# loyer-yuan/GeneralSparse

Hardware: AMD Instinct MI355X
Metric: SpMM GFLOP/s + achieved HBM GB/s vs rocSPARSE, pruned-weight fp16 N=32 (higher is better)
Workload: dtype f16 (fp32 accumulate)

## Files before the change

### generalsparse_amd/_lib.py

```python
import ctypes
import os

PKG_DIR = os.path.dirname(os.path.abspath(__file__))
LIB_PATH = os.environ.get("GS_LIBRARY") or os.path.join(PKG_DIR, "libgeneralsparse.so")

GS_F32 = 0
GS_F16 = 1
GS_BF16 = 2

u64p = ctypes.POINTER(ctypes.c_uint64)
f32p = ctypes.POINTER(ctypes.c_float)
f64p = ctypes.POINTER(ctypes.c_double)


class GsOpts(ctypes.Structure):
    _fields_ = [("pipeline", ctypes.c_char_p), ("dtype", ctypes.c_int), ("dense_n", ctypes.c_int),
                ("p0", ctypes.c_int), ("p1", ctypes.c_int), ("ones_values", ctypes.c_int),
                ("device", ctypes.c_int)]


class GsPlanInfo(ctypes.Structure):
    _fields_ = [("rows", ctypes.c_uint64), ("cols", ctypes.c_uint64), ("nnz", ctypes.c_uint64),
                ("nnz_stored", ctypes.c_uint64), ("n_units", ctypes.c_uint64),
                ("device_bytes_A", ctypes.c_uint64), ("family", ctypes.c_int), ("col_bytes", ctypes.c_int),
                ("dtype", ctypes.c_int), ("replicas", ctypes.c_int), ("needs_memset", ctypes.c_int),
                ("kernel_name", ctypes.c_char * 64), ("lds_stage", ctypes.c_int), ("lds_n", ctypes.c_uint32),
                ("lds_kc", ctypes.c_uint32), ("lds_chunks", ctypes.c_uint32), ("lds_waves", ctypes.c_uint32),
                ("lds_bytes", ctypes.c_uint64), ("tile_bytes", ctypes.c_uint64), ("ksplit", ctypes.c_uint32),
                ("n_kernels", ctypes.c_int), ("device_kernel", ctypes.c_char * 32),
                ("index_formulas", ctypes.c_int), ("index_bytes_saved", ctypes.c_uint64),
                ("ks_nt", ctypes.c_uint32), ("ks_head_groups", ctypes.c_uint32),
                ("nm_tiles", ctypes.c_uint32)]


SIGNATURES = {
    "gs_plan_logical_check": ([ctypes.c_void_p, ctypes.c_char_p, ctypes.c_int], ctypes.c_int),
    "gs_plan_array_set_u64": ([ctypes.c_void_p, ctypes.c_char_p, ctypes.c_uint64, ctypes.c_uint64], ctypes.c_int),
    "gs_last_error": ([], ctypes.c_char_p),
    "gs_version": ([], ctypes.c_char_p),
    "gs_opts_default": ([ctypes.POINTER(GsOpts)], None),
    "gs_plan_create_from_mtx": ([ctypes.c_char_p, ctypes.c_int, ctypes.POINTER(ctypes.c_void_p)], ctypes.c_int),
    "gs_plan_create_from_coo": ([ctypes.c_uint64, ctypes.c_uint64, ctypes.c_uint64, u64p, u64p, f32p,
                                 ctypes.POINTER(ctypes.c_void_p)], ctypes.c_int),
    "gs_set_config_int": ([ctypes.c_char_p, ctypes.c_longlong], ctypes.c_int),
    "gs_get_config_int": ([ctypes.c_char_p, ctypes.POINTER(ctypes.c_longlong)], ctypes.c_int),
    "gs_plan_add_operator": ([ctypes.c_void_p, ctypes.c_char_p, ctypes.POINTER(ctypes.c_longlong), ctypes.c_int],
                             ctypes.c_int),
    "gs_plan_run_pipeline": ([ctypes.c_void_p, ctypes.c_char_p, ctypes.c_int, ctypes.c_int, ctypes.c_int],
                             ctypes.c_int),
    "gs_plan_add_operator_sub": ([ctypes.c_void_p, ctypes.c_int, ctypes.c_char_p, ctypes.POINTER(ctypes.c_longlong),
                                  ctypes.c_int], ctypes.c_int),
    "gs_plan_run_pipeline_sub": ([ctypes.c_void_p, ctypes.c_int, ctypes.c_char_p, ctypes.c_int, ctypes.c_int,
                                  ctypes.c_int], ctypes.c_int),
    "gs_plan_sub_matrices": ([ctypes.c_void_p, ctypes.POINTER(ctypes.c_int), ctypes.c_int], ctypes.c_int),
    "gs_plan_compile": ([ctypes.c_void_p], ctypes.c_int),
    "gs_plan_generate_program": ([ctypes.c_void_p, ctypes.c_char_p, ctypes.c_int, ctypes.c_char_p, ctypes.c_int],
                                 ctypes.c_int),
    "gs_plan_upload": ([ctypes.c_void_p, ctypes.c_int, ctypes.c_int], ctypes.c_int),
    "gs_convert_values": ([f32p, ctypes.c_uint64, ctypes.c_int, ctypes.c_void_p], ctypes.c_int),
    "gs_plan_add_replica": ([ctypes.c_void_p], ctypes.c_int),
    "gs_spmm": ([ctypes.c_void_p, ctypes.c_void_p, ctypes.c_void_p, ctypes.c_int, ctypes.c_void_p], ctypes.c_int),
    "gs_spmm_replica": ([ctypes.c_void_p, ctypes.c_int, ctypes.c_void_p, ctypes.c_void_p, ctypes.c_int,
                         ctypes.c_void_p], ctypes.c_int),
    "gs_spmm_batch": ([ctypes.POINTER(ctypes.c_void_p), ctypes.POINTER(ctypes.c_int), ctypes.POINTER(ctypes.c_void_p),
                       ctypes.POINTER(ctypes.c_void_p), ctypes.c_int, ctypes.c_int, ctypes.c_void_p], ctypes.c_int),
    "gs_spmm_rotate": ([ctypes.c_void_p, ctypes.c_int, ctypes.c_int, ctypes.POINTER(ctypes.c_void_p),
                        ctypes.POINTER(ctypes.c_void_p), ctypes.c_int, ctypes.c_int, ctypes.c_void_p], ctypes.c_int),
    "gs_batch_launches": ([ctypes.POINTER(ctypes.c_void_p), ctypes.POINTER(ctypes.c_int), ctypes.c_int, ctypes.c_int,
                           ctypes.POINTER(ctypes.c_int), ctypes.c_int], ctypes.c_int),
    "gs_plan_device_status": ([ctypes.c_void_p, ctypes.c_void_p], ctypes.c_int),
    "gs_plan_info_get": ([ctypes.c_void_p, ctypes.POINTER(GsPlanInfo)], ctypes.c_int),
    "gs_plan_array_count": ([ctypes.c_void_p], ctypes.c_int),
    "gs_plan_array_key": ([ctypes.c_void_p, ctypes.c_int, ctypes.c_char_p, ctypes.c_int], ctypes.c_int),
    "gs_plan_array_len": ([ctypes.c_void_p, ctypes.c_char_p], ctypes.c_longlong),
    "gs_plan_array_is_float": ([ctypes.c_void_p, ctypes.c_char_p], ctypes.c_int),
    "gs_plan_array_read_u64": ([ctypes.c_void_p, ctypes.c_char_p, u64p, ctypes.c_uint64], ctypes.c_int),
    "gs_plan_array_read_f64": ([ctypes.c_void_p, ctypes.c_char_p, f64p, ctypes.c_uint64], ctypes.c_int),
    "gs_plan_log": ([ctypes.c_void_p, ctypes.c_char_p, ctypes.c_int], ctypes.c_int),
    "gs_plan_save": ([ctypes.c_void_p, ctypes.c_char_p], ctypes.c_int),
    "gs_plan_load": ([ctypes.c_char_p, ctypes.POINTER(ctypes.c_void_p)], ctypes.c_int),
    "gs_plan_index_compression": ([ctypes.c_void_p, ctypes.c_char_p, ctypes.c_char_p, ctypes.c_int, ctypes.c_char_p,
                                   ctypes.c_int, ctypes.POINTER(ctypes.c_int)], ctypes.c_int),
    "gs_index_compression_of_array": ([u64p, ctypes.c_uint64, ctypes.c_int, ctypes.c_int, ctypes.c_char_p, ctypes.c_int,
                                       u64p, ctypes.POINTER(ctypes.c_int)], ctypes.c_int),
    "gs_debug_mfma_timeline": ([ctypes.c_void_p, ctypes.c_void_p, ctypes.c_void_p, ctypes.c_int, ctypes.c_void_p,
# ... 42 lines not shown
```

### generalsparse_amd/csrc/hip_code/mfma_ks.hpp

```cpp
#pragma once

#include "kernel_common.hpp"

namespace gsk {

template <int N>
__device__ constexpr int vmcnt_imm() {
    static_assert(N >= 0 && N < 64, "vmcnt is six bits");
    return (N & 0xF) | ((N >> 4) << 14) | 0x70 | 0xF00;
}


template <int CT, int RT, int W, int D, int MAXG, bool STAMPS, bool AP = true, bool P8 = false, int NTL = 0, class ET = f16>
__device__ __forceinline__ void ks_body(const uint32_t *__restrict__ bmtb_first_row, const u32x4 *__restrict__ tP,
                                        const u32x4 *__restrict__ tV, const u32x2 *__restrict__ steps,
                                        const ET *__restrict__ B, ET *__restrict__ C, uint32_t K, uint32_t N, uint32_t S,
                                        uint32_t NS, uint32_t nwg, uint32_t row_base, float *__restrict__ slabs,
                                        uint32_t *__restrict__ arrivals, uint64_t *__restrict__ stamps, uint32_t bx,
                                        uint32_t prio) {
    constexpr uint32_t RB = 32 * CT;
    constexpr uint32_t UB = 2 * CT;
    constexpr uint32_t IMG = ks_image_bytes<RT>();
    constexpr uint32_t STG = 32u * RB;
    extern __shared__ __attribute__((aligned(16))) unsigned char lds[];
    const uint32_t tid = threadIdx.x, lane = tid & 63u;
    const uint32_t wv = __builtin_amdgcn_readfirstlane(tid >> 6);
    const uint32_t u = xcd_block(bx, nwg);
    const uint32_t g = u / S, q = u - g * S;
#define GS_KS_STAMP(slot)                                                                          \
    if constexpr (STAMPS) {                                                                        \
        if (lane == 0) stamps[((size_t)blockIdx.x * W + wv) * 32u + (slot)] = __builtin_amdgcn_s_memtime(); \
    }
    GS_KS_STAMP(0u);
    const uint32_t k0 = q * NS * 32u;
    const uint32_t col0 = blockIdx.y * 16u * CT, nv = min(16u * CT, N - col0);
    unsigned char *img = lds + wv * (IMG + STG);
    unsigned char *bst = img + IMG;
    const u32x4 zero4 = {0u, 0u, 0u, 0u};

    const uint32_t nsw = NS > wv ? (NS - wv + W - 1u) / W : 0u;
    const size_t ubase = (size_t)u * NS;
    using PV = typename std::conditional<P8, u32x2, u32x4>::type;
    const PV *tPp = reinterpret_cast<const PV *>(tP);
    PV P[D][MAXG];
    u32x4 V[D][MAXG], BR[D][CT];
    u32x2 NX[D];
    uint32_t CN[D];
    uint32_t vz;
    __asm__ volatile("v_mov_b32 %0, 0" : "=v"(vz));
    auto rec_of = [&](uint32_t i) -> u32x2 {
        const uint32_t st = __builtin_amdgcn_readfirstlane(i < nsw ? wv + i * W : 0u);
        return steps[ubase + st + vz];
    };
    auto load_b = [&](uint32_t i, u32x4 (&B_)[CT]) {
        const uint32_t st = __builtin_amdgcn_readfirstlane(i < nsw ? wv + i * W : 0u);
        const uint32_t kr = k0 + st * 32u;
#pragma unroll
        for (int c = 0; c < CT; c++) {
            const uint32_t un = lane + 64u * c;
            const uint32_t k = kr + un / UB, cu = (un % UB) * 8u;
            B_[c] = ld_once_if<(NTL & 2) != 0>(
                reinterpret_cast<const u32x4 *>(B + (size_t)(k < K ? k : K - 1u) * N + col0 + (cu < nv ? cu : 0u)));
        }
    };
    auto load_g_at = [&](uint32_t i, uint32_t b0, uint32_t gc, u32x2 &NX_, uint32_t &CN_, PV (&P_)[MAXG],
                         u32x4 (&V_)[MAXG]) {
        CN_ = gc;
        NX_ = rec_of(i + D);
#pragma unroll
        for (int j = 0; j < MAXG; j++) {
            const uint32_t qg = lane + 64u * j;
            const size_t at = (size_t)b0 + (qg < gc ? qg : 0u);
            P_[j] = ld_once_if<(NTL & 1) != 0>(tPp + at);
            V_[j] = ld_once_if<(NTL & 1) != 0>(tV + at);
        }
    };
    auto load_g = [&](uint32_t i, u32x2 &NX_, uint32_t &CN_, PV (&P_)[MAXG], u32x4 (&V_)[MAXG]) {
        load_g_at(i, __builtin_amdgcn_readfirstlane(NX_[0]), __builtin_amdgcn_readfirstlane(NX_[1]), NX_, CN_, P_, V_);
    };
    const uint32_t GH = (prio >> 8) & 0x3ffu;
    if (GH) {
#pragma unroll
        for (int d = 0; d < D; d++) load_b((uint32_t)d, BR[d]);
#pragma unroll
        for (int d = 0; d < D; d++) {
            const uint32_t st = (uint32_t)d < nsw ? wv + (uint32_t)d * W : 0u;
            load_g_at((uint32_t)d, (u * min((uint32_t)(W * D), NS) + st) * GH, GH, NX[d], CN[d], P[d], V[d]);
        }
        for (uint32_t x = lane; x < IMG / 16u; x += 64u) *reinterpret_cast<u32x4 *>(img + x * 16u) = zero4;
    } else {
#pragma unroll
        for (int d = 0; d < D; d++) NX[d] = rec_of((uint32_t)d);
#pragma unroll
        for (int d = 0; d < D; d++) load_b((uint32_t)d, BR[d]);
        for (uint32_t x = lane; x < IMG / 16u; x += 64u) *reinterpret_cast<u32x4 *>(img + x * 16u) = zero4;
#pragma unroll
        for (int d = 0; d < D; d++) load_g((uint32_t)d, NX[d], CN[d], P[d], V[d]);
    }
    GS_KS_STAMP(1u);

    f4v acc[RT][CT];
#pragma unroll
    for (int rt = 0; rt < RT; rt++)
#pragma unroll
        for (int ct = 0; ct < CT; ct++) acc[rt][ct] = f4v{0.f, 0.f, 0.f, 0.f};
    uint32_t arow[RT];
#pragma unroll
    for (int rt = 0; rt < RT; rt++) arow[rt] = (16u * rt + (lane & 15u)) * kKsStride + 16u * (lane >> 4);

    auto ent_h = [&](const PV &p, uint32_t hb, int e) -> uint32_t {
        if constexpr (P8) {
            const uint32_t b = (p[e >> 2] >> (8 * (e & 3))) & 0x7fu;
            return hb + 48u * (b >> 4) + (b & 15u);
        } else {
            return (p[e >> 1] >> (16 * (e & 1))) & 0xffffu;
        }
    };
    auto grp_hb = [&](const PV &p) -> uint32_t {
        if constexpr (P8) {
            const uint32_t x = p[0], y = p[1];
            const uint32_t sg = ((x >> 7) & 1u) | ((x >> 14) & 2u) | ((x >> 21) & 4u) | ((x >> 28) & 8u) | ((y >> 3) & 16u);
            return 384u * (sg >> 1) + 16u * (sg & 1u);
        } else {
            return 0u;
        }
    };
    auto step = [&](uint32_t i, u32x2 &NX_, uint32_t &CN_, PV (&P_)[MAXG], u32x4 (&V_)[MAXG], u32x4 (&B_)[CT]) {
        const bool live = i < nsw;
        const uint32_t gc = CN_;
        typedef typename mfma_elem<ET>::frag frag;
        frag av[RT], bv[CT];
        if (live) {
            const uint32_t kr = k0 + (wv + i * W) * 32u;
#pragma unroll
            for (int c = 0; c < CT; c++) {
                const uint32_t un = lane + 64u * c, k = un / UB, s = un % UB;
                *reinterpret_cast<u32x4 *>(bst + k * RB + b_piece<CT>(k, s >> 1) * 32u + (s & 1u) * 16u) =
                    kr + k < K && s * 8u < nv ? B_[c] : zero4;
            }
#pragma unroll
            for (int j = 0; j < MAXG; j++) {
                if (lane + 64u * j < gc) {
                    const uint32_t hb = grp_hb(P_[j]);
#pragma unroll
                    for (int e = 0; e < 8; e++) {
                        const uint32_t h = ent_h(P_[j], hb, e);
                        const uint16_t v = (uint16_t)((V_[j][e >> 1] >> (16 * (e & 1))) & 0xffffu);
                        *reinterpret_cast<uint16_t *>(img + h * 2u) = v;
                    }
                }
            }
#pragma unroll
            for (int rt = 0; rt < RT; rt++) av[rt] = *reinterpret_cast<const frag *>(img + arow[rt]);
            const uint32_t kb = 8u * (lane >> 4);
#pragma unroll
            for (int ct = 0; ct < CT; ct++) {
                s4v t[2];
#pragma unroll
                for (int hh = 0; hh < 2; hh++) {
                    const uint32_t k = kb + 4u * hh + ((lane & 15u) >> 2);
                    t[hh] = __builtin_amdgcn_ds_read_tr16_b64_v4i16(
                        (lds_s4v *)(bst + k * RB + b_piece<CT>(k, ct) * 32u + (lane & 3u) * 8u));
                }
                __builtin_memcpy(&bv[ct], t, 16);
            }
#pragma unroll
            for (int j = 0; j < MAXG; j++) {
                if (lane + 64u * j < gc) {
                    const uint32_t hb = grp_hb(P_[j]);
#pragma unroll
                    for (int e = 0; e < 8; e++) *reinterpret_cast<uint16_t *>(img + ent_h(P_[j], hb, e) * 2u) = (uint16_t)0;
                }
            }
        }
        load_b(i + D, B_);
        load_g(i + D, NX_, CN_, P_, V_);
        if (live) {
#pragma unroll
            for (int rt = 0; rt < RT; rt++)
#pragma unroll
                for (int ct = 0; ct < CT; ct++)
                    acc[rt][ct] = mfma_elem<ET>::mfma_16x16x32(av[rt], bv[ct], acc[rt][ct]);
            if (i < 16u) GS_KS_STAMP(3u + i);
        }
    };
    const bool young = wv >= W / 2u;
    if ((prio & 3u) && young) __builtin_amdgcn_s_setprio(1);
    for (uint32_t i0 = 0; i0 < nsw; i0 += D) {
#pragma unroll
        for (int d = 0; d < D; d++) step(i0 + d, NX[d], CN[d], P[d], V[d], BR[d]);
        if ((prio & 3u) == 2u && young && i0 + D >= nsw / 2u && i0 < nsw / 2u) __builtin_amdgcn_s_setprio(0);
    }
    if ((prio & 3u) && young) __builtin_amdgcn_s_setprio(0);
    GS_KS_STAMP(20u);
    uint32_t *arr = arrivals + (size_t)g * gridDim.y + blockIdx.y;
    uint32_t ticket = 0;
    if (S > 1 && wv == 0 && lane == 0) ticket = __hip_atomic_fetch_add(arr, 1u, __ATOMIC_RELAXED, __HIP_MEMORY_SCOPE_AGENT);
    constexpr bool APART = ks_red_apart(CT, RT, W, AP);
    f4v *red = reinterpret_cast<f4v *>(lds + (APART ? (size_t)W * (IMG + STG) : 0u));
    constexpr bool HALVES = !APART && ks_red_halves(CT, RT, W);
    constexpr uint32_t WR = HALVES ? W / 2 : W;
    uint32_t *flag = reinterpret_cast<uint32_t *>(reinterpret_cast<unsigned char *>(red) + (size_t)WR * RT * CT * 1024u);
    if constexpr (!APART) {
        __asm__ volatile("s_waitcnt lgkmcnt(0)" ::: "memory");
        __builtin_amdgcn_s_barrier();
        __asm__ volatile("" ::: "memory");
    }
    if constexpr (HALVES) {
        if (wv >= WR) {
#pragma unroll
            for (int rt = 0; rt < RT; rt++)
#pragma unroll
                for (int ct = 0; ct < CT; ct++) red[(((wv - WR) * RT + rt) * CT + ct) * 64u + lane] = acc[rt][ct];
        }
        __asm__ volatile("s_waitcnt lgkmcnt(0)" ::: "memory");
        __builtin_amdgcn_s_barrier();
        __asm__ volatile("" ::: "memory");
        if (wv < WR) {
#pragma unroll
            for (int rt = 0; rt < RT; rt++)
#pragma unroll
                for (int ct = 0; ct < CT; ct++) acc[rt][ct] += red[((wv * RT + rt) * CT + ct) * 64u + lane];
        }
        __asm__ volatile("s_waitcnt lgkmcnt(0)" ::: "memory");
        __builtin_amdgcn_s_barrier();
        __asm__ volatile("" ::: "memory");
    }
    if (wv < WR) {
#pragma unroll
        for (int rt = 0; rt < RT; rt++)
#pragma unroll
            for (int ct = 0; ct < CT; ct++) red[((wv * RT + rt) * CT + ct) * 64u + lane] = acc[rt][ct];
    }
    if (S > 1 && wv == 0 && lane == 0) *flag = ticket;
    __asm__ volatile("s_waitcnt lgkmcnt(0)" ::: "memory");
    __builtin_amdgcn_s_barrier();
    __asm__ volatile("" ::: "memory");
    constexpr uint32_t NI = RT * CT * 64u, NT = 64u * W;
    const uint32_t r0 = bmtb_first_row[g], R = bmtb_first_row[g + 1] - r0;
    auto item_sum = [&](uint32_t t) {
        f4v sum = red[t];
#pragma unroll
        for (uint32_t w = 1; w < WR; w++) sum += red[w * NI + t];
// ... 4 lines not shown
        const uint32_t col = 16u * ct + (ln & 15u), rb = 16u * rt + 4u * (ln >> 4);
        if (col >= nv) return;
#pragma unroll
        for (uint32_t i = 0; i < 4; i++)
            if (rb + i < R) C[(size_t)(row_base + r0 + rb + i) * N + col0 + col] = (ET)v[i];
    };
    GS_KS_STAMP(21u);
    if (S == 1) {
        for (uint32_t t = tid; t < NI; t += NT) store_item(t, item_sum(t));
        GS_KS_STAMP(22u);
        return;
    }
    const uint32_t tk = *flag & 0xffffu, tag = ((*flag >> 16) & 1u) ^ 1u;
    f4v *slab = reinterpret_cast<f4v *>(slabs) + ((size_t)u * gridDim.y + blockIdx.y) * NI;
    auto tagged = [&](const f4v &v) {
        u32x4 w;
        __builtin_memcpy(&w, &v, 16);
        w[0] = (w[0] & ~1u) | tag; w[1] = (w[1] & ~1u) | tag; w[2] = (w[2] & ~1u) | tag; w[3] = (w[3] & ~1u) | tag;
        return w;
    };
    for (uint32_t t = tid; t < NI; t += NT) {
        const u32x4 w = tagged(item_sum(t));
        __asm__ volatile("global_store_dwordx4 %0, %1, off sc1" ::"v"(slab + t), "v"(w) : "memory");
    }
    if (tk != S - 1u) {
        GS_KS_STAMP(22u);
        return;
    }
    if (tid == 0) __hip_atomic_store(arr, tag << 16, __ATOMIC_RELAXED, __HIP_MEMORY_SCOPE_AGENT);
    const f4v *base = reinterpret_cast<const f4v *>(slabs) + blockIdx.y * NI;
    const size_t qstride = (size_t)gridDim.y * NI;
    uint32_t *err = arrivals + (size_t)(nwg / S) * gridDim.y;
    for (uint32_t t = tid; t < NI; t += NT) {
        f4v sum = {0.f, 0.f, 0.f, 0.f};
        for (uint32_t qq = 0; qq < S; qq++) {
            u32x4 w;
            if (qq == q) {
                w = tagged(item_sum(t));
            } else {
                w = ks_slab_wait(reinterpret_cast<const uint32_t *>(base + ((size_t)g * S + qq) * qstride + t), tag, err,
                                 GS_KS_FORCE(prio));
            }
            w[0] &= ~1u; w[1] &= ~1u; w[2] &= ~1u; w[3] &= ~1u;
            f4v x;
            __builtin_memcpy(&x, &w, 16);
            sum += x;
        }
        store_item(t, sum);
    }
    GS_KS_STAMP(22u);
#undef GS_KS_STAMP
}

template <int CT, int RT, int W, int D, int MAXG, bool STAMPS = false, bool AP = true, bool P8 = false, int NTL = 0, class ET = f16>
__global__ __launch_bounds__(64 * W) void k_mfma_ks(const uint32_t *__restrict__ bmtb_first_row,
                                                    const u32x4 *__restrict__ tP,
                                                    const u32x4 *__restrict__ tV,
                                                    const u32x2 *__restrict__ steps,
                                                    const ET *__restrict__ B, ET *__restrict__ C, uint32_t K,
                                                    uint32_t N, uint32_t S, uint32_t NS, uint32_t nwg,
                                                    uint32_t row_base, float *__restrict__ slabs,
                                                    uint32_t *__restrict__ arrivals, uint64_t *__restrict__ stamps = nullptr,
                                                    uint32_t prio = 0) {
    ks_body<CT, RT, W, D, MAXG, STAMPS, AP, P8, NTL, ET>(bmtb_first_row, tP, tV, steps, B, C, K, N, S, NS, nwg, row_base, slabs,
                                                    arrivals, stamps, blockIdx.x, prio);
}

#ifdef GS_EXPERIMENTS
template <int CT, int RT, int W, int D, int MAXG, int NTL = 0>
__global__ __launch_bounds__(64 * W) void k_mfma_ks_persist(const uint32_t *__restrict__ bmtb_first_row,
                                                            const u32x4 *__restrict__ tP, const u32x4 *__restrict__ tV,
                                                            const u32x2 *__restrict__ steps, const f16 *__restrict__ B,
                                                            f16 *__restrict__ C, uint32_t K, uint32_t N, uint32_t S,
                                                            uint32_t NS, uint32_t nunits, uint32_t row_base,
                                                            float *__restrict__ slabs, uint32_t *__restrict__ arrivals,
                                                            uint32_t prio, uint32_t *__restrict__ queue) {
    __shared__ uint32_t next_sh;
    uint32_t xcc;
    asm volatile("s_getreg_b32 %0, hwreg(HW_REG_XCC_ID, 0, 4)" : "=s"(xcc));
    xcc &= 7u;
    const uint32_t grid = gridDim.x;
    uint32_t u = blockIdx.x, qx = xcc, tried = 0;
    while (u < nunits) {
        uint32_t pulled = 0;
        if (threadIdx.x == 0) pulled = __hip_atomic_fetch_add(queue + qx, 1u, __ATOMIC_RELAXED, __HIP_MEMORY_SCOPE_AGENT);
        ks_body<CT, RT, W, D, MAXG, false, true, false, NTL>(bmtb_first_row, tP, tV, steps, B, C, K, N, S, NS, nunits,
                                                          row_base, slabs, arrivals, nullptr, u, prio);
        __syncthreads();
        if (threadIdx.x == 0) next_sh = pulled;
        __syncthreads();
        u = grid + qx + 8u * next_sh;
        __syncthreads();
        while (u >= nunits && ++tried < 8u) {
            qx = (qx + 1u) & 7u;
            if (threadIdx.x == 0) next_sh = __hip_atomic_fetch_add(queue + qx, 1u, __ATOMIC_RELAXED, __HIP_MEMORY_SCOPE_AGENT);
            __syncthreads();
            u = grid + qx + 8u * next_sh;
            __syncthreads();
        }
    }
    if (threadIdx.x == 0 && __hip_atomic_fetch_add(queue + 8, 1u, __ATOMIC_RELAXED, __HIP_MEMORY_SCOPE_AGENT) == grid - 1u) {
        for (int i = 0; i < 9; i++) __hip_atomic_store(queue + i, 0u, __ATOMIC_RELAXED, __HIP_MEMORY_SCOPE_AGENT);
    }
}
#endif

struct ks_entry {
    const uint32_t *tbr;
    const u32x4 *tP, *tV;
    const u32x2 *steps;
    const void *B;
    void *C;
    float *slabs;
    uint32_t *arrivals;
    uint32_t K, S, NS, nwg, row_base, pad0, pad1, pad2;
};
struct ks_group_args {
    uint32_t begin[kKsGroupMax + 1];
    uint32_t n, N, pad[2];
    ks_entry e[kKsGroupMax];
};

template <int CT, int RT, int W, int D, int MAXG, bool P8 = false, bool AP = true, int NTL = 0, class ET = f16>
__global__ __launch_bounds__(64 * W) void k_mfma_ks_group(ks_group_args args) {
    const uint32_t bx = blockIdx.x, n = args.n;
    uint32_t sel = 0;
#pragma unroll
    for (int i = 1; i < kKsGroupMax; i++)
        if ((uint32_t)i < n && args.begin[i] <= bx) sel = (uint32_t)i;
    sel = __builtin_amdgcn_readfirstlane(sel);
    const ks_entry &e = args.e[sel];
    if (bx - args.begin[sel] >= e.nwg) return;
    ks_body<CT, RT, W, D, MAXG, false, AP, P8, NTL, ET>(e.tbr, e.tP, e.tV, e.steps, (const ET *)e.B, (ET *)e.C, e.K, args.N, e.S, e.NS,
                                                   e.nwg, e.row_base, e.slabs, e.arrivals, nullptr, bx - args.begin[sel],
                                                   args.pad[0] | (e.pad0 << 8));
}

}
```

### generalsparse_amd/csrc/host/capi.cc

```cpp
#include "../../../include/generalsparse.h"
#include "gs_plan.hpp"
#include "index_compress.hpp"

#include <algorithm>
#include <cstring>
#include <map>
#include <memory>

struct replica_scratch {
    std::vector<void *> bufs;
    void **ptrs_dev = nullptr;
    uint32_t N = 0;
};

struct parent_group {
    uint64_t base = 0, rows = 0;
    std::vector<gs::plan_state *> subs;
    std::vector<uint32_t> part_rows;
    std::vector<replica_scratch> rep;
    uint32_t *rows_dev = nullptr;
    int device = 0;
};

struct gs_plan {
// ... 758 lines not shown
                                   "): the affected rows of C hold NaN", GS_ERR_DEVICE);
    });
}

int gs_spmm(gs_plan_t *p, const void *B, void *C, int N, gs_stream_t stream) {
    return gs_spmm_replica(p, 0, B, C, N, stream);
}

int gs_debug_mfma_timeline(gs_plan_t *p, const void *B, void *C, int N, gs_stream_t stream, uint64_t *stamps,
                           uint64_t n_stamps) {
    return guard([&] {
        GS_CHECK(p && B && C && stamps, "null argument");
        gs::debug_mfma_timeline(p->st, B, C, (uint32_t)N, (hipStream_t)stream, stamps, n_stamps);
    });
}

int gs_plan_info_get(gs_plan_t *p, gs_plan_info *info) {
    return guard([&] {
        GS_CHECK(p && info, "null argument");
        std::memset(info, 0, sizeof(*info));
        auto ks = kernel_states(p, false);
        auto &s = *ks.front();
        info->rows = s.M;
        info->cols = s.K;
        info->nnz = s.nnz;
        info->n_kernels = (int)ks.size();
        for (gs::plan_state *k : ks) info->nnz_stored += s.meta->u(gs::GLOBAL_META, "nz_col_indices", k->cg->get_sub_matrix_id()).size();
        if (s.cg->is_compiled()) {
            const auto &sp = s.cg->get_kernel_spec();
            info->family = sp.family;
            std::strncpy(info->kernel_name, sp.name().c_str(), sizeof(info->kernel_name) - 1);
        }
        if (s.uploaded) {
            info->n_units = s.dev.n_units;
            info->device_bytes_A = s.dev.bytes_A;
            info->col_bytes = s.dev.col_bytes;
            info->dtype = s.dev.dtype;
            info->replicas = (int)s.dev.replicas.size();
            info->needs_memset = s.dev.needs_memset ? 1 : 0;
            info->lds_stage = s.dev.nm ? 3 : (s.dev.mfma ? 2 : (s.dev.lds ? 1 : 0));
            info->lds_n = s.dev.lds_N;
            info->lds_kc = s.dev.KC;
            info->lds_chunks = s.dev.nc;
            info->lds_waves = s.dev.waves;
            info->lds_bytes = s.dev.lds_bytes;
            info->tile_bytes = s.dev.bytes_tile;
            info->ksplit = s.dev.ksplit;
            const std::string dk = !s.dev.kernel.empty() ? s.dev.kernel : s.cg->get_kernel_spec().name();
            std::strncpy(info->device_kernel, dk.c_str(), sizeof(info->device_kernel) - 1);
            info->index_formulas = s.dev.index_formulas;
            info->index_bytes_saved = s.dev.index_bytes_saved;
            info->ks_nt = s.dev.ks ? s.dev.ks_nt : 0;
            info->ks_head_groups = s.dev.ks ? s.dev.ks_gh : 0;
            info->nm_tiles = s.dev.nm ? s.dev.nm_tiles : 0;
        }
    });
}

int gs_plan_array_count(gs_plan_t *p) { return p ? (int)p->st.meta->keys().size() : GS_ERR_ARG; }

int gs_plan_array_key(gs_plan_t *p, int i, char *buf, int buf_len) {
    return guard([&] {
        GS_CHECK(p && buf && buf_len > 0, "bad argument");
        auto k = p->st.meta->keys();
        GS_CHECK(i >= 0 && (size_t)i < k.size(), "index out of range");
        std::strncpy(buf, k[i].c_str(), buf_len - 1);
        buf[buf_len - 1] = 0;
    });
}

long long gs_plan_array_len(gs_plan_t *p, const char *key) {
    if (!p || !key || !p->st.meta->is_exist(key)) return -1;
    return (long long)p->st.meta->get_element(key)->meta_data_arr->get_len();
}

int gs_plan_array_is_float(gs_plan_t *p, const char *key) {
    if (!p || !key || !p->st.meta->is_exist(key)) return GS_ERR_ARG;
    return p->st.meta->get_element(key)->meta_data_arr->is_float() ? 1 : 0;
}

int gs_plan_array_read_u64(gs_plan_t *p, const char *key, uint64_t *out, uint64_t n) {
    return guard([&] {
        GS_CHECK(p && key && out, "null argument");
        auto a = p->st.meta->get_element(key)->meta_data_arr;
        GS_CHECK(!a->is_float(), "array is a value array");
        GS_CHECK(n >= a->get_len(), "buffer too small");
        std::copy(a->u().begin(), a->u().end(), out);
    });
}

int gs_plan_array_read_f64(gs_plan_t *p, const char *key, double *out, uint64_t n) {
    return guard([&] {
        GS_CHECK(p && key && out, "null argument");
        auto a = p->st.meta->get_element(key)->meta_data_arr;
        GS_CHECK(n >= a->get_len(), "buffer too small");
        for (uint64_t i = 0; i < a->get_len(); i++) out[i] = a->read_float_from_arr(i);
    });
}

int gs_plan_log(gs_plan_t *p, char *buf, int buf_len) {
    return guard([&] {
        GS_CHECK(p && buf && buf_len > 0, "bad argument");
        std::string s;
        for (auto &l : p->st.exec->log()) s += l + "\n";
        std::strncpy(buf, s.c_str(), buf_len - 1);
        buf[buf_len - 1] = 0;
// ... 107 lines not shown
```

### generalsparse_amd/csrc/host/code_generator.cc

```cpp
#include "code_generator.hpp"
#include "device_layout.hpp"
#include "index_compress.hpp"

#include <cstdio>
#include <filesystem>
#include <fstream>
#include <sstream>
#include <sys/stat.h>

#include <dlfcn.h>

namespace gs {

const char *reduction_kind_name(reduction_kind k) {
    switch (k) {
        case reduction_kind::TOTAL_BMT_RESULT: return "total_BMT_result_reduce_to_one_register_token";
        case reduction_kind::THREAD_BIT_MAP: return "thread_bit_map_reduce_to_two_register_token";
        case reduction_kind::TOTAL_WARP_RESULT: return "total_warp_result_reduce_to_one_register_token";
        case reduction_kind::WARP_SEGMENT: return "warp_segment_reduce_token";
        case reduction_kind::TOTAL_BLOCK_RESULT: return "total_block_reduce_to_one_register_token";
        case reduction_kind::WARP_BIT_MAP: return "warp_bit_map_reduce_token";
        case reduction_kind::TBLOCK_BIT_MAP: return "tblock_bit_map_reduce_token";
        default: return "none";
    }
// ... 152 lines not shown
    if (sub != 0)
        for (auto &k : s.arrays)
            if (k.size() > 2 && k.compare(k.size() - 2, 2, "_0") == 0) k = k.substr(0, k.size() - 2) + "_" + std::to_string(sub);
    for (auto &k : s.arrays) GS_CHECK(m.is_exist(k), "compile: plan array missing: " + k);
    if (grid.size() == 2) s.ref_grid = {{grid[0], grid[1]}};
    if (block.size() == 2) s.ref_block = {{block[0], block[1]}};
    spec = s;
    compiled = true;
}

namespace {

std::string matrix_core_source(const meta_data_set &m, const mc_layout &L, int repeat) {
    std::ostringstream o;
    const uint32_t N = L.N, CT = L.kind == mc_layout::NM ? std::max<uint32_t>(1, N / 16)
                                                         : (L.kind == mc_layout::KS ? L.ks.CT : ks_ct(N));
    const uint32_t NT = L.kind == mc_layout::KS ? ks_col_tiles_ct(N, CT) : ks_col_tiles(N);
    const char *kname = L.kind == mc_layout::KS ? "k_mfma_ks"
                        : L.kind == mc_layout::BM ? (L.bm.kb ? "k_mfma_kb" : L.bm.v2 ? "k_mfma_bm2" : "k_mfma_bm")
                        : L.kind == mc_layout::ROWS ? "k_mfma_rows"
                        : (L.nm_ks ? "k_nm_mfma_ks" : (L.nm4 ? "k_nm_mfma4" : "k_nm_mfma"));
    o << "// kernel_file.hip -- generated by generalsparse_amd code_generator: the matrix-core kernel " << kname << "\n"
      << "// build: sh make_kernel.sh; run: ./a.out [matrix.mtx] [N]  -> perf_result (ms, GFLOP/s)\n"
      << (L.kind == mc_layout::BM || L.nm_ks || L.nm4 || L.rows_flags ? "#define GS_EXPERIMENTS  // an experiments-build kernel\n" : "")
      << "#include \"kernel_lib.hpp\"\n#include <cstdio>\n#include <cstdlib>\n#include <cstring>\n#include <fstream>\n"
      << "#include <string>\n#include <vector>\n\n"
      << "typedef gsk::f16 VT;\n"
      << "static std::vector<uint64_t> rd(const char *n) {\n"
      << "    std::ifstream f(n); std::vector<uint64_t> v; unsigned long long x; while (f >> x) v.push_back(x); return v; }\n"
      << "static std::vector<double> rdf(const char *n) {\n"
      << "    std::ifstream f(n); std::vector<double> v; double x; while (f >> x) v.push_back(x); return v; }\n"
      << "template <class T> static std::vector<T> rdb(const char *n) {  // binary sidecar\n"
      << "    std::ifstream f(n, std::ios::binary | std::ios::ate); std::vector<T> v((size_t)f.tellg() / sizeof(T));\n"
      << "    f.seekg(0); f.read(reinterpret_cast<char *>(v.data()), v.size() * sizeof(T)); return v; }\n"
      << "template <class T> static T *up(const std::vector<T> &h, size_t pad = 64) {\n"
      << "    T *p; hipMalloc(&p, (h.size() + pad) * sizeof(T)); hipMemset(p, 0, (h.size() + pad) * sizeof(T));\n"
      << "    hipMemcpy(p, h.data(), h.size() * sizeof(T), hipMemcpyHostToDevice); return p; }\n\n"
      << "int main(int argc, char **argv) {\n"
      << "    const uint32_t N = argc > 2 ? (uint32_t)atoi(argv[2]) : " << N << ";\n"
      << "    if (N != " << N << ") { printf(\"this program's " << kname << " layout is built for N = " << N
      << "\\n\"); return 2; }\n"
      << "    const int repeat = " << repeat << ";\n"
      << "    const uint64_t M = " << m.scalar(GLOBAL_META, "origin_row_num", -1) << ", K = "
      << m.scalar(GLOBAL_META, "origin_col_num", -1) << ", NNZ = " << m.scalar(GLOBAL_META, "origin_nnz_num", -1) << ";\n"
      << "    auto rows = rd(\"GLOBAL_META_nz_row_indices_0\");\n"
      << "    auto vals = rdf(\"GLOBAL_META_nz_vals_0\");\n"
      << "    uint64_t row_num = rows.back() + 1;\n";
    std::string launch, setup;
    if (L.kind == mc_layout::KS) {
        const ks_tiles &t = L.ks;
        const uint64_t nb = L.tbr.size() - 1, nwg = nb * t.S;
        o << "    auto tbr = rd(\"TBLOCK_META_first_row_indices_0\");\n"
          << "    std::vector<uint32_t> t32(tbr.begin(), tbr.end()); uint32_t *d_tbr = up(t32);\n"
          << (t.P8 ? "    uint8_t *d_pos = up(rdb<uint8_t>(\"TBLOCK_META_mfma_ks_entry_pos_0.bin\"));  // 8-bit positions\n"
                   : "    uint16_t *d_pos = up(rdb<uint16_t>(\"TBLOCK_META_mfma_ks_entry_pos_0.bin\"));\n")
          << "    uint16_t *d_val = up(rdb<uint16_t>(\"TBLOCK_META_mfma_ks_entry_val_0.bin\"));\n"
          << "    uint32_t *d_steps = up(rdb<uint32_t>(\"TBLOCK_META_mfma_ks_steps_0.bin\"));\n"
          << "    // the tagged slabs start (and are left by every launch) all 0\n"
          << "    float *d_ws; uint32_t *d_arr; hipMalloc(&d_ws, " << nwg * NT * 256 * t.RT * CT * 4 << "ull + 16);\n"
          << "    hipMemset(d_ws, 0, " << nwg * NT * 256 * t.RT * CT * 4 << "ull + 16);\n"
          << "    hipMalloc(&d_arr, " << nb * NT * 4 << "ull + 4); hipMemset(d_arr, 0, " << nb * NT * 4
          << "ull + 4);\n";
        const std::string k = "gsk::k_mfma_ks<" + std::to_string(CT) + ", " + std::to_string(t.RT) + ", " +
                              std::to_string(t.W) + ", " + std::to_string(kKsDepth) + ", " + std::to_string(t.MAXG) +
                              std::string(", false, ") + (t.AP ? "true" : "false") + ", " + (t.P8 ? "true" : "false") +
                              (t.NT ? ", " + std::to_string(t.NT) + ">" : ">");
        setup = "hipFuncSetAttribute((const void *)" + k + ", hipFuncAttributeMaxDynamicSharedMemorySize, " +
                std::to_string(t.lds_bytes) + ")";
        launch = k + "<<<dim3(" + std::to_string(nwg) + ", " + std::to_string(NT) + "), " +
                 std::to_string(64 * t.W) + ", " + std::to_string(t.lds_bytes) +
                 ">>>(d_tbr, (const gsk::u32x4 *)d_pos, (const gsk::u32x4 *)d_val, (const gsk::u32x2 *)d_steps, d_B, d_C, "
                 "(uint32_t)K, N, " + std::to_string(t.S) + "u, " + std::to_string(t.NS) + "u, " + std::to_string(nwg) + "u, 0u, d_ws, d_arr, nullptr, " +
                 std::to_string((uint32_t)get_config().KS_PRIO | (t.GH << 8)) + "u)";
    } else if (L.kind == mc_layout::BM) {
        const bm_tiles &t = L.bm;
        const uint64_t nb = L.tbr.size() - 1, nwg = nb * t.S;
        o << "    auto tbr = rd(\"TBLOCK_META_first_row_indices_0\");\n"
          << "    std::vector<uint32_t> t32(tbr.begin(), tbr.end()); uint32_t *d_tbr = up(t32);\n"
          << "    uint32_t *d_rec = up(rdb<uint32_t>(\"TBLOCK_META_mfma_bm_records_0.bin\"));\n"
          << "    uint32_t *d_sb = up(rdb<uint32_t>(\"TBLOCK_META_mfma_bm_step_base_0.bin\"));\n"
          << "    uint16_t *d_val = up(rdb<uint16_t>(\"TBLOCK_META_mfma_bm_values_0.bin\"));\n"
          << "    float *d_ws; uint32_t *d_arr; hipMalloc(&d_ws, " << nwg * ks_col_tiles(N) * 256 * t.RT * CT * 4 << "ull + 16);\n"
          << "    hipMalloc(&d_arr, " << nb * ks_col_tiles(N) * t.RT * 4 << "ull + 4); hipMemset(d_arr, 0, "
          << nb * ks_col_tiles(N) * t.RT * 4 << "ull + 4);\n";
        if (t.kb) o << "    hipMemset(d_ws, 0, " << nwg * ks_col_tiles(N) * 256 * t.RT * CT * 4 << "ull + 16);\n";
        const std::string k = t.kb ? "gsk::k_mfma_kb<" + std::to_string(CT) + ", " + std::to_string(t.RT) + ", " +
                                         std::to_string(t.W) + ", " + std::to_string(kKsDepth) + ", " +
                                         std::to_string(t.NVB) + ">"
                            : t.v2 ? "gsk::k_mfma_bm2<" + std::to_string(CT) + ", " + std::to_string(t.RT) + ">"
                                   : "gsk::k_mfma_bm<" + std::to_string(CT) + ", " + std::to_string(t.RT) + ", " +
                                         std::to_string(t.W) + ", " + std::to_string(gsk::bm_nbt(CT, t.RT)) + ">";
        setup = "hipFuncSetAttribute((const void *)" + k + ", hipFuncAttributeMaxDynamicSharedMemorySize, " +
                std::to_string(t.lds_bytes) + ")";
        launch = k + "<<<dim3(" + std::to_string(nwg) + ", " + std::to_string(ks_col_tiles(N)) + "), " +
                 std::to_string(64 * t.W) + ", " + std::to_string(t.lds_bytes) +
                 ">>>(d_tbr, (const uint2 *)d_rec, d_sb, (const gsk::f16 *)d_val, d_B, d_C, (uint32_t)K, N, " +
                 std::to_string(t.S) + "u, " + std::to_string(t.NS) + "u, " + std::to_string(nwg) + "u, 0u, d_ws, d_arr" +
                 (t.kb ? ", nullptr, " + std::to_string(get_config().KS_PRIO) + "u)" : std::string(")"));
    } else if (L.kind == mc_layout::ROWS) {
        const mfma_tiles &t = L.rows;
        const uint64_t nb = L.tbr.size() - 1;
        o << "    auto tbr = rd(\"TBLOCK_META_first_row_indices_0\");\n"
          << "    std::vector<uint32_t> t32(tbr.begin(), tbr.end()); uint32_t *d_tbr = up(t32);\n"
          << "    uint32_t *d_seg = up(rdb<uint32_t>(\"TBLOCK_META_mfma_seg_start_0.bin\"));\n"
          << "    uint16_t *d_pos = up(rdb<uint16_t>(\"TBLOCK_META_mfma_entry_pos_0.bin\"));\n"
          << "    uint16_t *d_val = up(rdb<uint16_t>(\"TBLOCK_META_mfma_entry_val_0.bin\"));\n"
          << "    float *d_ws = nullptr; uint32_t *d_arr = nullptr;\n";
        if (L.rows_ksplit > 1)
            o << "    hipMalloc(&d_ws, " << nb * L.rows_ksplit * t.RMAX * N * 4 << "ull); hipMalloc(&d_arr, " << nb * 4
              << "ull); hipMemset(d_arr, 0, " << nb * 4 << "ull);\n";
        const std::string k = "gsk::k_mfma_rows<" + std::to_string(CT) + ", " + std::to_string(t.RT) + ", " +
                              std::to_string(t.lgKC) + ", " + std::to_string(L.rows_maxa) + ", false, " +
                              std::to_string(L.rows_glds) + ", " + std::to_string(L.rows_nbg) + ", " +
                              std::to_string(L.rows_wct) + (L.rows_flags ? ", 0, true>" : ">");
        setup = "hipFuncSetAttribute((const void *)" + k + ", hipFuncAttributeMaxDynamicSharedMemorySize, " +
                std::to_string(t.lds_bytes) + ")";
        launch = k + "<<<" + std::to_string(nb * L.rows_ksplit) + ", " + std::to_string(kMfmaThreads) + ", " +
                 std::to_string(t.lds_bytes) + ">>>(d_tbr, d_seg, (const gsk::u32x4 *)d_pos, (const gsk::u32x4 *)d_val, d_B, d_C, " +
                 "(uint32_t)K, N, " + std::to_string(t.nc) + "u, " + std::to_string(t.RMAX) + "u, 0u, " +
                 std::to_string(L.rows_ksplit) + "u, " + std::to_string(L.rows_ncs) + "u, d_ws, d_arr, nullptr, 0u)";
    } else if (L.nm_ks) {
        const uint64_t nb = (L.nm_rows + 255) / 256, ngr = nb * 4;
        o << "    unsigned char *d_blk = up(rdb<unsigned char>(\"THREAD_META_nm_panels_0.bin\"));\n"
          << "    float *d_ws; uint32_t *d_arr; hipMalloc(&d_ws, " << ngr * L.nm_split * 64 * N * 4 << "ull + 16);\n"
          << "    hipMalloc(&d_arr, " << ngr * 4 << "ull); hipMemset(d_arr, 0, " << ngr * 4 << "ull);\n";
        const std::string k = "gsk::k_nm_mfma_ks<" + std::to_string(CT) + ">";
// ... 224 lines not shown
                         "d_r0, d_rr, d_r1, n_units, N, X, 0, (uint32_t)M, d_a4, (uint32_t)lay.empty.size(), 64u, nullptr, nullptr); "
                         "gsk::k_merge_fixup<VT><<<dim3((n_units * N + 255) / 256), 256>>>(d_rr, d_r0, d_r1, d_C, n_units, N)";
            break;
        }
        default:
            throw gs_error("no family");
    }
    o << "    std::vector<VT> hB(K * N, (VT)1.0f);  // x_arr = 1 (code_generator.cc:464-467)\n"
      << "    VT *d_B = up(hB, 0); VT *d_C; hipMalloc(&d_C, M * N * sizeof(VT)); hipMemset(d_C, 0, M * N * sizeof(VT));\n"
      << "    auto run = [&]() {\n"
      << "        if (al && N % " << cf << " == 0) {\n"
      << "            constexpr int CF = " << cf << ", SCF = 4; uint32_t X = 1; while (X < 64 && X * CF < N) X <<= 1;\n"
      << "            uint32_t tiles = (N + X * CF - 1) / (X * CF); " << launch << ";\n"
      << "        } else {\n"
      << "            constexpr int CF = 1, SCF = 1; uint32_t X = 1; while (X < 64 && X * CF < N) X <<= 1;\n"
      << "            uint32_t tiles = (N + X * CF - 1) / (X * CF); " << launch << ";\n"
      << "        }\n"
      << "    };\n"
      << "    run(); hipDeviceSynchronize();\n"
      << "    // check (kernel_lib.hpp:884-921 of the reference): all-ones B, C[i][j] = sum of row i's values\n"
      << "    std::vector<VT> hC(M * N); hipMemcpy(hC.data(), d_C, M * N * sizeof(VT), hipMemcpyDeviceToHost);\n"
      << "    std::vector<double> ref(M, 0.0);\n"
      << "    std::vector<uint64_t> orig_of(row_num);\n";
    if (spec.row_sorted)
        o << "    { auto order = rd(\"GLOBAL_META_original_nz_row_indices_0\"); for (uint64_t i = 0; i < row_num; i++) orig_of[i] = order[i]; }\n";
    else
        o << "    for (uint64_t i = 0; i < row_num; i++) orig_of[i] = i;\n";
    o << "    for (size_t i = 0; i < rows.size(); i++) ref[orig_of[rows[i]]] += vals[i];\n"
      << "    long wrong = 0;\n"
      << "    for (uint64_t i = 0; i < M; i++) for (uint32_t j = 0; j < N; j++) {\n"
      << "        double c = (double)(float)hC[i * N + j], r = (double)(float)(VT)(float)ref[i];\n"
      << "        const double tol = " << (half ? "1e-1" : "1e-3") << " * (1 + (r < 0 ? -r : r));  // north_star fp16 / fp32\n"
      << "        if (c - r > tol || r - c > tol) {\n"
      << "            if (wrong < 10) printf(\"Wrong result: i = %llu, j = %u, result = %f, reference = %f.\\n\", (unsigned long long)i, j, c, r);\n"
      << "            wrong++; } }\n"
      << "    printf(\"wrong number:%ld\\n\", wrong); if (!wrong) printf(\"correct\\n\");\n"
      << "    hipEvent_t e0, e1; hipEventCreate(&e0); hipEventCreate(&e1);\n"
      << "    hipEventRecord(e0, 0); for (int i = 0; i < repeat; i++) run(); hipEventRecord(e1, 0); hipEventSynchronize(e1);\n"
      << "    float ms = 0; hipEventElapsedTime(&ms, e0, e1);\n"
      << "    double gflops = " << get_config().FLOAT_RATE << ".0 * (double)NNZ * N * repeat / (ms * 1e-3) / 1e9;\n"
      << "    FILE *pr = fopen(\"perf_result\", \"w\"); fprintf(pr, \"%f\\n%f\\n\", ms, gflops); fclose(pr);  // code_generator.cc:643-648\n"
      << "    printf(\"time %f ms for %d launches, %f GFLOP/s\\n\", ms, repeat, gflops);\n"
      << "    return wrong ? 1 : 0;\n}\n";
    return o.str();
}

uint64_t code_generator::generate_final_program(int repeat, const std::string &root, std::string *dir_out) {
    GS_CHECK(compiled, "compile() before generate_final_program");
    GS_CHECK(sub == 0, "the standalone program is emitted for an undivided matrix");
    std::string dir;
    uint64_t id = meta->output_format_to_dir(root, spec.arrays, &dir);
    const mc_layout L = emitted_layout(*meta, spec, sub);
    if (L.kind == mc_layout::KS) {
        if (L.ks.P8)
            write_bin(dir + "/TBLOCK_META_mfma_ks_entry_pos_0.bin", L.ks.pos8);
        else
            write_bin(dir + "/TBLOCK_META_mfma_ks_entry_pos_0.bin", L.ks.pos);
        write_bin(dir + "/TBLOCK_META_mfma_ks_entry_val_0.bin", L.ks.val);
        write_bin(dir + "/TBLOCK_META_mfma_ks_steps_0.bin", L.ks.steps);
    } else if (L.kind == mc_layout::BM) {
        write_bin(dir + "/TBLOCK_META_mfma_bm_records_0.bin", L.bm.rec);
        write_bin(dir + "/TBLOCK_META_mfma_bm_step_base_0.bin", L.bm.sbase);
        write_bin(dir + "/TBLOCK_META_mfma_bm_values_0.bin", L.bm.val);
    } else if (L.kind == mc_layout::ROWS) {
        write_bin(dir + "/TBLOCK_META_mfma_seg_start_0.bin", L.rows.seg_start);
        write_bin(dir + "/TBLOCK_META_mfma_entry_pos_0.bin", L.rows.pos);
        write_bin(dir + "/TBLOCK_META_mfma_entry_val_0.bin", L.rows.val);
    } else if (L.kind == mc_layout::NM) {
        write_bin(dir + "/THREAD_META_nm_panels_0.bin", L.nm_blk);
    }
    {
        std::ofstream f(dir + "/kernel_file.hip");
        f << (L.kind != mc_layout::NONE ? matrix_core_source(*meta, L, repeat) : generate_gather_source(repeat));
    }
    std::string hdr_dir;
    Dl_info info;
    if (dladdr((void *)&kernel_family_name, &info) && info.dli_fname) {
        std::string so = info.dli_fname;
        hdr_dir = so.substr(0, so.find_last_of('/') + 1) + "csrc/hip_code/";
    }
    if (!hdr_dir.empty()) {
        std::error_code ec;
        for (const auto &ent : std::filesystem::directory_iterator(hdr_dir, ec)) {
            if (ent.path().extension() != ".hpp") continue;
            std::ifstream in(ent.path(), std::ios::binary);
            std::ofstream out(dir + "/" + ent.path().filename().string(), std::ios::binary);
            out << in.rdbuf();
        }
        if (ec) fprintf(stderr, "generalsparse: no device headers copied from %s: %s\n", hdr_dir.c_str(), ec.message().c_str());
    }
    {
        std::ofstream f(dir + "/make_kernel.sh");
        f << "hipcc --offload-arch=gfx950 -O3 -std=c++17 kernel_file.hip -o a.out\n";
    }
    if (dir_out) *dir_out = dir;
    return id;
}

}
```

### generalsparse_amd/csrc/host/device_layout.cc

```cpp
#include "device_layout.hpp"

#include <algorithm>
#include <cstring>

namespace gs {

uint16_t f32_to_f16_bits(float f) {
    uint32_t x;
    std::memcpy(&x, &f, 4);
    const uint32_t sign = (x >> 16) & 0x8000u, exp = (x >> 23) & 0xffu;
    uint32_t man = x & 0x7fffffu;
    if (exp == 0xffu) return (uint16_t)(sign | 0x7c00u | (man ? (0x200u | (man >> 13)) : 0u));
    const int e = (int)exp - 127 + 15;
    if (e >= 31) return (uint16_t)(sign | 0x7c00u);
    if (e <= 0) {
        if (e < -10) return (uint16_t)sign;
        man |= 0x800000u;
        const int shift = 14 - e;
        uint32_t hm = man >> shift;
        const uint32_t rem = man & ((1u << shift) - 1u), halfway = 1u << (shift - 1);
        if (rem > halfway || (rem == halfway && (hm & 1u))) hm++;
        return (uint16_t)(sign | hm);
    }
    uint32_t h = sign | ((uint32_t)e << 10) | (man >> 13);
    const uint32_t rem = man & 0x1fffu;
    if (rem > 0x1000u || (rem == 0x1000u && (h & 1u))) h++;
    return (uint16_t)h;
}

uint16_t f32_to_bf16_bits(float f) {
    uint32_t x;
    std::memcpy(&x, &f, 4);
    if ((x & 0x7fffffffu) > 0x7f800000u) return (uint16_t)((x >> 16) | 0x0040u);
    return (uint16_t)((x + 0x7fffu + ((x >> 16) & 1u)) >> 16);
}

void convert_values(const float *in, uint64_t n, int dtype, void *out) {
    GS_CHECK(dtype_ok(dtype), "dtype must be 0 (fp32), 1 (fp16) or 2 (bf16)");
    if (dtype == kF32) {
        if (n) std::memcpy(out, in, n * sizeof(float));
        return;
    }
    uint16_t *o = static_cast<uint16_t *>(out);
    for (uint64_t i = 0; i < n; i++) o[i] = value_bits16(in[i], dtype);
}



canon_rows canonical_rows(const std::vector<uint32_t> &rp, const std::vector<uint64_t> &col, const universal_array &vals) {
    canon_rows c;
    const uint64_t nr = rp.size() - 1;
    c.rp.assign(nr + 1, 0);
    c.col.reserve(col.size());
    c.val.reserve(col.size());
    std::vector<std::pair<uint64_t, uint64_t>> ent;
// ... 84 lines not shown
    for (const auto &bk : bucket) GS_CHECK(bk.empty(), "bank ordering lost an entry");
}

static size_t pos8_step(const std::vector<uint16_t> &row, const std::vector<uint16_t> &colw,
                        const std::vector<uint16_t> &hv, uint32_t RS, std::vector<uint8_t> &out_pos8,
                        std::vector<uint16_t> &out_val) {
    const size_t n = row.size();
    uint32_t nseg = 0;
    for (size_t i = 0; i < n; i++) nseg = std::max<uint32_t>(nseg, (uint32_t)((row[i] / 8) * 2 + colw[i] / 16) + 1);
    std::vector<std::vector<uint32_t>> seg(nseg);
    for (uint32_t i = 0; i < n; i++) seg[(row[i] / 8) * 2 + colw[i] / 16].push_back(i);
    size_t groups = 0;
    std::vector<std::vector<uint32_t>> bucket(32);
    for (uint32_t sg = 0; sg < nseg; sg++) {
        const auto &es = seg[sg];
        if (es.empty()) continue;
        GS_CHECK(sg < 256, "KS_POS8: segment id beyond 8 bits");
        const size_t ng = (es.size() + 7) / 8;
        for (auto &b : bucket) b.clear();
        for (uint32_t i : es) bucket[((uint32_t)row[i] * RS + colw[i]) / 2 % 32].push_back(i);
        std::vector<uint32_t> slot(ng * 8, UINT32_MAX);
        std::vector<int> order(32);
        for (int e = 0; e < 8; e++) {
            for (int k = 0; k < 32; k++) order[k] = k;
            std::stable_sort(order.begin(), order.end(), [&](int a, int b) { return bucket[a].size() > bucket[b].size(); });
            size_t l = 0;
            bool progress = true;
            while (l < ng && progress) {
                progress = false;
                for (int k = 0; k < 32 && l < ng; k++) {
                    auto &bk = bucket[order[k]];
                    if (bk.empty()) continue;
                    slot[l * 8 + e] = bk.back();
                    bk.pop_back();
                    l++;
                    progress = true;
                }
            }
        }
        for (const auto &bk : bucket) GS_CHECK(bk.empty(), "KS_POS8: bank ordering lost an entry");
        const uint32_t first = slot[0];
        for (size_t gi = 0; gi < ng; gi++)
            for (int e = 0; e < 8; e++) {
                const uint32_t i = slot[gi * 8 + e] == UINT32_MAX ? first : slot[gi * 8 + e];
                const uint8_t p7 = (uint8_t)(((row[i] % 8) << 4) | (colw[i] % 16));
                out_pos8.push_back((uint8_t)((((sg >> e) & 1u) << 7) | p7));
                out_val.push_back(hv[i]);
            }
        groups += ng;
    }
    return groups;
}

bool build_mfma_tiles(const std::vector<uint64_t> &tb_rows, const std::vector<uint32_t> &row_ptr,
                      const std::vector<uint64_t> &col, const std::vector<float> &vals, uint64_t K, uint32_t N,
                      size_t lds_budget, int64_t max_fill, mfma_tiles &t, std::string &why) {
    const uint64_t nb = tb_rows.size() - 1;
    if (nb == 0 || K == 0) { why = "empty plan"; return false; }
    if (N == 0 || N > 64 || N % 8 != 0) { why = "N must be a multiple of 8 up to 64"; return false; }
    const uint32_t CT = ks_ct(N);
    uint64_t rmax = 0, nnz = 0;
    for (uint64_t g = 0; g < nb; g++) rmax = std::max<uint64_t>(rmax, tb_rows[g + 1] - tb_rows[g]);
    for (uint64_t g = 0; g < nb; g++) nnz += row_ptr[tb_rows[g + 1]] - row_ptr[tb_rows[g]];
    if (rmax == 0 || rmax > 64) { why = "BMTBs of 1..64 rows only"; return false; }
    const uint32_t RT = (uint32_t)((rmax + 15) / 16);
    if (nnz == 0 || (double)nb * 16 * RT * K > (double)max_fill * nnz) {
        why = "row blocks too sparse for dense tiles";
        return false;
    }
    if ((double)nb * K * N * 2 > 6.0 * 4.0 * nnz && max_fill < (1 << 20)) {
        why = "row blocks too short: B traffic per row block exceeds A's";
        return false;
    }
    for (uint32_t lg = 10; lg >= 8; lg--) {
        const uint64_t KC = 1ull << lg;
        if ((rmax + 1) * (KC + 16) > 65536 || mfma_lds_bytes(lg, CT, (uint32_t)rmax) > lds_budget) continue;
        const uint64_t nc = (K + KC - 1) / KC;
        uint64_t gmax = 0;
        std::vector<uint64_t> cnt(nc);
        for (uint64_t g = 0; g < nb; g++) {
            std::fill(cnt.begin(), cnt.end(), 0);
            for (uint64_t e = row_ptr[tb_rows[g]]; e < row_ptr[tb_rows[g + 1]]; e++) cnt[col[e] >> lg]++;
            for (uint64_t j = 0; j < nc; j++) gmax = std::max(gmax, (cnt[j] + 7) / 8);
        }
        if (gmax > 2ull * kMfmaAThreads || nc > 63) continue;
        if (((KC * 32 * CT) / 16) % kMfmaBThreads) continue;
        if ((KC * 32 * CT) / 16 / kMfmaBThreads > 8) continue;
        if ((size_t)gsk::kMfmaCompute * RT * CT * 1024 > mfma_lds_bytes(lg, CT, (uint32_t)rmax)) continue;
        t.lgKC = lg; t.nc = (uint32_t)nc; t.RT = RT; t.RMAX = (uint32_t)rmax;
        t.MAXA = gmax <= kMfmaAThreads ? 1 : 2;
        t.gmax = (uint32_t)gmax;
        t.lds_bytes = mfma_lds_bytes(lg, CT, (uint32_t)rmax);
        break;
    }
    if (!t.lgKC) { why = "no chunk width fits LDS and the stage buffers"; return false; }
    const uint32_t KC = 1u << t.lgKC;
    t.seg_start.assign(1, 0);
    std::vector<uint64_t> cur;
    std::vector<uint16_t> pos, hv;
    for (uint64_t g = 0; g < nb; g++) {
        const uint64_t r0 = tb_rows[g], R = tb_rows[g + 1] - r0;
        cur.assign(R, 0);
        for (uint64_t i = 0; i < R; i++) cur[i] = row_ptr[r0 + i];
        for (uint32_t j = 0; j < t.nc; j++) {
            const uint64_t lim = (uint64_t)(j + 1) * KC;
            pos.clear();
// ... 3 lines not shown
                for (; e < row_ptr[r0 + i + 1] && col[e] < lim; e++) {
                    pos.push_back((uint16_t)(i * (KC + 16) + (col[e] - (uint64_t)j * KC)));
                    hv.push_back(f32_to_f16_bits(vals[e]));
                }
                cur[i] = e;
            }
            bank_order_segment(pos, hv, (uint32_t)(R * (KC + 16)), t.pos, t.val);
            t.seg_start.push_back((uint32_t)(t.pos.size() / 8));
        }
    }
    t.pos.insert(t.pos.end(), 8, 0);
    t.val.insert(t.val.end(), 8, 0);
    return true;
}




bool build_ks_tiles(const std::vector<uint64_t> &tb_rows, const std::vector<uint32_t> &row_ptr,
                    const std::vector<uint64_t> &col, const std::vector<float> &vals, uint64_t K, uint32_t N,
                    int64_t s_cfg, int64_t min_rows, int64_t max_fill, ks_tiles &t, std::string &why, int dtype) {
    const uint64_t nb = tb_rows.size() - 1;
    if (nb == 0 || K == 0) { why = "empty plan"; return false; }
    if (N == 0 || N % 8 != 0) { why = "N must be a multiple of 8"; return false; }
    uint32_t W = kKsWaves;
    uint64_t rmax = 0;
    for (uint64_t g = 0; g < nb; g++) rmax = std::max<uint64_t>(rmax, tb_rows[g + 1] - tb_rows[g]);
    if (rmax < (uint64_t)std::max<int64_t>(1, min_rows) || rmax > 128) { why = "row blocks outside the k_mfma_ks range"; return false; }
    const uint32_t RT = std::max<uint32_t>(2, (uint32_t)((rmax + 15) / 16));
    const uint32_t CT = ks_ct_rt(N, RT);
    t.CT = CT;
    if (RT > 5 && CT > 2) { why = "row blocks over 80 rows at N > 32"; return false; }
    if (get_config().KS_WAVES == 16 && CT <= 4 && gsk::ks_lds_bytes(CT, RT, 16) <= 160 * 1024) W = 16;
    if (get_config().KS_WAVES == 4 && CT == 2) W = 4;
    if (get_config().KS_WAVES == 12 && CT == 2 && RT <= 5 && gsk::ks_lds_bytes(CT, RT, 12) <= 160 * 1024) W = 12;
    const uint64_t nnz = row_ptr[tb_rows[nb]] - row_ptr[tb_rows[0]];
    if (nnz == 0 || (double)nb * 16 * RT * K > (double)max_fill * nnz) {
        why = "row blocks too sparse for dense tiles";
        return false;
    }
    {
        const int64_t ap = get_config().KS_APART;
        const bool can_overlap = CT == 2 && ((RT <= 5 && W == kKsWaves) || W == 4);
        const size_t la = gsk::ks_lds_bytes(CT, RT, W, true), lo = gsk::ks_lds_bytes(CT, RT, W, false);
        t.AP = W != 4 && (!can_overlap || ap > 0 || (ap < 0 && (160u * 1024u) / la >= (160u * 1024u) / lo));
    }
    t.lds_bytes = gsk::ks_lds_bytes(CT, RT, W, t.AP);
    if (t.lds_bytes > 160 * 1024) { why = "k_mfma_ks wave stages exceed LDS"; return false; }
    t.RT = RT;
    t.RMAX = (uint32_t)rmax;
    t.W = W;
    t.P8 = get_config().KS_POS8 && CT == 2 && (W == kKsWaves || W == 4);
    t.NT = (CT == 2 || CT == 8) && (W == kKsWaves || W == 12) && !t.P8 && t.AP && get_config().KS_NT ? 1u : 0u;
    uint64_t gmax = 1;
    {
        const uint32_t nsg = 4 * RT;
        std::vector<uint32_t> cnt((size_t)((K + 31) / 32) * (t.P8 ? nsg : 1u));
        for (uint64_t g = 0; g < nb; g++) {
            std::fill(cnt.begin(), cnt.end(), 0u);
            for (uint64_t r = tb_rows[g]; r < tb_rows[g + 1]; r++)
                for (uint64_t e = row_ptr[r]; e < row_ptr[r + 1]; e++) {
                    const uint64_t st = col[e] / 32;
                    if (t.P8)
                        cnt[st * nsg + ((r - tb_rows[g]) / 8) * 2 + (col[e] % 32) / 16]++;
                    else
                        cnt[st]++;
                }
            if (t.P8) {
                for (size_t st = 0; st < cnt.size() / nsg; st++) {
                    uint64_t ngs = 0;
                    for (uint32_t k = 0; k < nsg; k++) ngs += (cnt[st * nsg + k] + 7) / 8;
                    gmax = std::max<uint64_t>(gmax, ngs);
                }
            } else {
                for (uint32_t c : cnt) gmax = std::max<uint64_t>(gmax, (c + 7) / 8);
            }
        }
    }
    t.GCAP = (uint32_t)gmax;
    t.MAXG = gmax <= 64 ? 1 : (gmax <= 128 ? 2 : (gmax <= 192 ? 3 : (gmax <= 256 ? 4 : 0)));
    if (!t.MAXG) { why = "a k-step holds more than 256 entry groups"; return false; }
    if (t.CT == 8 && !ks_ct8_fits(RT, t.MAXG)) {
        t.CT = 4;
        t.NT = 0;
        t.lds_bytes = gsk::ks_lds_bytes(4, RT, W, t.AP);
    }
    if (!t.AP && t.MAXG > 2 && W != 4) {
        t.AP = true;
        t.lds_bytes = gsk::ks_lds_bytes(t.CT, RT, W, true);
        if (t.lds_bytes > 160 * 1024) { why = "k_mfma_ks wave stages exceed LDS"; return false; }
    }
    {
        const uint64_t ctiles = ks_col_tiles_ct(N, t.CT);
        uint64_t S = s_cfg > 0 ? (uint64_t)s_cfg : std::min<uint64_t>(8, (256 + nb * ctiles - 1) / (nb * ctiles));
        S = std::max<uint64_t>(1, std::min<uint64_t>(S, (K + 31) / 32));
        const uint64_t KR = ((K + S - 1) / S + 31) / 32 * 32;
        t.S = (uint32_t)((K + KR - 1) / KR);
        t.NS = (uint32_t)(KR / 32);
    }
    const uint64_t S = t.S, KR = (uint64_t)t.NS * 32;
    const uint32_t HS = std::min<uint32_t>(W * kKsDepth, t.NS);
    if (!t.P8 && get_config().KS_HEAD) {
        uint64_t gh = 1, head_groups = 0, all_groups = 0;
        std::vector<uint32_t> c2((size_t)S * t.NS);
        for (uint64_t g = 0; g < nb; g++) {
            std::fill(c2.begin(), c2.end(), 0u);
            for (uint64_t r = tb_rows[g]; r < tb_rows[g + 1]; r++)
                for (uint64_t e = row_ptr[r]; e < row_ptr[r + 1]; e++) c2[col[e] / 32]++;
            for (size_t st = 0; st < c2.size(); st++) {
                const uint64_t ng = (c2[st] + 7) / 8;
                all_groups += ng;
                if (st % t.NS < HS) {
                    head_groups += ng;
                    gh = std::max(gh, ng);
                }
            }
        }
        const uint64_t padded = (uint64_t)nb * S * HS * gh;
        if ((double)(padded - head_groups) <= 0.06 * (double)all_groups && (double)padded < 2.0e9) t.GH = (uint32_t)gh;
    }
    if ((double)(row_ptr[tb_rows[nb]] - row_ptr[tb_rows[0]]) / 8.0 + (double)nb * S * t.NS * 2.0 >= 4.0e9) {
        why = "k_mfma_ks layout exceeds 32-bit group indices";
        return false;
    }
    const uint32_t RS = gsk::kKsStride / 2;
    const uint32_t pad_h = 16 * RT * RS;
    if (t.P8)
        t.pos8.reserve(row_ptr[tb_rows[nb]] - row_ptr[tb_rows[0]] + (size_t)nb * S * t.NS * 8 * RT + 8);
    else
        t.pos.reserve(row_ptr[tb_rows[nb]] - row_ptr[tb_rows[0]] + (size_t)nb * S * t.NS * 8 + 8);
    t.val.reserve(t.P8 ? t.pos8.capacity() : t.pos.capacity());
    t.steps.reserve((size_t)nb * S * t.NS * 2);
    if (t.GH) {
        t.pos.assign((size_t)nb * S * HS * t.GH * 8, (uint16_t)pad_h);
        t.val.assign(t.pos.size(), 0);
    }
    std::vector<uint64_t> cur;
    std::vector<uint16_t> pos, hv, prow, pcol, hpos, hval;
    for (uint64_t g = 0; g < nb; g++) {
        const uint64_t r0 = tb_rows[g], R = tb_rows[g + 1] - r0;
        cur.assign(R, 0);
        for (uint64_t i = 0; i < R; i++) cur[i] = row_ptr[r0 + i];
        for (uint64_t q = 0; q < S; q++)
            for (uint32_t s = 0; s < t.NS; s++) {
                const uint64_t base = q * KR + 32ull * s, lim = base + 32;
                pos.clear();
                hv.clear();
                prow.clear();
                pcol.clear();
                for (uint64_t i = 0; i < R; i++) {
                    uint64_t e = cur[i];
                    for (; e < row_ptr[r0 + i + 1] && col[e] < lim; e++) {
                        pos.push_back((uint16_t)(i * RS + (col[e] - base)));
                        prow.push_back((uint16_t)i);
                        pcol.push_back((uint16_t)(col[e] - base));
                        hv.push_back(value_bits16(vals[e], dtype));
                    }
                    cur[i] = e;
                }
                size_t before, ng;
                if (t.GH && s < HS) {
                    hpos.clear();
                    hval.clear();
                    bank_order_segment(pos, hv, pad_h, hpos, hval, RS / 2);
                    ng = hpos.size() / 8;
                    GS_CHECK(ng <= t.GH, "k_mfma_ks head step exceeds its slot");
                    before = (((size_t)g * S + q) * HS + s) * t.GH * 8;
                    std::copy(hpos.begin(), hpos.end(), t.pos.begin() + before);
                    std::copy(hval.begin(), hval.end(), t.val.begin() + before);
                } else if (t.P8) {
                    before = t.pos8.size();
                    ng = pos8_step(prow, pcol, hv, RS, t.pos8, t.val);
                } else {
                    before = t.pos.size();
                    bank_order_segment(pos, hv, pad_h, t.pos, t.val, RS / 2);
                    ng = (t.pos.size() - before) / 8;
                }
                GS_CHECK(ng <= t.GCAP, "k_mfma_ks step exceeds its capacity");
                t.steps.push_back((uint32_t)(before / 8));
                t.steps.push_back((uint32_t)ng);
            }
    }
    if (t.P8)
        t.pos8.insert(t.pos8.end(), 8, (uint8_t)0);
    else
        t.pos.insert(t.pos.end(), 8, (uint16_t)pad_h);
    t.val.insert(t.val.end(), 8, 0);
    return true;
}

bool build_bm_tiles(const std::vector<uint64_t> &tb_rows, const std::vector<uint32_t> &row_ptr,
                    const std::vector<uint64_t> &col, const std::vector<float> &vals, uint64_t K, uint32_t N,
                    int64_t s_cfg, int64_t waves, int64_t max_fill, bm_tiles &t, std::string &why) {
    const uint64_t nb = tb_rows.size() - 1;
    if (nb == 0 || K == 0) { why = "empty plan"; return false; }
    if (N == 0 || N % 8 != 0) { why = "N must be a multiple of 8"; return false; }
    uint64_t rmax = 0;
    for (uint64_t g = 0; g < nb; g++) rmax = std::max<uint64_t>(rmax, tb_rows[g + 1] - tb_rows[g]);
    if (rmax == 0 || rmax > 96) { why = "row blocks outside the k_mfma_bm range (1..96 rows)"; return false; }
    const uint32_t RT = (uint32_t)((rmax + 15) / 16);
    const uint64_t nnz = row_ptr[tb_rows[nb]] - row_ptr[tb_rows[0]];
    if (nnz == 0 || (double)nb * 16 * RT * K > (double)max_fill * nnz) {
        why = "row blocks too sparse for dense tiles";
        return false;
    }
    const bool kb = get_config().BM_KB;
    const uint32_t W = kb || waves != 4 ? 8u : 4u;
    uint64_t S = s_cfg > 0 ? (uint64_t)s_cfg
                           : kb ? std::min<uint64_t>(8, (256 + nb - 1) / nb) : std::max<uint64_t>(1, std::min<uint64_t>(8, 256 / nb));
    S = std::max<uint64_t>(1, std::min<uint64_t>(S, (K + 31) / 32));
    const uint64_t KR = ((K + S - 1) / S + 31) / 32 * 32;
    S = (K + KR - 1) / KR;
    t.S = (uint32_t)S;
    t.NS = (uint32_t)(KR / 32);
    t.RT = RT;
    t.RMAX = (uint32_t)rmax;
    t.W = W;
    t.lds_bytes = gsk::bm_lds_bytes(ks_ct(N), RT, W);
    const size_t slice = 128u + (size_t)t.NS * 32u * 32u * ks_ct(N);
    t.kb = kb;
    t.v2 = !kb && get_config().BM_V2 && slice <= 160u * 1024u;
    if (t.v2) {
        t.lds_bytes = slice;
        t.W = RT;
    }
    const uint64_t nrec = nb * S * t.NS * 64;
    GS_CHECK(nrec < (1ull << 31), "k_mfma_bm layout exceeds 31-bit record indices");
    t.rec.assign(nrec * 2, 0u);
    auto rec_of = [&](uint64_t g, uint64_t i, uint64_t c, uint32_t &tt, uint32_t &bit) -> uint64_t {
        const uint64_t qq = c / KR, cc = c % KR, st = cc / 32, w = cc % 32;
        tt = (uint32_t)(i / 16);
        bit = (uint32_t)(w % 8);
        const uint64_t lane = (w / 8) * 16 + i % 16;
        return ((g * S + qq) * t.NS + st) * 64 + lane;
    };
    auto mask_byte = [&](uint64_t r, uint32_t tt) -> uint32_t {
// ... 232 lines not shown
```

### generalsparse_amd/csrc/host/device_layout.hpp

```cpp
#pragma once

#include "gs_core.hpp"
#include "code_generator.hpp"
#include "../hip_code/kernel_consts.hpp"

#include <string>
#include <vector>

namespace gs {

constexpr uint32_t kMfmaThreads = 64 * gsk::kMfmaWaves;
constexpr uint32_t kKsWaves = 8, kKsDepth = 2;

uint16_t f32_to_f16_bits(float f);
uint16_t f32_to_bf16_bits(float f);

constexpr int kF32 = 0, kF16 = 1, kBF16 = 2;
inline bool dtype_ok(int dtype) { return dtype == kF32 || dtype == kF16 || dtype == kBF16; }
inline uint32_t elem_bytes(int dtype) { return dtype == kF32 ? 4u : 2u; }
inline uint16_t value_bits16(float f, int dtype) { return dtype == kBF16 ? f32_to_bf16_bits(f) : f32_to_f16_bits(f); }
void convert_values(const float *in, uint64_t n, int dtype, void *out);

struct canon_rows {
    std::vector<uint32_t> rp;
    std::vector<uint64_t> col;
    std::vector<float> val;
};

canon_rows canonical_rows(const std::vector<uint32_t> &rp, const std::vector<uint64_t> &col, const universal_array &vals);

struct mfma_tiles {
    uint32_t lgKC = 0, nc = 0, RT = 0, RMAX = 0, MAXA = 0, gmax = 0;
    size_t lds_bytes = 0;
    std::vector<uint32_t> seg_start;
    std::vector<uint16_t> pos, val;
};

size_t mfma_lds_bytes(uint32_t lgKC, uint32_t CT, uint32_t RMAX);
size_t mfma_rows_lds_need(uint32_t lgKC, uint32_t CT, uint32_t RT, uint32_t RMAX, int glds, int nbg, int wct);
bool build_mfma_tiles(const std::vector<uint64_t> &tb_rows, const std::vector<uint32_t> &row_ptr,
                      const std::vector<uint64_t> &col, const std::vector<float> &vals, uint64_t K, uint32_t N,
                      size_t lds_budget, int64_t max_fill, mfma_tiles &t, std::string &why);

struct ks_tiles {
    uint32_t S = 0, NS = 0, RT = 0, RMAX = 0, MAXG = 0, GCAP = 0, W = 0;
    uint32_t CT = 0;
    bool AP = true;
    bool P8 = false;
    uint32_t NT = 0;
    uint32_t GH = 0;
    size_t lds_bytes = 0;
    std::vector<uint16_t> pos, val;
    std::vector<uint8_t> pos8;
    std::vector<uint32_t> steps;
};

inline uint32_t ks_ct(uint32_t N) { return N <= 16 ? 1u : (N <= 32 ? 2u : 4u); }
inline uint32_t ks_col_tiles(uint32_t N) { return (N + 16 * ks_ct(N) - 1) / (16 * ks_ct(N)); }
inline uint32_t ks_ct_rt(uint32_t N, uint32_t RT) { return N >= 128 && RT <= 3 ? 8u : ks_ct(N); }
inline bool ks_ct8_fits(uint32_t RT, uint32_t MAXG) { return (RT == 2 && MAXG <= 3) || (RT == 3 && MAXG == 1); }
inline uint32_t ks_col_tiles_ct(uint32_t N, uint32_t CT) { return (N + 16 * CT - 1) / (16 * CT); }

bool build_ks_tiles(const std::vector<uint64_t> &tb_rows, const std::vector<uint32_t> &row_ptr,
                    const std::vector<uint64_t> &col, const std::vector<float> &vals, uint64_t K, uint32_t N,
                    int64_t s_cfg, int64_t min_rows, int64_t max_fill, ks_tiles &t, std::string &why, int dtype = kF16);

struct bm_tiles {
    uint32_t S = 0, NS = 0, RT = 0, RMAX = 0, W = 0;
    bool kb = false;
    uint32_t NVB = 0;
    bool v2 = false;
    size_t lds_bytes = 0;
    std::vector<uint32_t> rec;
    std::vector<uint32_t> sbase;
    std::vector<uint16_t> val;
};

bool build_bm_tiles(const std::vector<uint64_t> &tb_rows, const std::vector<uint32_t> &row_ptr,
                    const std::vector<uint64_t> &col, const std::vector<float> &vals, uint64_t K, uint32_t N,
                    int64_t s_cfg, int64_t waves, int64_t max_fill, bm_tiles &t, std::string &why);

bool build_nm_panels(const std::vector<uint64_t> &rows, const std::vector<uint64_t> &col, const universal_array &vals,
                     uint64_t row_num, uint64_t K, std::vector<unsigned char> &blk, uint32_t &S, std::string &why,
                     uint32_t T = 8);
uint32_t nm_tiles_for(uint64_t row_num, int64_t cfg_tiles, uint32_t N);

struct mc_layout {
    enum kind_t { NONE, ROWS, KS, NM, BM } kind = NONE;
    uint32_t N = 0;
    std::vector<uint64_t> tbr;
    mfma_tiles rows;
    uint32_t rows_ksplit = 1, rows_ncs = 0;
    int rows_glds = 2, rows_nbg = 3, rows_wct = 6, rows_maxa = 1;
    bool rows_flags = false;
    ks_tiles ks;
    bm_tiles bm;
    std::vector<unsigned char> nm_blk;
    uint32_t nm_S = 0;
    uint32_t nm_T = 8;
    uint64_t nm_rows = 0;
    bool nm_ks = false;
    bool nm4 = false;
    bool nm_nt = false;
    uint32_t nm_split = 1, nm_ncs = 0;
    std::string why;
};
// ... 4 lines not shown
```

### generalsparse_amd/csrc/host/gs_core.cc

```cpp
#include "gs_core.hpp"

#include <algorithm>
#include <atomic>
#include <chrono>
#include <cmath>
#include <cstdio>
#include <cstdlib>
#include <cstring>
#include <fstream>
#include <sstream>
#include <sys/stat.h>

namespace gs {

std::string code_of_data_type(data_type t) {
    switch (t) {
        case CHAR: return "char";
        case UNSIGNED_CHAR: return "unsigned char";
        case SHORT: return "short";
        case UNSIGNED_SHORT: return "unsigned short";
        case INT: return "int";
        case UNSIGNED_INT: return "unsigned int";
        case LONG: return "long";
        case UNSIGNED_LONG: return "unsigned long";
// ... 59 lines not shown
bool g_cfg_loaded = false;
config_t g_cfg;

void apply_kv(config_t &c, const std::string &k, const std::string &v) {
    auto b = [&]() { return v == "true" || v == "1"; };
    auto i = [&]() { return (int64_t)std::atof(v.c_str()); };
    if (k == "DENSE_MATRIX_SIZE") c.DENSE_MATRIX_SIZE = i();
    else if (k == "VECTOR_WIDTH") c.VECTOR_WIDTH = i();
    else if (k == "HALF") c.HALF = b();
    else if (k == "PRECISE_OF_FLOAT") c.PRECISE_OF_FLOAT = v;
    else if (k == "ROOT_PATH_STR") c.ROOT_PATH_STR = v;
    else if (k == "DATA_SET") c.DATA_SET = v;
    else if (k == "OPERATOR_RUNTIME_CHECK") c.OPERATOR_RUNTIME_CHECK = b();
    else if (k == "PADDING_RATE_UP_BOUND") c.PADDING_RATE_UP_BOUND = i();
    else if (k == "DATA_TYPE_COMPRESS") c.DATA_TYPE_COMPRESS = b();
    else if (k == "BRANCH_COMPRESS_MAX_SIZE") c.BRANCH_COMPRESS_MAX_SIZE = i();
    else if (k == "FLOAT_RATE") c.FLOAT_RATE = i();
    else if (k == "GFLOPS_UP_BOUND") c.GFLOPS_UP_BOUND = std::atof(v.c_str());
    else if (k == "SHARED_MEM_TOTAL_SIZE") c.SHARED_MEM_TOTAL_SIZE = i();
    else if (k == "MAX_DIV_TIMES_OF_DIV") c.MAX_DIV_TIMES_OF_DIV = i();
    else if (k == "MFMA_GLDS") c.MFMA_GLDS = i();
    else if (k == "MFMA_GLDS_NBUF") c.MFMA_GLDS_NBUF = i();
    else if (k == "MFMA_COMPUTE_WAVES") c.MFMA_COMPUTE_WAVES = i();
    else if (k == "FORMAT_OF_MTX") c.FORMAT_OF_MTX = v;
    else if (k == "PERFORMANCE_FLAG") c.PERFORMANCE_FLAG = v;
    else if (k == "Graph_Algorithm") c.Graph_Algorithm = v;
    else if (k == "MODEL_DRIVEN_COMPRESS") c.MODEL_DRIVEN_COMPRESS = b();
    else if (k == "LDS_STAGE_B") c.LDS_STAGE_B = b();
    else if (k == "MFMA_TILES") c.MFMA_TILES = b();
    else if (k == "MFMA_MAX_FILL") c.MFMA_MAX_FILL = i();
    else if (k == "MFMA_KROT") c.MFMA_KROT = i();
    else if (k == "WARP_ROWS_GROUPS") c.WARP_ROWS_GROUPS = i();
    else if (k == "WARP_ROWS_CHUNKS") c.WARP_ROWS_CHUNKS = i();
    else if (k == "MFMA_KSPLIT") c.MFMA_KSPLIT = i();
    else if (k == "NM_MFMA") c.NM_MFMA = b();
    else if (k == "MFMA_KS") c.MFMA_KS = b();
    else if (k == "MFMA_BM") c.MFMA_BM = b();
    else if (k == "NM_KS") c.NM_KS = b();
    else if (k == "MFMA_FLAGS") c.MFMA_FLAGS = b();
    else if (k == "NM_SPLIT") c.NM_SPLIT = i();
    else if (k == "BM_SPLIT") c.BM_SPLIT = i();
    else if (k == "BM_WAVES") c.BM_WAVES = i();
    else if (k == "BM_V2") c.BM_V2 = b();
    else if (k == "BM_KB") c.BM_KB = b();
    else if (k == "KS_MIN_ROWS") c.KS_MIN_ROWS = i();
    else if (k == "KS_SPLIT") c.KS_SPLIT = i();
    else if (k == "KS_WAVES") c.KS_WAVES = i();
    else if (k == "KS_PRIO") c.KS_PRIO = i();
    else if (k == "KS_FORCE_TIMEOUT") c.KS_FORCE_TIMEOUT = i();
    else if (k == "KS_APART") c.KS_APART = i();
    else if (k == "NM_V4") c.NM_V4 = i();
    else if (k == "KS_POS8") c.KS_POS8 = i();
    else if (k == "KS_NT") c.KS_NT = i();
    else if (k == "NM_KROT") c.NM_KROT = i();
    else if (k == "NM_TILES") c.NM_TILES = i();
    else if (k == "LDS_KSPLIT") c.LDS_KSPLIT = i();
    else if (k == "LDS_DMA") c.LDS_DMA = i();
    else if (k == "MP_COL_PARTS") c.MP_COL_PARTS = i();
    else if (k == "MP_HUB_COLS") c.MP_HUB_COLS = i();
    else if (k == "KS_PERSIST") c.KS_PERSIST = i();
    else if (k == "KS_HEAD") c.KS_HEAD = i();
    else if (k == "NM_NT") c.NM_NT = i();
    else if (k == "MP_ROWS") c.MP_ROWS = b();
    else if (k == "MP_SOLO") c.MP_SOLO = i();
    else if (k == "MP_COL_PERM") c.MP_COL_PERM = i();
    else if (k == "MP_PERM_HOT") c.MP_PERM_HOT = i();
    else if (k == "MP_PERM_SCATTER") c.MP_PERM_SCATTER = i();
}

void load_json(config_t &c, const std::string &path) {
    std::ifstream in(path);
    if (!in) return;
    std::stringstream ss;
    ss << in.rdbuf();
    std::string s = ss.str();
    size_t p = 0;
    while (true) {
        size_t q0 = s.find('"', p);
        if (q0 == std::string::npos) break;
        size_t q1 = s.find('"', q0 + 1);
        if (q1 == std::string::npos) break;
        std::string key = s.substr(q0 + 1, q1 - q0 - 1);
        size_t colon = s.find(':', q1);
        if (colon == std::string::npos) break;
        size_t v0 = s.find_first_not_of(" \t\r\n", colon + 1);
        if (v0 == std::string::npos) break;
        std::string val;
        if (s[v0] == '"') {
            size_t v1 = s.find('"', v0 + 1);
            val = s.substr(v0 + 1, v1 - v0 - 1);
            p = v1 + 1;
        } else {
            size_t v1 = s.find_first_of(",}\n", v0);
            val = s.substr(v0, v1 - v0);
            while (!val.empty() && isspace((unsigned char)val.back())) val.pop_back();
            p = v1;
        }
#ifndef GS_EXPERIMENTS
        if (refused_in_release(key, std::atoi(val.c_str()), val == "true"))
            throw gs_error(key + " in " + path + " selects an experiments-build kernel", -2);
#endif
        apply_kv(c, key, val);
    }
}

void ensure_loaded() {
    if (g_cfg_loaded) return;
    g_cfg = config_t();
    const char *env = std::getenv("GS_CONFIG");
    load_json(g_cfg, env ? env : "global_config.json");
    g_cfg_loaded = true;
}
}

config_t get_config() {
    std::lock_guard<std::mutex> l(g_cfg_mu);
    ensure_loaded();
    return g_cfg;
}

void set_config(const std::string &key, int64_t value) {
#ifndef GS_EXPERIMENTS
    if (refused_in_release(key, value, false))
        throw gs_error(key + " selects an experiments-build kernel (make -C generalsparse_amd/csrc exp)", -2);
#endif
    std::lock_guard<std::mutex> l(g_cfg_mu);
    ensure_loaded();
    apply_kv(g_cfg, key, std::to_string(value));
}

int64_t get_config_int(const std::string &k) {
#ifdef GS_EXPERIMENTS
    if (k == "GS_EXPERIMENTS") return 1;
#else
    if (k == "GS_EXPERIMENTS") return 0;
#endif
    const config_t c = get_config();
#define GS_KEY(name) \
    if (k == #name) return (int64_t)c.name;
    GS_KEY(DENSE_MATRIX_SIZE) GS_KEY(VECTOR_WIDTH) GS_KEY(HALF) GS_KEY(OPERATOR_RUNTIME_CHECK)
    GS_KEY(PADDING_RATE_UP_BOUND) GS_KEY(DATA_TYPE_COMPRESS) GS_KEY(BRANCH_COMPRESS_MAX_SIZE) GS_KEY(FLOAT_RATE)
    GS_KEY(SHARED_MEM_TOTAL_SIZE) GS_KEY(MAX_DIV_TIMES_OF_DIV) GS_KEY(MFMA_GLDS) GS_KEY(MFMA_COMPUTE_WAVES)
    GS_KEY(MFMA_GLDS_NBUF) GS_KEY(MODEL_DRIVEN_COMPRESS) GS_KEY(LDS_STAGE_B) GS_KEY(MFMA_TILES) GS_KEY(MFMA_KROT)
    GS_KEY(WARP_ROWS_GROUPS) GS_KEY(WARP_ROWS_CHUNKS) GS_KEY(MFMA_MAX_FILL) GS_KEY(NM_MFMA) GS_KEY(MFMA_KSPLIT) GS_KEY(MFMA_KS)
    GS_KEY(NM_KS) GS_KEY(NM_SPLIT) GS_KEY(MFMA_FLAGS) GS_KEY(MFMA_BM) GS_KEY(BM_SPLIT) GS_KEY(BM_WAVES) GS_KEY(BM_V2) GS_KEY(BM_KB) GS_KEY(KS_MIN_ROWS) GS_KEY(KS_SPLIT) GS_KEY(KS_WAVES) GS_KEY(KS_PRIO) GS_KEY(KS_FORCE_TIMEOUT) GS_KEY(KS_APART) GS_KEY(NM_V4) GS_KEY(KS_POS8) GS_KEY(KS_NT) GS_KEY(NM_KROT) GS_KEY(NM_TILES) GS_KEY(LDS_KSPLIT) GS_KEY(LDS_DMA) GS_KEY(MP_COL_PARTS) GS_KEY(MP_HUB_COLS) GS_KEY(KS_PERSIST) GS_KEY(KS_HEAD) GS_KEY(NM_NT) GS_KEY(MP_ROWS) GS_KEY(MP_SOLO) GS_KEY(MP_COL_PERM) GS_KEY(MP_PERM_HOT) GS_KEY(MP_PERM_SCATTER)
#undef GS_KEY
    throw gs_error("get_config_int: no integer key " + k);
}

void set_config_str(const std::string &key, const std::string &value) {
    std::lock_guard<std::mutex> l(g_cfg_mu);
    ensure_loaded();
    apply_kv(g_cfg, key, value);
}

void reset_config() {
    std::lock_guard<std::mutex> l(g_cfg_mu);
    g_cfg_loaded = false;
}

universal_array::universal_array(std::vector<uint64_t> v, data_type t)
    : type_(t), is_float_(false), u_(std::move(v)) {}

universal_array::universal_array(std::vector<double> v, data_type t) : type_(t), is_float_(true), f_(std::move(v)) {
    GS_CHECK(t == FLOAT || t == DOUBLE, "float array type");
}

uint64_t universal_array::max_integer() const {
    uint64_t m = 0;
    for (uint64_t x : u_) m = std::max(m, x);
    return m;
}

data_type universal_array::get_compress_data_type() const {
    if (is_float_) return type_;
    if (!get_config().DATA_TYPE_COMPRESS) return type_;
    return find_most_suitable_data_type(max_integer());
}

void universal_array::output_2_file(const std::string &path) const {
    FILE *f = std::fopen(path.c_str(), "w");
    GS_CHECK(f, "cannot write " + path);
    std::vector<char> buf(1 << 20);
    std::setvbuf(f, buf.data(), _IOFBF, buf.size());
    if (is_float_) {
        for (double x : f_) {
            std::fprintf(f, "%.6g\n", std::fabs(x) <= 1e-10 ? 0.0 : x);
        }
    } else {
        for (uint64_t x : u_) std::fprintf(f, "%llu\n", (unsigned long long)x);
    }
    std::fclose(f);
}

void meta_data_set::add_element(POS_TYPE pos, const std::string &name, int sub, std::shared_ptr<universal_array> arr,
                                bool constant) {
    std::string key = get_metadata_item_name(pos, name, sub);
    GS_CHECK(data_map.count(key) == 0, "meta_data_set::add_element: key exists: " + key);
// ... 218 lines not shown
```

### generalsparse_amd/csrc/host/gs_core.hpp

```cpp
#pragma once

#include <cstdint>
#include <map>
#include <memory>
#include <mutex>
#include <stdexcept>
#include <string>
#include <vector>

namespace gs {

enum data_type {
    CHAR, UNSIGNED_CHAR, CHAR2, CHAR4, CHAR8,
    SHORT, UNSIGNED_SHORT, SHORT2, SHORT4, SHORT8,
    INT, UNSIGNED_INT, INT2, INT4, NONE_DATA_TYPE_1,
    LONG, UNSIGNED_LONG, LONG2, NONE_DATA_TYPE_2, NONE_DATA_TYPE_3,
    LONG_LONG, UNSIGNED_LONG_LONG,
    HALF, HALF2, HALF4, HALF8,
    FLOAT, FLOAT2, FLOAT4, NONE_DATA_TYPE_4,
    DOUBLE, DOUBLE2, NONE_DATA_TYPE_5, NONE_DATA_TYPE_6,
    BOOL, NONE_DATA_TYPE,
};

std::string code_of_data_type(data_type t);
// ... 14 lines not shown
struct config_t {
    int64_t DENSE_MATRIX_SIZE = 8;
    int64_t VECTOR_WIDTH = 8;
    bool HALF = true;
    std::string PRECISE_OF_FLOAT = "float";
    std::string ROOT_PATH_STR = ".";
    std::string DATA_SET = "";
    bool OPERATOR_RUNTIME_CHECK = true;
    int64_t PADDING_RATE_UP_BOUND = 4;
    bool DATA_TYPE_COMPRESS = true;
    int64_t BRANCH_COMPRESS_MAX_SIZE = 5;
    int64_t FLOAT_RATE = 2;
    double GFLOPS_UP_BOUND = 10000;
    int64_t SHARED_MEM_TOTAL_SIZE = 160 * 1024;
    int64_t MAX_DIV_TIMES_OF_DIV = 12;
    int64_t MFMA_GLDS = 1;
    int64_t MFMA_COMPUTE_WAVES = 6;
    int64_t MFMA_GLDS_NBUF = 3;
    std::string FORMAT_OF_MTX = "COO";
    std::string PERFORMANCE_FLAG = "throughput";
    std::string Graph_Algorithm = "";
    bool MODEL_DRIVEN_COMPRESS = false;
    bool LDS_STAGE_B = true;
    bool MFMA_TILES = true;
    int64_t MFMA_KROT = 0;
    int64_t WARP_ROWS_CHUNKS = 3;
    int64_t WARP_ROWS_GROUPS = 1;
    int64_t MFMA_MAX_FILL = 16;
    bool NM_MFMA = true;
    int64_t MFMA_KSPLIT = 0;
    bool MFMA_FLAGS = false;
    bool NM_KS = false;
    int64_t NM_SPLIT = 0;
    bool MFMA_BM = false;
    int64_t BM_SPLIT = 0;
    int64_t BM_WAVES = 8;
    bool BM_KB = false;
    bool BM_V2 = false;
    bool MFMA_KS = true;
    int64_t KS_MIN_ROWS = 40;
    bool MP_ROWS = false;
    int64_t MP_COL_PERM = -1;
    int64_t MP_PERM_SCATTER = 0;
    int64_t MP_PERM_HOT = 0;
    int64_t MP_SOLO = 16;
    int64_t KS_WAVES = 8;
    int64_t KS_SPLIT = 0;
    int64_t NM_V4 = 0;
    int64_t KS_POS8 = 0;
    int64_t KS_APART = 1;
    int64_t KS_FORCE_TIMEOUT = 0;
    int64_t KS_PRIO = 1;
    int64_t KS_NT = 0;
    int64_t KS_HEAD = 1;
    int64_t KS_PERSIST = 0;
    int64_t MP_HUB_COLS = 0;
    int64_t MP_COL_PARTS = 0;
    int64_t LDS_DMA = 1;
    int64_t LDS_KSPLIT = 0;
    int64_t NM_TILES = 0;
    int64_t NM_KROT = 1;
    int64_t NM_NT = 1;
};
config_t get_config();
void set_config(const std::string &key, int64_t value);
int64_t get_config_int(const std::string &key);
void set_config_str(const std::string &key, const std::string &value);
void reset_config();

class universal_array {
  public:
    universal_array(std::vector<uint64_t> v, data_type t = UNSIGNED_LONG);
    universal_array(std::vector<double> v, data_type t);
    uint64_t get_len() const { return is_float_ ? f_.size() : u_.size(); }
    data_type get_data_type() const { return type_; }
    bool is_float() const { return is_float_; }
    uint64_t read_integer_from_arr(uint64_t i) const { return u_[i]; }
    double read_float_from_arr(uint64_t i) const { return is_float_ ? f_[i] : (double)u_[i]; }
    const std::vector<uint64_t> &u() const { return u_; }
    const std::vector<double> &f() const { return f_; }
    std::vector<uint64_t> &u_mut() { return u_; }
    data_type get_compress_data_type() const;
    uint64_t max_integer() const;
    void output_2_file(const std::string &path) const;
    bool check() const { return true; }

  private:
    data_type type_;
    bool is_float_;
    std::vector<uint64_t> u_;
    std::vector<double> f_;
};

struct meta_data_item {
    std::shared_ptr<universal_array> meta_data_arr;
    POS_TYPE meta_position;
    std::string name;
    int sub_matrix_id;
    bool is_constant;
    std::shared_ptr<universal_array> get_metadata_arr() const { return meta_data_arr; }
};

class meta_data_set {
  public:
    std::string matrix_name;
    void add_element(POS_TYPE pos, const std::string &name, int sub, std::shared_ptr<universal_array> arr,
// ... 45 lines not shown
```

### generalsparse_amd/csrc/host/gs_plan.hpp

```cpp
#pragma once

#include "operator.hpp"
#include "device_layout.hpp"
#include "../hip_code/idx_formula.hpp"

#include <hip/hip_runtime.h>

namespace gs {

struct device_arrays {
    void *col = nullptr, *val = nullptr;
    void *pad_out = nullptr;
    void *tcol = nullptr, *tval = nullptr;
    uint32_t *t0 = nullptr, *t1 = nullptr, *t2 = nullptr, *t3 = nullptr, *t4 = nullptr;
    uint32_t *a0 = nullptr, *a1 = nullptr, *a2 = nullptr, *a3 = nullptr, *a4 = nullptr;
    uint64_t *m0 = nullptr;
    float *ws = nullptr;
    float *ws2 = nullptr;
    uint32_t *cperm = nullptr;
    void *bperm = nullptr;
    std::vector<void *> pp;
};
enum { MP_PART_COL, MP_PART_VAL, MP_PART_WZ, MP_PART_WQ, MP_PART_ENDS, MP_PART_RID, MP_PART_EMPTY, MP_PART_WS,
       MP_PART_WS2, MP_PART_T0, MP_PART_CHAIN, MP_PART_CNT, MP_PART_OUT, kMpPartPtrs };

struct device_plan {
    int device = 0;
    int dtype = 1;
    int col_bytes = 2;
    int scf = 4;
    bool needs_memset = false;
    uint64_t n_out_rows = 0;
    uint64_t pad_rows = 0;
    uint32_t pad_N = 0;
    uint64_t out_lo = 0;
    uint64_t n_units = 0;
    uint64_t n_rows_aux = 0;
    uint64_t row_base = 0;
    uint32_t ks_ctw = 0;
    bool ks_ap = true;
    bool ks_p8 = false;
    uint32_t ks_gh = 0;
    uint32_t ks_nt = 0;
    uint32_t ks_persist = 0;
    bool nm_nt = false;
    uint32_t nm_tiles = 8;
    bool lds_dma = false;
    uint32_t mp_parts = 0;
    std::vector<uint32_t> mp_part_W, mp_part_rows, mp_part_fin;
    uint64_t err_at = 0;
    uint64_t nnz_stored = 0;
    size_t bytes_A = 0;
    bool lds = false;
    bool nm_ks = false;
    bool nm = false;
    bool nm4 = false;
    bool mfma = false;
    bool ks = false;
    uint32_t ks_ns = 0, ks_gcap = 0;
    bool bmkb = false;
    bool bm2 = false;
    bool bm = false;

    bool mp_rows = false;
    uint32_t mp_solo = 16;
    bool col_perm = false;
    bool perm_scatter = false;
    int mfma_glds = 2, mfma_nbg = 3, mfma_wct = 6, mfma_maxa = 1;
    bool mfma_flags = false;
    std::string kernel;
    uint32_t ksplit = 1, ncs = 0;
    uint32_t ws_n = 0;
    uint64_t n_fin = 0;
    uint32_t span = 0;
    uint32_t bmw_rows_max = 0;
    double mean_row_nnz = 0.0;
    uint32_t ilv = 0;
    uint32_t lds_N = 0, KC = 0, nc = 0, RSB = 0, rpw_max = 0, seg_cap = 0, waves = 0, maxr = 0;
    size_t lds_bytes = 0, bytes_tile = 0;
    gsk::idx_formula f0, f1;
    int index_formulas = 0;
    uint64_t index_bytes_saved = 0;
    std::vector<device_arrays> replicas;
    std::vector<void *> allocations;
};

struct plan_state {
    std::shared_ptr<meta_data_set> meta;
    std::shared_ptr<code_generator> cg;
    std::shared_ptr<operator_executer> exec;
    std::string pipeline;
    uint64_t M = 0, K = 0, nnz = 0;
    device_plan dev;
    bool uploaded = false;
// ... 47 lines not shown
```

### generalsparse_amd/csrc/kernels/device_plan.hip

```cpp
#include "../hip_code/parts.hpp"
#include "../hip_code/host_layouts.hpp"
#include "../host/gs_plan.hpp"
#include "../host/index_compress.hpp"
#include "../host/device_layout.hpp"

#include <algorithm>
#include <cstdlib>
#include <cstring>
#include <map>
#include <mutex>

namespace gs {

#define HIP_OK(x)                                                                                   \
    do {                                                                                            \
        hipError_t e_ = (x);                                                                        \
        if (e_ != hipSuccess) throw gs_error(std::string(#x) + ": " + hipGetErrorString(e_), -3); \
    } while (0)

namespace {

constexpr uint64_t kPad = 64;

template <class T>
// ... 481 lines not shown
            const uint64_t ngr = (mc.nm_rows + 255) / 256 * 4;
            a.ws = dev_copy(d, std::vector<float>((size_t)ngr * mc.nm_split * 64 * mc.N, 0.f));
            a.t2 = dev_copy(d, std::vector<uint32_t>((size_t)ngr, 0u));
        }
        if (mc.nm4 && mc.nm_split > 1) {
            const uint64_t nb = (mc.nm_rows + 255) / 256;
            a.ws = dev_copy(d, std::vector<float>((size_t)nb * mc.nm_split * 256 * mc.N, 0.f));
            a.t2 = dev_copy(d, std::vector<uint32_t>((size_t)nb + 1u, 0u));
            d.err_at = nb;
        }
        d.replicas.push_back(a);
        p.uploaded = true;
        return;
    }
    uint64_t maxc = 0;
    for (uint64_t c : col) maxc = std::max(maxc, c);
    d.col_bytes = maxc <= 0xffff ? 2 : 4;
    const bool defer_csr = dtype != kF32 && get_config().MFMA_TILES &&
                           (sp.family == KF_WARP_TOTAL || sp.family == KF_BLOCK_TOTAL) &&
                           m.is_exist(TBLOCK_META, "first_row_indices", sb);
    if (sp.family == KF_MERGE_PATH) {
        const config_t cfg = get_config();
        const uint64_t b_bytes = p.K * (uint64_t)std::max<int64_t>(1, cfg.DENSE_MATRIX_SIZE) * elem_bytes(dtype);
        d.col_perm = !sp.interleaved && p.K < (1ull << 32) &&
                     (cfg.MP_COL_PERM > 0 || (cfg.MP_COL_PERM < 0 && b_bytes >= (64ull << 20)));
        const int64_t Nd = std::max<int64_t>(1, cfg.DENSE_MATRIX_SIZE);
        if (d.col_perm && dtype == 0 && sb == 0 && !pidx && cfg.MP_COL_PARTS > 1 && Nd <= 32 && p.K >= 64 * (uint64_t)cfg.MP_COL_PARTS)
            d.mp_parts = (uint32_t)std::min<int64_t>(cfg.MP_COL_PARTS, 8);
    }
    if (!defer_csr) upload_csr(p, a);
    GS_CHECK(!d.col_perm || (a.cperm && a.bperm), "merge-path column permutation: arrays not uploaded");
    uint64_t row_num = row_num_of_sub_matrix(m, sb);
    auto try_mfma = [&](const std::vector<uint32_t> &) {
        if (mc.kind == mc_layout::KS) {
            const ks_tiles &kt = mc.ks;
            d.mfma = true;
            d.ks = true;
            d.kernel = "k_mfma_ks";
            d.lds_N = mc.N;
            d.ksplit = kt.S;
            d.ks_ns = kt.NS;
            d.maxr = kt.RT;
            d.rpw_max = kt.RMAX;
            d.seg_cap = kt.MAXG;
            d.waves = kt.W;
            d.lds_bytes = kt.lds_bytes;
            const uint64_t nb = mc.tbr.size() - 1;
            d.n_rows_aux = nb;
            const size_t before = d.bytes_A;
            d.ks_gcap = kt.GCAP;
            d.ks_ctw = kt.CT;
            d.ks_ap = kt.AP;
            d.ks_p8 = kt.P8;
            d.ks_nt = kt.NT;
            d.ks_gh = kt.GH;
            d.ks_persist = (uint32_t)std::max<int64_t>(0, get_config().KS_PERSIST);
            if (d.ks_persist) a.t3 = dev_copy(d, std::vector<uint32_t>(9, 0u));
            a.t0 = dev_copy(d, to_u32(mc.tbr, "BMTB first_row_indices"));
            a.tcol = kt.P8 ? (void *)dev_copy(d, kt.pos8) : (void *)dev_copy(d, kt.pos);
            a.tval = dev_copy(d, kt.val);
            a.t1 = dev_copy(d, kt.steps);
            d.bytes_tile = d.bytes_A - before;
            if (kt.S > 1) {
                const uint32_t CT = kt.CT, nt = ks_col_tiles_ct(mc.N, CT);
                a.ws = dev_copy(d, std::vector<float>((size_t)nb * kt.S * nt * 256 * kt.RT * CT, 0.f));
                a.t2 = dev_copy(d, std::vector<uint32_t>((size_t)nb * nt + 1u, 0u));
                d.err_at = (uint64_t)nb * nt;
            }
            return true;
        }
        if (mc.kind == mc_layout::BM) {
            const bm_tiles &bt = mc.bm;
            d.mfma = true;
            d.bm = true;
            d.bm2 = bt.v2;
            d.bmkb = bt.kb;
            d.seg_cap = bt.NVB;
            d.kernel = bt.kb ? "k_mfma_kb" : bt.v2 ? "k_mfma_bm2" : "k_mfma_bm";
            d.lds_N = mc.N;
            d.ksplit = bt.S;
            d.ks_ns = bt.NS;
            d.maxr = bt.RT;
            d.rpw_max = bt.RMAX;
            d.waves = bt.W;
            d.lds_bytes = bt.lds_bytes;
            const uint64_t nb = mc.tbr.size() - 1;
            d.n_rows_aux = nb;
            const size_t before = d.bytes_A;
            a.t0 = dev_copy(d, to_u32(mc.tbr, "BMTB first_row_indices"));
            a.tcol = dev_copy(d, bt.rec);
            a.t1 = dev_copy(d, bt.sbase);
            a.tval = dev_copy(d, bt.val);
            d.bytes_tile = d.bytes_A - before;
            if (bt.S > 1) {
                const uint32_t nt = ks_col_tiles(mc.N), CT = ks_ct(mc.N);
                a.ws = dev_copy(d, std::vector<float>((size_t)nb * bt.S * nt * 256 * bt.RT * CT, 0.f));
                a.t2 = dev_copy(d, std::vector<uint32_t>((size_t)nb * nt * (bt.v2 ? bt.RT : 1u) + 1u, 0u));
                if (bt.kb) d.err_at = (uint64_t)nb * nt;
            }
            return true;
        }
        if (mc.kind != mc_layout::ROWS) return false;
        const mfma_tiles &t = mc.rows;
        d.mfma = true;
        d.kernel = "k_mfma_rows";
        d.lds_N = mc.N;
        d.KC = 1u << t.lgKC; d.nc = t.nc; d.maxr = t.RT; d.rpw_max = t.RMAX; d.RSB = t.lgKC;
        d.seg_cap = t.gmax;
        d.mfma_glds = mc.rows_glds; d.mfma_nbg = mc.rows_nbg; d.mfma_wct = mc.rows_wct; d.mfma_maxa = mc.rows_maxa;
        d.mfma_flags = mc.rows_flags;
        const uint64_t nb = mc.tbr.size() - 1;
        d.ncs = mc.rows_ncs;
// ... 257 lines not shown
        }
        default:
            throw gs_error("no gfx950 kernel family for this plan");
    }
    if (defer_csr && !d.mfma) upload_csr(p, a);
    const uint64_t prows = row_num_of_sub_matrix(m, sb);
    if (sb == 0 && !pidx && prows > p.M) {
        d.pad_rows = prows;
        d.pad_N = (uint32_t)std::max<int64_t>(1, get_config().DENSE_MATRIX_SIZE);
        a.pad_out = dev_copy(d, std::vector<uint32_t>((prows * d.pad_N * elem_bytes(dtype) + 3) / 4, 0u));
    }
    d.replicas.push_back(a);
    p.uploaded = true;
}

void ensure_csr(plan_state &p) {
    bool need = false;
    for (device_arrays &a : p.dev.replicas) need |= !a.col;
    if (!need) return;
    int prev = 0;
    HIP_OK(hipGetDevice(&prev));
    for (device_arrays &a : p.dev.replicas)
        if (!a.col) upload_csr(p, a);
    HIP_OK(hipSetDevice(prev));
}

void add_replica(plan_state &p) {
    GS_CHECK(p.uploaded, "upload the plan before adding replicas");
    HIP_OK(hipSetDevice(p.dev.device));
    const device_arrays &s = p.dev.replicas[0];
    device_arrays r = s;
    size_t n0 = p.dev.allocations.size();
    std::vector<void *> base(p.dev.allocations.begin(), p.dev.allocations.begin() + n0);
    auto dup = [&](void *src) -> void * {
        if (!src) return nullptr;
        size_t bytes = 0;
        HIP_OK(hipMemPtrGetInfo(src, &bytes));
        void *dst = nullptr;
        HIP_OK(hipMalloc(&dst, bytes));
        HIP_OK(hipMemcpy(dst, src, bytes, hipMemcpyDeviceToDevice));
        p.dev.allocations.push_back(dst);
        return dst;
    };
    r.col = s.pp.empty() ? dup(s.col) : nullptr;
    r.val = s.pp.empty() ? dup(s.val) : nullptr;
    r.a0 = (uint32_t *)dup(s.a0);
    r.a1 = (uint32_t *)dup(s.a1);
    r.a2 = (uint32_t *)dup(s.a2);
    r.a3 = (uint32_t *)dup(s.a3);
    r.a4 = (uint32_t *)dup(s.a4);
    r.m0 = (uint64_t *)dup(s.m0);
    r.tcol = dup(s.tcol);
    r.tval = dup(s.tval);
    r.t0 = (uint32_t *)dup(s.t0);
    r.t1 = (uint32_t *)dup(s.t1);
    r.t2 = (uint32_t *)dup(s.t2);
    r.t3 = (uint32_t *)dup(s.t3);
    r.t4 = (uint32_t *)dup(s.t4);
    r.ws = (float *)dup(s.ws);
    r.ws2 = (float *)dup(s.ws2);
    r.cperm = (uint32_t *)dup(s.cperm);
    r.bperm = dup(s.bperm);
    r.pad_out = dup(s.pad_out);
    for (size_t i = 0; i < s.pp.size(); i++) r.pp[i] = dup(s.pp[i]);
    if (!s.pp.empty()) {
        r.col = r.pp[MP_PART_COL];
        r.val = r.pp[MP_PART_VAL];
    }
    p.dev.replicas.push_back(r);
}

void memset_rows(void *C, uint64_t lo, uint64_t hi, uint32_t N, size_t e, hipStream_t stream) {
    HIP_OK(hipMemsetAsync((char *)C + lo * N * e, 0, (hi - lo) * N * e, stream));
}

void combine_parts(const void *const *parts, const uint32_t *rows, uint32_t n, void *C, uint64_t row0, uint64_t P,
                   uint32_t N, int dtype, hipStream_t stream) {
    GS_CHECK(P * N < (1ull << 40) && n > 0, "combine_parts: bad sizes");
    const uint64_t total = P * N;
    const uint32_t blocks = (uint32_t)std::min<uint64_t>((total + 255) / 256, 4096);
    if (blocks == 0) return;
    if (dtype == kF32)
        hipLaunchKernelGGL(gsk::k_combine_parts<float>, dim3(blocks), dim3(256), 0, stream,
                           (const float *const *)parts, rows, n, (float *)C + row0 * N, total, N);
    else if (dtype == kBF16)
        hipLaunchKernelGGL(gsk::k_combine_parts<gsk::bf16>, dim3(blocks), dim3(256), 0, stream,
                           (const gsk::bf16 *const *)parts, rows, n, (gsk::bf16 *)C + row0 * N, total, N);
    else
        hipLaunchKernelGGL(gsk::k_combine_parts<gsk::f16>, dim3(blocks), dim3(256), 0, stream,
                           (const gsk::f16 *const *)parts, rows, n, (gsk::f16 *)C + row0 * N, total, N);
    HIP_OK(hipGetLastError());
}

void free_device(plan_state &p) {
    if (!p.dev.allocations.empty()) (void)hipSetDevice(p.dev.device);
    for (void *x : p.dev.allocations) (void)hipFree(x);
    p.dev.allocations.clear();
    p.dev.replicas.clear();
    p.uploaded = false;
}

static void launch_body(plan_state &p, int replica, const void *B, void *C, uint32_t N, hipStream_t stream) {
    GS_CHECK(p.dev.dtype != kBF16 || (!p.dev.nm && !p.dev.lds && (!p.dev.mfma || p.dev.ks)),
             "bf16 plans run k_mfma_ks or a gather family: the other matrix-core and LDS kernels are fp16 / fp32 kernels");
    if (p.dev.nm) {
        launch_nm(p, p.dev.replicas[replica], B, C, N, stream);
// ... 35 lines not shown
```

### generalsparse_amd/csrc/kernels/ks_launch.hip

```cpp
#include "../hip_code/mfma_ks.hpp"
#ifdef GS_EXPERIMENTS
#include "../hip_code/mfma_bm_exp.hpp"
#endif
#include "../host/gs_plan.hpp"

#include <cstring>
#include <map>
#include <mutex>

namespace gs {

#define HIP_OK(x)                                                                                   \
    do {                                                                                            \
        hipError_t e_ = (x);                                                                        \
        if (e_ != hipSuccess) throw gs_error(std::string(#x) + ": " + hipGetErrorString(e_), -3); \
    } while (0)

namespace {

uint32_t ks_prio_arg() {
    const config_t c = get_config();
    return (uint32_t)(c.KS_PRIO & 3) | (c.KS_FORCE_TIMEOUT ? 16u : 0u);
}

template <class KERN>
void grant_lds(int device, KERN kern, size_t bytes) {
    static std::mutex mu;
    static std::map<std::pair<int, const void *>, size_t> granted;
    std::lock_guard<std::mutex> l(mu);
    size_t &g = granted[{device, reinterpret_cast<const void *>(kern)}];
    if (g < bytes) {
        HIP_OK(hipFuncSetAttribute(reinterpret_cast<const void *>(kern), hipFuncAttributeMaxDynamicSharedMemorySize,
                                   (int)bytes));
        g = bytes;
    }
}

template <int CT, int RT, int MAXG, bool STAMPS = false, int W = (int)kKsWaves, class ET = gsk::f16>
void launch_ks_k(const plan_state &p, const device_arrays &a, const ET *B, ET *C, uint32_t N, hipStream_t s,
                 uint64_t *stamps = nullptr) {
    const device_plan &d = p.dev;
    constexpr bool F16 = std::is_same<ET, gsk::f16>::value;
    if constexpr (!F16) {
        static_assert(W == (int)kKsWaves && !STAMPS, "bf16: the release instantiations only");
        GS_CHECK(d.waves == kKsWaves && !d.ks_p8 && d.ks_ap && !d.ks_persist,
                 "k_mfma_ks at bf16 is built for 8 waves, 16-bit positions and the apart LDS layout: the experiments "
                 "variants (KS_WAVES, KS_POS8, KS_APART = 0, KS_PERSIST) are fp16 kernels");
    }
#ifdef GS_EXPERIMENTS
    if constexpr (F16 && W == (int)kKsWaves && !STAMPS) {
        if (d.waves == 16) {
            launch_ks_k<CT, RT, MAXG, false, 16>(p, a, B, C, N, s, stamps);
            return;
        }
        if constexpr (CT == 2 && RT <= 5) {
            if (d.waves == 12) {
                launch_ks_k<CT, RT, MAXG, false, 12>(p, a, B, C, N, s, stamps);
                return;
            }
        }
    }
    if constexpr (F16 && W == (int)kKsWaves && !STAMPS && CT == 2 &&
                  ((RT == 3 && MAXG == 1) || (RT == 4 && MAXG == 2) || (RT == 5 && MAXG <= 2) || (RT == 7 && MAXG == 3))) {
        static const int dep = getenv("GS_KS_DEPTH") ? atoi(getenv("GS_KS_DEPTH")) : 0;
        if (dep == 1 || dep == 3 || dep == 4) {
            auto kd = dep == 1 ? gsk::k_mfma_ks<CT, RT, W, 1, MAXG, false>
                               : dep == 3 ? gsk::k_mfma_ks<CT, RT, W, 3, MAXG, false> : gsk::k_mfma_ks<CT, RT, W, 4, MAXG, false>;
            grant_lds(d.device, kd, d.lds_bytes);
            hipLaunchKernelGGL(kd, dim3((uint32_t)d.n_rows_aux * d.ksplit, ks_col_tiles_ct(N, CT)), dim3(64 * W), d.lds_bytes, s,
                               a.t0, (const gsk::u32x4 *)a.tcol, (const gsk::u32x4 *)a.tval, (const gsk::u32x2 *)a.t1, B, C,
                               (uint32_t)p.K, N, d.ksplit, d.ks_ns, (uint32_t)d.n_rows_aux * d.ksplit, (uint32_t)d.row_base,
                               a.ws, a.t2, stamps, ks_prio_arg());
            HIP_OK(hipGetLastError());
            return;
        }
    }
    if constexpr (F16 && W == (int)kKsWaves && !STAMPS) {
        if (d.waves == 4) {
            if constexpr (CT == 2) {
                GS_CHECK(!d.ks_ap, "k_mfma_ks with 4 waves runs the overlapped LDS layout");
                auto k4 = d.ks_p8 ? gsk::k_mfma_ks<CT, RT, 4, (int)kKsDepth, MAXG, false, false, true>
                                  : gsk::k_mfma_ks<CT, RT, 4, (int)kKsDepth, MAXG, false, false, false>;
                GS_CHECK(gsk::ks_lds_bytes(CT, RT, 4, false) <= d.lds_bytes, "k_mfma_ks: LDS size disagrees with the upload");
                grant_lds(d.device, k4, d.lds_bytes);
                hipLaunchKernelGGL(k4, dim3((uint32_t)d.n_rows_aux * d.ksplit, ks_col_tiles_ct(N, CT)), dim3(256), d.lds_bytes,
                                   s, a.t0, (const gsk::u32x4 *)a.tcol, (const gsk::u32x4 *)a.tval, (const gsk::u32x2 *)a.t1, B,
                                   C, (uint32_t)p.K, N, d.ksplit, d.ks_ns, (uint32_t)d.n_rows_aux * d.ksplit,
                                   (uint32_t)d.row_base, a.ws, a.t2, stamps, ks_prio_arg() | (d.ks_gh << 8));
                HIP_OK(hipGetLastError());
                return;
            } else {
                throw gs_error("k_mfma_ks with 4 waves is built for N = 32");
            }
        }
    }
#else
    GS_CHECK(d.waves == kKsWaves && !d.ks_p8 && d.ks_ap,
             "k_mfma_ks with 4 or 16 waves, 8-bit positions or the overlapped LDS layout: experiments build");
#endif
    auto kern = gsk::k_mfma_ks<CT, RT, W, (int)kKsDepth, MAXG, STAMPS, true, false, 0, ET>;
    if (d.ks_nt) {
        if constexpr ((CT == 2 || CT == 8) && (W == (int)kKsWaves || W == 12) && !STAMPS) {
            GS_CHECK(d.ks_ap && !d.ks_p8, "k_mfma_ks: non-temporal loads are built for the apart layout, 16-bit positions");
            GS_CHECK(d.ks_nt == 1, "k_mfma_ks: KS_NT is built for A's groups (1)");
            kern = gsk::k_mfma_ks<CT, RT, W, (int)kKsDepth, MAXG, false, true, false, 1, ET>;
        } else {
            throw gs_error("k_mfma_ks: non-temporal loads are built for N = 32 and 128-column tiles, 8 waves");
        }
    }
#ifdef GS_EXPERIMENTS
    if (d.ks_p8) {
        if constexpr (F16 && CT == 2 && W == (int)kKsWaves && !STAMPS) {
            GS_CHECK(d.ks_ap, "k_mfma_ks: 8-bit positions are built with the apart LDS layout");
            kern = gsk::k_mfma_ks<CT, RT, W, (int)kKsDepth, MAXG, false, true, true>;
        } else {
            throw gs_error("k_mfma_ks: 8-bit positions are built for N = 32, 8 waves");
        }
    }
    if (!d.ks_ap) {
        if constexpr (F16 && CT == 2 && RT <= 5 && MAXG <= 2 && W == (int)kKsWaves)
            kern = gsk::k_mfma_ks<CT, RT, W, (int)kKsDepth, MAXG, STAMPS, false>;
        else
            throw gs_error("k_mfma_ks: the overlapped-LDS layout is built for N = 32, RT <= 5, MAXG <= 2");
    }
#endif
#ifdef GS_EXPERIMENTS
    if (d.ks_persist) {
        if constexpr (F16 && W == (int)kKsWaves && !STAMPS && (CT == 2 || CT == 8)) {
            GS_CHECK(d.ks_ap && !d.ks_p8 && a.t3 && ks_col_tiles_ct(N, CT) == 1, "k_mfma_ks_persist: 8 waves, apart layout, one column tile");
            auto kp = d.ks_nt ? gsk::k_mfma_ks_persist<CT, RT, W, (int)kKsDepth, MAXG, 1>
                              : gsk::k_mfma_ks_persist<CT, RT, W, (int)kKsDepth, MAXG, 0>;
            grant_lds(d.device, kp, d.lds_bytes);
            const uint32_t nunits = (uint32_t)d.n_rows_aux * d.ksplit;
            hipLaunchKernelGGL(kp, dim3(std::min(d.ks_persist, nunits)), dim3(64 * W), d.lds_bytes, s, a.t0,
                               (const gsk::u32x4 *)a.tcol, (const gsk::u32x4 *)a.tval, (const gsk::u32x2 *)a.t1, B, C,
                               (uint32_t)p.K, N, d.ksplit, d.ks_ns, nunits, (uint32_t)d.row_base, a.ws, a.t2,
                               ks_prio_arg() | (d.ks_gh << 8), a.t3);
            HIP_OK(hipGetLastError());
            return;
        } else {
            throw gs_error("k_mfma_ks_persist is built for N = 32 and 128-column tiles, 8 waves");
        }
    }
#else
    GS_CHECK(!d.ks_persist, "k_mfma_ks_persist is an experiments-build kernel");
#endif
    GS_CHECK(gsk::ks_lds_bytes(CT, RT, W, d.ks_ap) <= d.lds_bytes, "k_mfma_ks: LDS size disagrees with the upload");
    grant_lds(d.device, kern, d.lds_bytes);
    hipLaunchKernelGGL(kern, dim3((uint32_t)d.n_rows_aux * d.ksplit, ks_col_tiles_ct(N, CT)), dim3(64 * W), d.lds_bytes, s, a.t0,
                       (const gsk::u32x4 *)a.tcol, (const gsk::u32x4 *)a.tval, (const gsk::u32x2 *)a.t1, B, C,
                       (uint32_t)p.K, N, d.ksplit, d.ks_ns, (uint32_t)d.n_rows_aux * d.ksplit, (uint32_t)d.row_base, a.ws, a.t2, stamps,
                       ks_prio_arg() | (d.ks_gh << 8));
    HIP_OK(hipGetLastError());
}

template <int CT, int RT, class ET>
void launch_ks_rt(const plan_state &p, const device_arrays &a, const ET *B, ET *C, uint32_t N, hipStream_t s) {
    if constexpr (CT == 8) {
        GS_CHECK(ks_ct8_fits(RT, p.dev.seg_cap), "k_mfma_ks: 128-column tile instantiation not built for this plan");
        if constexpr (RT == 2) {
            switch (p.dev.seg_cap) {
                case 1: launch_ks_k<CT, RT, 1, false, (int)kKsWaves, ET>(p, a, B, C, N, s); break;
                case 2: launch_ks_k<CT, RT, 2, false, (int)kKsWaves, ET>(p, a, B, C, N, s); break;
                default: launch_ks_k<CT, RT, 3, false, (int)kKsWaves, ET>(p, a, B, C, N, s); break;
            }
        } else {
            launch_ks_k<CT, RT, 1, false, (int)kKsWaves, ET>(p, a, B, C, N, s);
        }
    } else {
        switch (p.dev.seg_cap) {
            case 1: launch_ks_k<CT, RT, 1, false, (int)kKsWaves, ET>(p, a, B, C, N, s); break;
            case 2: launch_ks_k<CT, RT, 2, false, (int)kKsWaves, ET>(p, a, B, C, N, s); break;
            case 3: launch_ks_k<CT, RT, 3, false, (int)kKsWaves, ET>(p, a, B, C, N, s); break;
            default: launch_ks_k<CT, RT, 4, false, (int)kKsWaves, ET>(p, a, B, C, N, s); break;
        }
    }
}

template <int CT, class ET>
void launch_ks_ct(const plan_state &p, const device_arrays &a, const ET *B, ET *C, uint32_t N, hipStream_t s) {
    if constexpr (CT == 8) {
        switch (p.dev.maxr) {
            case 2: launch_ks_rt<CT, 2, ET>(p, a, B, C, N, s); return;
            case 3: launch_ks_rt<CT, 3, ET>(p, a, B, C, N, s); return;
            default: throw gs_error("k_mfma_ks: 128-column tiles take row blocks of up to 48 rows");
        }
    } else {
        switch (p.dev.maxr) {
            case 2: launch_ks_rt<CT, 2, ET>(p, a, B, C, N, s); break;
            case 3: launch_ks_rt<CT, 3, ET>(p, a, B, C, N, s); break;
            case 4: launch_ks_rt<CT, 4, ET>(p, a, B, C, N, s); break;
            case 5: launch_ks_rt<CT, 5, ET>(p, a, B, C, N, s); break;
            case 6: if constexpr (CT <= 2) { launch_ks_rt<CT, 6, ET>(p, a, B, C, N, s); break; } [[fallthrough]];
            case 7: if constexpr (CT <= 2) { launch_ks_rt<CT, 7, ET>(p, a, B, C, N, s); break; } [[fallthrough]];
            case 8: if constexpr (CT <= 2) { launch_ks_rt<CT, 8, ET>(p, a, B, C, N, s); break; } [[fallthrough]];
            default: throw gs_error("k_mfma_ks: row tiles outside 2..8 (6..8 for N <= 32)");
        }
    }
}

#ifdef GS_EXPERIMENTS
template <int CT, int RT, int W, bool STAMPS = false>
void launch_bm_k(const plan_state &p, const device_arrays &a, const gsk::f16 *B, gsk::f16 *C, uint32_t N, hipStream_t s,
                 uint64_t *stamps = nullptr) {
    const device_plan &d = p.dev;
// ... 54 lines not shown
}

template <int CT>
void launch_bm_ct(const plan_state &p, const device_arrays &a, const gsk::f16 *B, gsk::f16 *C, uint32_t N, hipStream_t s) {
    switch (p.dev.maxr) {
        case 1: launch_bm_rt<CT, 1>(p, a, B, C, N, s); break;
        case 2: launch_bm_rt<CT, 2>(p, a, B, C, N, s); break;
        case 3: launch_bm_rt<CT, 3>(p, a, B, C, N, s); break;
        case 4: launch_bm_rt<CT, 4>(p, a, B, C, N, s); break;
        case 5: launch_bm_rt<CT, 5>(p, a, B, C, N, s); break;
        case 6: launch_bm_rt<CT, 6>(p, a, B, C, N, s); break;
        default: throw gs_error("k_mfma_bm: row tiles outside 1..6");
    }
}

#endif

}

#ifndef GS_KS_BF16_OBJECT
#ifdef GS_EXPERIMENTS
void launch_bm(const plan_state &p, const device_arrays &a, const void *B, void *C, uint32_t N, hipStream_t s) {
    const gsk::f16 *b = (const gsk::f16 *)B;
    gsk::f16 *c = (gsk::f16 *)C;
    GS_CHECK(N == p.dev.lds_N, "k_mfma_bm runs the plan's dense width");
    switch (ks_ct(N)) {
        case 1: launch_bm_ct<1>(p, a, b, c, N, s); break;
        case 2: launch_bm_ct<2>(p, a, b, c, N, s); break;
        default: launch_bm_ct<4>(p, a, b, c, N, s); break;
    }
}

#else
void launch_bm(const plan_state &, const device_arrays &, const void *, void *, uint32_t, hipStream_t) {
    throw gs_error("k_mfma_bm is an experiments-build kernel (make -C generalsparse_amd/csrc exp)", -2);
}
#endif
#endif

namespace {
template <int RT, int MAXG, int W = (int)kKsWaves, class ET = gsk::f16>
void launch_ks_group_k(const std::vector<ks_group_item> &it, uint32_t N, hipStream_t s) {
    constexpr bool AP = W == (int)kKsWaves;
    constexpr bool F16 = std::is_same<ET, gsk::f16>::value;
    if constexpr (!F16)
        GS_CHECK(it[0].p->dev.waves == kKsWaves && !it[0].p->dev.ks_p8, "k_mfma_ks_group at bf16: 8 waves, 16-bit positions");
#ifdef GS_EXPERIMENTS
    if constexpr (F16 && W == (int)kKsWaves) {
        if (it[0].p->dev.waves == 4) {
            launch_ks_group_k<RT, MAXG, 4>(it, N, s);
            return;
        }
    }
    auto kern = gsk::k_mfma_ks_group<2, RT, W, (int)kKsDepth, MAXG, false, AP, 0, ET>;
    if constexpr (F16) {
        if (it[0].p->dev.ks_p8) kern = gsk::k_mfma_ks_group<2, RT, W, (int)kKsDepth, MAXG, true, AP>;
    }
#else
    GS_CHECK(!it[0].p->dev.ks_p8, "k_mfma_ks_group: 8-bit positions are an experiments-build layout");
    auto kern = gsk::k_mfma_ks_group<2, RT, W, (int)kKsDepth, MAXG, false, AP, 0, ET>;
#endif
    if constexpr (AP) {
        if (it[0].p->dev.ks_nt) kern = gsk::k_mfma_ks_group<2, RT, W, (int)kKsDepth, MAXG, false, true, 1, ET>;
    }
    GS_CHECK(!it.empty() && it.size() <= (size_t)gsk::kKsGroupMax, "k_mfma_ks_group: 1..32 entries");
    gsk::ks_group_args args;
    std::memset(&args, 0, sizeof(args));
    size_t lds = 0;
    uint32_t wg = 0;
    for (size_t i = 0; i < it.size(); i++) {
        const plan_state &p = *it[i].p;
        const device_plan &d = p.dev;
        const device_arrays &a = d.replicas[(size_t)it[i].replica];
        GS_CHECK(gsk::ks_lds_bytes(2, RT, W, AP) <= d.lds_bytes, "k_mfma_ks_group: LDS size disagrees with the upload");
        lds = std::max(lds, d.lds_bytes);
        gsk::ks_entry &e = args.e[i];
        e.tbr = a.t0;
        e.tP = (const gsk::u32x4 *)a.tcol;
        e.tV = (const gsk::u32x4 *)a.tval;
        e.steps = (const gsk::u32x2 *)a.t1;
        e.B = it[i].B;
        e.C = it[i].C;
        e.slabs = a.ws;
        e.arrivals = a.t2;
        e.K = (uint32_t)p.K;
        e.S = d.ksplit;
        e.NS = d.ks_ns;
        e.nwg = (uint32_t)d.n_rows_aux * d.ksplit;
        e.row_base = (uint32_t)d.row_base;
        e.pad0 = d.ks_gh;
        args.begin[i] = wg;
        wg += (e.nwg + 7u) & ~7u;
    }
    args.begin[it.size()] = wg;
    args.n = (uint32_t)it.size();
    args.N = N;
    args.pad[0] = ks_prio_arg();
    grant_lds(it[0].p->dev.device, kern, lds);
    hipLaunchKernelGGL(kern, dim3(wg, ks_col_tiles(N)), dim3(64 * W), lds, s, args);
    HIP_OK(hipGetLastError());
}

template <int RT, class ET>
void launch_ks_group_rt(const std::vector<ks_group_item> &it, uint32_t N, hipStream_t s) {
    switch (it[0].p->dev.seg_cap) {
        case 1: launch_ks_group_k<RT, 1, (int)kKsWaves, ET>(it, N, s); break;
        case 2: launch_ks_group_k<RT, 2, (int)kKsWaves, ET>(it, N, s); break;
        case 3: launch_ks_group_k<RT, 3, (int)kKsWaves, ET>(it, N, s); break;
        default: launch_ks_group_k<RT, 4, (int)kKsWaves, ET>(it, N, s); break;
    }
}
template <class ET>
void launch_ks_group_et(const std::vector<ks_group_item> &it, uint32_t N, hipStream_t s) {
    switch (it[0].p->dev.maxr) {
        case 2: launch_ks_group_rt<2, ET>(it, N, s); break;
        case 3: launch_ks_group_rt<3, ET>(it, N, s); break;
        case 4: launch_ks_group_rt<4, ET>(it, N, s); break;
        case 5: launch_ks_group_rt<5, ET>(it, N, s); break;
        case 6: launch_ks_group_rt<6, ET>(it, N, s); break;
        case 7: launch_ks_group_rt<7, ET>(it, N, s); break;
        case 8: launch_ks_group_rt<8, ET>(it, N, s); break;
        default: throw gs_error("k_mfma_ks_group: row tiles outside 2..8");
    }
}
template <class ET>
void launch_ks_et(const plan_state &p, const device_arrays &a, const void *B, void *C, uint32_t N, hipStream_t s) {
    const ET *b = (const ET *)B;
    ET *c = (ET *)C;
    switch (p.dev.ks_ctw) {
        case 1: launch_ks_ct<1, ET>(p, a, b, c, N, s); break;
        case 2: launch_ks_ct<2, ET>(p, a, b, c, N, s); break;
        case 4: launch_ks_ct<4, ET>(p, a, b, c, N, s); break;
        case 8: launch_ks_ct<8, ET>(p, a, b, c, N, s); break;
        default: throw gs_error("k_mfma_ks: bad column tile count");
    }
}
}

#ifdef GS_KS_BF16_OBJECT
void launch_ks_bf16(const plan_state &p, const device_arrays &a, const void *B, void *C, uint32_t N, hipStream_t s) {
    launch_ks_et<gsk::bf16>(p, a, B, C, N, s);
}
void launch_ks_group_bf16(const std::vector<ks_group_item> &it, uint32_t N, hipStream_t s) {
    launch_ks_group_et<gsk::bf16>(it, N, s);
}
#else
void launch_ks_bf16(const plan_state &p, const device_arrays &a, const void *B, void *C, uint32_t N, hipStream_t s);
void launch_ks_group_bf16(const std::vector<ks_group_item> &it, uint32_t N, hipStream_t s);

uint32_t ks_group_key(const plan_state &p, uint32_t N) {
    const device_plan &d = p.dev;
    const bool w8 = d.waves == kKsWaves && d.ks_ap, w4 = d.waves == 4 && !d.ks_ap;
    if (!p.uploaded || !d.mfma || !d.ks || d.pad_rows || N != 32 || d.lds_N != 32 || !(w8 || w4) || d.ks_persist) return 0;
    if (d.dtype == kBF16 && (d.ks_p8 || !w8)) return 0;
#ifndef GS_EXPERIMENTS
    if (d.ks_p8 || !w8) return 0;
#endif
    return (d.dtype == kBF16 ? 1u << 20 : 0u) | (d.ks_nt << 18) | (w4 ? 1u << 17 : 0u) | (d.ks_p8 ? 1u << 16 : 0u) | (d.maxr << 8) |
           d.seg_cap;
}

void launch_ks_group(const std::vector<ks_group_item> &it, uint32_t N, hipStream_t s) {
    GS_CHECK(!it.empty(), "empty group");
    const uint32_t key = ks_group_key(*it[0].p, N);
    GS_CHECK(key != 0, "k_mfma_ks_group: not a groupable k_mfma_ks plan");
    for (const auto &x : it) GS_CHECK(ks_group_key(*x.p, N) == key, "k_mfma_ks_group: entries of different instantiations");
    if (it[0].p->dev.dtype == kBF16) launch_ks_group_bf16(it, N, s);
    else launch_ks_group_et<gsk::f16>(it, N, s);
}

void launch_ks(const plan_state &p, const device_arrays &a, const void *B, void *C, uint32_t N, hipStream_t s) {
    GS_CHECK(N == p.dev.lds_N, "k_mfma_ks runs the plan's dense width");
    GS_CHECK(p.dev.ks_ctw == ks_ct_rt(N, p.dev.maxr) || (p.dev.ks_ctw == 4 && ks_ct_rt(N, p.dev.maxr) == 8 &&
                                                         !ks_ct8_fits(p.dev.maxr, p.dev.seg_cap)),
             "k_mfma_ks: column tiles disagree with the upload");
    if (p.dev.dtype == kBF16) launch_ks_bf16(p, a, B, C, N, s);
    else launch_ks_et<gsk::f16>(p, a, B, C, N, s);
}

#ifdef GS_EXPERIMENTS
void debug_bm_timeline(const plan_state &p, const void *B, void *C, uint32_t N, hipStream_t s, uint64_t *host,
                       size_t n_host) {
    const device_plan &d = p.dev;
    GS_CHECK(N == 32 && d.maxr == 5 && d.waves == 8, "k_mfma_bm timeline build: N=32, RT=5, 8 waves only");
    const size_t n = (size_t)d.n_rows_aux * d.ksplit * 8 * 16;
    uint64_t *dst = nullptr;
    HIP_OK(hipMalloc(&dst, n * 8));
    HIP_OK(hipMemsetAsync(dst, 0, n * 8, s));
    launch_bm_k<2, 5, 8, true>(p, d.replicas[0], (const gsk::f16 *)B, (gsk::f16 *)C, N, s, dst);
    HIP_OK(hipStreamSynchronize(s));
    HIP_OK(hipMemcpy(host, dst, std::min(n, n_host) * 8, hipMemcpyDeviceToHost));
    (void)hipFree(dst);
}

void debug_ks_timeline(const plan_state &p, const void *B, void *C, uint32_t N, hipStream_t s, uint64_t *host,
                       size_t n_host) {
    const device_plan &d = p.dev;
    GS_CHECK(N == 32 && d.maxr >= 2 && d.maxr <= 5 && d.seg_cap <= 2 && d.waves == kKsWaves && d.dtype == kF16,
             "k_mfma_ks timeline build: fp16, N=32, RT 2..5, MAXG <= 2, 8 waves only");
    const size_t n = (size_t)d.n_rows_aux * d.ksplit * ks_col_tiles(N) * kKsWaves * 32;
    uint64_t *dst = nullptr;
    HIP_OK(hipMalloc(&dst, n * 8));
    HIP_OK(hipMemsetAsync(dst, 0, n * 8, s));
    const device_arrays &a = d.replicas[0];
    const gsk::f16 *b = (const gsk::f16 *)B;
    gsk::f16 *c = (gsk::f16 *)C;
    const bool g1 = d.seg_cap == 1;
    switch (d.maxr) {
        case 2: g1 ? launch_ks_k<2, 2, 1, true>(p, a, b, c, N, s, dst) : launch_ks_k<2, 2, 2, true>(p, a, b, c, N, s, dst); break;
        case 3: g1 ? launch_ks_k<2, 3, 1, true>(p, a, b, c, N, s, dst) : launch_ks_k<2, 3, 2, true>(p, a, b, c, N, s, dst); break;
        case 4: g1 ? launch_ks_k<2, 4, 1, true>(p, a, b, c, N, s, dst) : launch_ks_k<2, 4, 2, true>(p, a, b, c, N, s, dst); break;
// ... 20 lines not shown
```

### include/generalsparse.h

```cpp
#ifndef GENERALSPARSE_H
#define GENERALSPARSE_H

#include <stdint.h>

#ifdef __cplusplus
extern "C" {
#endif

typedef struct gs_plan gs_plan_t;
typedef void *gs_stream_t;

enum { GS_OK = 0, GS_ERR = -1, GS_ERR_ARG = -2, GS_ERR_HIP = -3,
       GS_ERR_DEVICE = -4  };
enum { GS_F32 = 0, GS_F16 = 1, GS_BF16 = 2 };

typedef struct {
    const char *pipeline;
    int dtype;
    int dense_n;
    int p0, p1;
    int ones_values;
    int device;
} gs_opts;

typedef struct {
    uint64_t rows, cols, nnz;
    uint64_t nnz_stored;
    uint64_t n_units;
    uint64_t device_bytes_A;
    int family;
    int col_bytes, dtype , replicas, needs_memset;
    char kernel_name[64];
    int lds_stage;
    uint32_t lds_n, lds_kc, lds_chunks, lds_waves;
    uint64_t lds_bytes, tile_bytes;
    uint32_t ksplit;
    int n_kernels;
    char device_kernel[32];
    int index_formulas;
    uint64_t index_bytes_saved;
    uint32_t ks_nt;
    uint32_t ks_head_groups;
    uint32_t nm_tiles;
} gs_plan_info;

const char *gs_last_error(void);
const char *gs_version(void);

void gs_opts_default(gs_opts *o);

int gs_plan_create_from_mtx(const char *path, int ones_values, gs_plan_t **out);
int gs_plan_create_from_coo(uint64_t n_rows, uint64_t n_cols, uint64_t nnz, const uint64_t *row,
                            const uint64_t *col, const float *val, gs_plan_t **out);
int gs_set_config_int(const char *key, long long value);
int gs_get_config_int(const char *key, long long *value);

int gs_plan_add_operator(gs_plan_t *p, const char *op_name, const long long *args, int nargs);
int gs_plan_run_pipeline(gs_plan_t *p, const char *name, int dense_n, int p0, int p1);
int gs_plan_add_operator_sub(gs_plan_t *p, int sub, const char *op_name, const long long *args, int nargs);
int gs_plan_run_pipeline_sub(gs_plan_t *p, int sub, const char *name, int dense_n, int p0, int p1);
int gs_plan_sub_matrices(gs_plan_t *p, int *ids, int cap);
int gs_plan_compile(gs_plan_t *p);
int gs_plan_generate_program(gs_plan_t *p, const char *root_dir, int repeat, char *dir_out, int dir_out_len);

int gs_plan_upload(gs_plan_t *p, int dtype, int device);
int gs_convert_values(const float *in, uint64_t n, int dtype, void *out);
int gs_plan_add_replica(gs_plan_t *p);
int gs_spmm(gs_plan_t *p, const void *B, void *C, int N, gs_stream_t stream);
int gs_spmm_replica(gs_plan_t *p, int replica, const void *B, void *C, int N, gs_stream_t stream);
int gs_spmm_rotate(gs_plan_t *p, int count, int first, const void *const *B_ptrs, void *const *C_ptrs, int n_ptrs,
                   int N, gs_stream_t stream);
int gs_spmm_batch(gs_plan_t *const *plans, const int *replicas, const void *const *B, void *const *C, int n, int N,
                  gs_stream_t stream);

int gs_batch_launches(gs_plan_t *const *plans, const int *replicas, int n, int N, int *entries_per_launch, int cap);
int gs_plan_device_status(gs_plan_t *p, gs_stream_t stream);

int gs_plan_info_get(gs_plan_t *p, gs_plan_info *info);
int gs_plan_array_count(gs_plan_t *p);
int gs_plan_array_key(gs_plan_t *p, int i, char *buf, int buf_len);
long long gs_plan_array_len(gs_plan_t *p, const char *key);
int gs_plan_array_is_float(gs_plan_t *p, const char *key);
int gs_plan_array_read_u64(gs_plan_t *p, const char *key, uint64_t *out, uint64_t n);
int gs_plan_array_read_f64(gs_plan_t *p, const char *key, double *out, uint64_t n);
int gs_plan_log(gs_plan_t *p, char *buf, int buf_len);

int gs_plan_index_compression(gs_plan_t *p, const char *key, char *kind_out, int kind_len, char *expr_out,
                              int expr_len, int *exact);
int gs_index_compression_of_array(const uint64_t *a, uint64_t n, int type_ori, int branch_max, char *kind_out,
                                  int kind_len, uint64_t *params , int *exact);

int gs_debug_mfma_timeline(gs_plan_t *p, const void *B, void *C, int N, gs_stream_t stream, uint64_t *stamps,
                           uint64_t n_stamps);

int gs_plan_save(gs_plan_t *p, const char *path);
int gs_plan_load(const char *path, gs_plan_t **out);
// ... 12 lines not shown
```

Baseline: 39540.

## Add windowed 8-bit entry positions and a full-tile fast path to k_mfma_ks

Adds a new position format for the k-split MFMA kernel. Each group carries a one-byte window index plus 8-bit offsets within that window, in place of 16-bit positions, which cuts index bytes read from HBM and simplifies the LDS scatter address math. It also adds a fast path for full tiles that skips the per-element bounds checks and uses precomputed B offsets during the loop. The window format is opt-in through a KS_WPOS flag and restricted to fp16 with 8 waves, which adds template variants, a group-entry field and new host checks.

```diff
diff --git a/generalsparse_amd/_lib.py b/generalsparse_amd/_lib.py
--- a/generalsparse_amd/_lib.py
+++ b/generalsparse_amd/_lib.py
@@ -30,7 +30,7 @@
                 ("n_kernels", ctypes.c_int), ("device_kernel", ctypes.c_char * 32),
                 ("index_formulas", ctypes.c_int), ("index_bytes_saved", ctypes.c_uint64),
                 ("ks_nt", ctypes.c_uint32), ("ks_head_groups", ctypes.c_uint32),
-                ("nm_tiles", ctypes.c_uint32)]
+                ("nm_tiles", ctypes.c_uint32), ("ks_wpos", ctypes.c_uint32)]
 
 
 SIGNATURES = {
diff --git a/generalsparse_amd/csrc/hip_code/mfma_ks.hpp b/generalsparse_amd/csrc/hip_code/mfma_ks.hpp
--- a/generalsparse_amd/csrc/hip_code/mfma_ks.hpp
+++ b/generalsparse_amd/csrc/hip_code/mfma_ks.hpp
@@ -11,13 +11,18 @@
 }
 
 
-template <int CT, int RT, int W, int D, int MAXG, bool STAMPS, bool AP = true, bool P8 = false, int NTL = 0, class ET = f16>
+#ifndef GS_KS_FULL_TILE
+#define GS_KS_FULL_TILE 1
+#endif
+enum : int { kKsPosU16 = 0, kKsPos8 = 1, kKsPosWin = 2 };
+template <int CT, int RT, int W, int D, int MAXG, bool STAMPS, bool AP = true, int PF = kKsPosU16, int NTL = 0, class ET = f16>
 __device__ __forceinline__ void ks_body(const uint32_t *__restrict__ bmtb_first_row, const u32x4 *__restrict__ tP,
                                         const u32x4 *__restrict__ tV, const u32x2 *__restrict__ steps,
                                         const ET *__restrict__ B, ET *__restrict__ C, uint32_t K, uint32_t N, uint32_t S,
                                         uint32_t NS, uint32_t nwg, uint32_t row_base, float *__restrict__ slabs,
                                         uint32_t *__restrict__ arrivals, uint64_t *__restrict__ stamps, uint32_t bx,
-                                        uint32_t prio) {
+                                        uint32_t prio, const uint8_t *__restrict__ tW = nullptr) {
+    constexpr bool P8 = PF == kKsPos8, WP = PF == kKsPosWin;
     constexpr uint32_t RB = 32 * CT;
     constexpr uint32_t UB = 2 * CT;
     constexpr uint32_t IMG = ks_image_bytes<RT>();
@@ -40,10 +45,11 @@
 
     const uint32_t nsw = NS > wv ? (NS - wv + W - 1u) / W : 0u;
     const size_t ubase = (size_t)u * NS;
-    using PV = typename std::conditional<P8, u32x2, u32x4>::type;
+    using PV = typename std::conditional<P8 || WP, u32x2, u32x4>::type;
     const PV *tPp = reinterpret_cast<const PV *>(tP);
     PV P[D][MAXG];
     u32x4 V[D][MAXG], BR[D][CT];
+    uint32_t WN[D][MAXG];
     u32x2 NX[D];
     uint32_t CN[D];
     uint32_t vz;
@@ -52,9 +58,18 @@
         const uint32_t st = __builtin_amdgcn_readfirstlane(i < nsw ? wv + i * W : 0u);
         return steps[ubase + st + vz];
     };
-    auto load_b = [&](uint32_t i, u32x4 (&B_)[CT]) {
+    uint32_t boff[CT];
+#pragma unroll
+    for (int c = 0; c < CT; c++) boff[c] = ((lane + 64u * c) / UB) * N + ((lane + 64u * c) % UB) * 8u;
+    auto load_b = [&](auto fast, uint32_t i, u32x4 (&B_)[CT]) {
         const uint32_t st = __builtin_amdgcn_readfirstlane(i < nsw ? wv + i * W : 0u);
         const uint32_t kr = k0 + st * 32u;
+        if constexpr (decltype(fast)::value) {
+            const ET *Bk = B + (size_t)kr * N + col0;
+#pragma unroll
+            for (int c = 0; c < CT; c++) B_[c] = ld_once_if<(NTL & 2) != 0>(reinterpret_cast<const u32x4 *>(Bk + boff[c]));
+            return;
+        }
 #pragma unroll
         for (int c = 0; c < CT; c++) {
             const uint32_t un = lane + 64u * c;
@@ -64,7 +79,7 @@
         }
     };
     auto load_g_at = [&](uint32_t i, uint32_t b0, uint32_t gc, u32x2 &NX_, uint32_t &CN_, PV (&P_)[MAXG],
-                         u32x4 (&V_)[MAXG]) {
+                         u32x4 (&V_)[MAXG], uint32_t (&W_)[MAXG]) {
         CN_ = gc;
         NX_ = rec_of(i + D);
 #pragma unroll
@@ -73,29 +88,30 @@
             const size_t at = (size_t)b0 + (qg < gc ? qg : 0u);
             P_[j] = ld_once_if<(NTL & 1) != 0>(tPp + at);
             V_[j] = ld_once_if<(NTL & 1) != 0>(tV + at);
-        }
-    };
-    auto load_g = [&](uint32_t i, u32x2 &NX_, uint32_t &CN_, PV (&P_)[MAXG], u32x4 (&V_)[MAXG]) {
-        load_g_at(i, __builtin_amdgcn_readfirstlane(NX_[0]), __builtin_amdgcn_readfirstlane(NX_[1]), NX_, CN_, P_, V_);
+            if constexpr (WP) W_[j] = ld_once_if<(NTL & 1) != 0>(tW + at);
+        }
+    };
+    auto load_g = [&](uint32_t i, u32x2 &NX_, uint32_t &CN_, PV (&P_)[MAXG], u32x4 (&V_)[MAXG], uint32_t (&W_)[MAXG]) {
+        load_g_at(i, __builtin_amdgcn_readfirstlane(NX_[0]), __builtin_amdgcn_readfirstlane(NX_[1]), NX_, CN_, P_, V_, W_);
     };
     const uint32_t GH = (prio >> 8) & 0x3ffu;
     if (GH) {
 #pragma unroll
-        for (int d = 0; d < D; d++) load_b((uint32_t)d, BR[d]);
+        for (int d = 0; d < D; d++) load_b(std::false_type{}, (uint32_t)d, BR[d]);
 #pragma unroll
         for (int d = 0; d < D; d++) {
             const uint32_t st = (uint32_t)d < nsw ? wv + (uint32_t)d * W : 0u;
-            load_g_at((uint32_t)d, (u * min((uint32_t)(W * D), NS) + st) * GH, GH, NX[d], CN[d], P[d], V[d]);
+            load_g_at((uint32_t)d, (u * min((uint32_t)(W * D), NS) + st) * GH, GH, NX[d], CN[d], P[d], V[d], WN[d]);
         }
         for (uint32_t x = lane; x < IMG / 16u; x += 64u) *reinterpret_cast<u32x4 *>(img + x * 16u) = zero4;
     } else {
 #pragma unroll
         for (int d = 0; d < D; d++) NX[d] = rec_of((uint32_t)d);
 #pragma unroll
-        for (int d = 0; d < D; d++) load_b((uint32_t)d, BR[d]);
+        for (int d = 0; d < D; d++) load_b(std::false_type{}, (uint32_t)d, BR[d]);
         for (uint32_t x = lane; x < IMG / 16u; x += 64u) *reinterpret_cast<u32x4 *>(img + x * 16u) = zero4;
 #pragma unroll
-        for (int d = 0; d < D; d++) load_g((uint32_t)d, NX[d], CN[d], P[d], V[d]);
+        for (int d = 0; d < D; d++) load_g((uint32_t)d, NX[d], CN[d], P[d], V[d], WN[d]);
     }
     GS_KS_STAMP(1u);
 
@@ -125,7 +141,8 @@
             return 0u;
         }
     };
-    auto step = [&](uint32_t i, u32x2 &NX_, uint32_t &CN_, PV (&P_)[MAXG], u32x4 (&V_)[MAXG], u32x4 (&B_)[CT]) {
+    auto step = [&](auto fast, uint32_t i, u32x2 &NX_, uint32_t &CN_, PV (&P_)[MAXG], u32x4 (&V_)[MAXG], u32x4 (&B_)[CT],
+                    uint32_t (&W_)[MAXG]) {
         const bool live = i < nsw;
         const uint32_t gc = CN_;
         typedef typename mfma_elem<ET>::frag frag;
@@ -135,8 +152,18 @@
 #pragma unroll
             for (int c = 0; c < CT; c++) {
                 const uint32_t un = lane + 64u * c, k = un / UB, s = un % UB;
-                *reinterpret_cast<u32x4 *>(bst + k * RB + b_piece<CT>(k, s >> 1) * 32u + (s & 1u) * 16u) =
-                    kr + k < K && s * 8u < nv ? B_[c] : zero4;
+                u32x4 b = B_[c];
+                if constexpr (!decltype(fast)::value) b = kr + k < K && s * 8u < nv ? b : zero4;
+                *reinterpret_cast<u32x4 *>(bst + k * RB + b_piece<CT>(k, s >> 1) * 32u + (s & 1u) * 16u) = b;
+            }
+            unsigned char *wa[WP ? MAXG : 1][8];
+            if constexpr (WP) {
+#pragma unroll
+                for (int j = 0; j < MAXG; j++) {
+                    unsigned char *wb = img + W_[j] * 480u;
+#pragma unroll
+                    for (int e = 0; e < 8; e++) wa[j][e] = wb + 2u * ((P_[j][e >> 2] >> (8 * (e & 3))) & 0xffu);
+                }
             }
 #pragma unroll
             for (int j = 0; j < MAXG; j++) {
@@ -144,9 +171,13 @@
                     const uint32_t hb = grp_hb(P_[j]);
 #pragma unroll
                     for (int e = 0; e < 8; e++) {
-                        const uint32_t h = ent_h(P_[j], hb, e);
                         const uint16_t v = (uint16_t)((V_[j][e >> 1] >> (16 * (e & 1))) & 0xffffu);
-                        *reinterpret_cast<uint16_t *>(img + h * 2u) = v;
+                        if constexpr (WP) {
+                            *reinterpret_cast<uint16_t *>(wa[j][e]) = v;
+                        } else {
+                            const uint32_t h = ent_h(P_[j], hb, e);
+                            *reinterpret_cast<uint16_t *>(img + h * 2u) = v;
+                        }
                     }
                 }
             }
@@ -169,12 +200,15 @@
                 if (lane + 64u * j < gc) {
                     const uint32_t hb = grp_hb(P_[j]);
 #pragma unroll
-                    for (int e = 0; e < 8; e++) *reinterpret_cast<uint16_t *>(img + ent_h(P_[j], hb, e) * 2u) = (uint16_t)0;
+                    for (int e = 0; e < 8; e++) {
+                        if constexpr (WP) *reinterpret_cast<uint16_t *>(wa[j][e]) = (uint16_t)0;
+                        else *reinterpret_cast<uint16_t *>(img + ent_h(P_[j], hb, e) * 2u) = (uint16_t)0;
+                    }
                 }
             }
         }
-        load_b(i + D, B_);
-        load_g(i + D, NX_, CN_, P_, V_);
+        load_b(fast, i + D, B_);
+        load_g(i + D, NX_, CN_, P_, V_, W_);
         if (live) {
 #pragma unroll
             for (int rt = 0; rt < RT; rt++)
@@ -186,9 +220,21 @@
     };
     const bool young = wv >= W / 2u;
     if ((prio & 3u) && young) __builtin_amdgcn_s_setprio(1);
-    for (uint32_t i0 = 0; i0 < nsw; i0 += D) {
-#pragma unroll
-        for (int d = 0; d < D; d++) step(i0 + d, NX[d], CN[d], P[d], V[d], BR[d]);
+    const uint32_t fsp = min(NS, K > k0 ? (K - k0) / 32u : 0u);
+    const uint32_t nfull = fsp > wv ? (fsp - wv + W - 1u) / W : 0u;
+    uint32_t fast_end = 0;
+    if (GS_KS_FULL_TILE && nv == 16u * CT)
+        fast_end = fsp == NS ? nsw : (nfull >= 2u * D ? ((nfull - 2u * D) / D + 1u) * D : 0u);
+    fast_end = __builtin_amdgcn_readfirstlane(fast_end);
+    uint32_t i0 = 0;
+    for (; i0 < fast_end; i0 += D) {
+#pragma unroll
+        for (int d = 0; d < D; d++) step(std::true_type{}, i0 + d, NX[d], CN[d], P[d], V[d], BR[d], WN[d]);
+        if ((prio & 3u) == 2u && young && i0 + D >= nsw / 2u && i0 < nsw / 2u) __builtin_amdgcn_s_setprio(0);
+    }
+    for (; i0 < nsw; i0 += D) {
+#pragma unroll
+        for (int d = 0; d < D; d++) step(std::false_type{}, i0 + d, NX[d], CN[d], P[d], V[d], BR[d], WN[d]);
         if ((prio & 3u) == 2u && young && i0 + D >= nsw / 2u && i0 < nsw / 2u) __builtin_amdgcn_s_setprio(0);
     }
     if ((prio & 3u) && young) __builtin_amdgcn_s_setprio(0);
@@ -299,7 +345,7 @@
 #undef GS_KS_STAMP
 }
 
-template <int CT, int RT, int W, int D, int MAXG, bool STAMPS = false, bool AP = true, bool P8 = false, int NTL = 0, class ET = f16>
+template <int CT, int RT, int W, int D, int MAXG, bool STAMPS = false, bool AP = true, int PF = kKsPosU16, int NTL = 0, class ET = f16>
 __global__ __launch_bounds__(64 * W) void k_mfma_ks(const uint32_t *__restrict__ bmtb_first_row,
                                                     const u32x4 *__restrict__ tP,
                                                     const u32x4 *__restrict__ tV,
@@ -308,9 +354,10 @@
                                                     uint32_t N, uint32_t S, uint32_t NS, uint32_t nwg,
                                                     uint32_t row_base, float *__restrict__ slabs,
                                                     uint32_t *__restrict__ arrivals, uint64_t *__restrict__ stamps = nullptr,
-                                                    uint32_t prio = 0) {
-    ks_body<CT, RT, W, D, MAXG, STAMPS, AP, P8, NTL, ET>(bmtb_first_row, tP, tV, steps, B, C, K, N, S, NS, nwg, row_base, slabs,
-                                                    arrivals, stamps, blockIdx.x, prio);
+                                                    uint32_t prio = 0,
+                                                    const uint8_t *__restrict__ tW = nullptr) {
+    ks_body<CT, RT, W, D, MAXG, STAMPS, AP, PF, NTL, ET>(bmtb_first_row, tP, tV, steps, B, C, K, N, S, NS, nwg, row_base, slabs,
+                                                    arrivals, stamps, blockIdx.x, prio, tW);
 }
 
 #ifdef GS_EXPERIMENTS
@@ -331,7 +378,7 @@
     while (u < nunits) {
         uint32_t pulled = 0;
         if (threadIdx.x == 0) pulled = __hip_atomic_fetch_add(queue + qx, 1u, __ATOMIC_RELAXED, __HIP_MEMORY_SCOPE_AGENT);
-        ks_body<CT, RT, W, D, MAXG, false, true, false, NTL>(bmtb_first_row, tP, tV, steps, B, C, K, N, S, NS, nunits,
+        ks_body<CT, RT, W, D, MAXG, false, true, kKsPosU16, NTL>(bmtb_first_row, tP, tV, steps, B, C, K, N, S, NS, nunits,
                                                           row_base, slabs, arrivals, nullptr, u, prio);
         __syncthreads();
         if (threadIdx.x == 0) next_sh = pulled;
@@ -360,15 +407,17 @@
     void *C;
     float *slabs;
     uint32_t *arrivals;
-    uint32_t K, S, NS, nwg, row_base, pad0, pad1, pad2;
+    uint32_t K, S, NS, nwg, row_base, pad0;
+    const uint8_t *tW;
 };
+static_assert(sizeof(ks_entry) == 96, "ks_entry is 96 bytes");
 struct ks_group_args {
     uint32_t begin[kKsGroupMax + 1];
     uint32_t n, N, pad[2];
     ks_entry e[kKsGroupMax];
 };
 
-template <int CT, int RT, int W, int D, int MAXG, bool P8 = false, bool AP = true, int NTL = 0, class ET = f16>
+template <int CT, int RT, int W, int D, int MAXG, int PF = kKsPosU16, bool AP = true, int NTL = 0, class ET = f16>
 __global__ __launch_bounds__(64 * W) void k_mfma_ks_group(ks_group_args args) {
     const uint32_t bx = blockIdx.x, n = args.n;
     uint32_t sel = 0;
@@ -378,9 +427,9 @@
     sel = __builtin_amdgcn_readfirstlane(sel);
     const ks_entry &e = args.e[sel];
     if (bx - args.begin[sel] >= e.nwg) return;
-    ks_body<CT, RT, W, D, MAXG, false, AP, P8, NTL, ET>(e.tbr, e.tP, e.tV, e.steps, (const ET *)e.B, (ET *)e.C, e.K, args.N, e.S, e.NS,
+    ks_body<CT, RT, W, D, MAXG, false, AP, PF, NTL, ET>(e.tbr, e.tP, e.tV, e.steps, (const ET *)e.B, (ET *)e.C, e.K, args.N, e.S, e.NS,
                                                    e.nwg, e.row_base, e.slabs, e.arrivals, nullptr, bx - args.begin[sel],
-                                                   args.pad[0] | (e.pad0 << 8));
-}
-
-}
+                                                   args.pad[0] | (e.pad0 << 8), e.tW);
+}
+
+}
diff --git a/generalsparse_amd/csrc/host/capi.cc b/generalsparse_amd/csrc/host/capi.cc
--- a/generalsparse_amd/csrc/host/capi.cc
+++ b/generalsparse_amd/csrc/host/capi.cc
@@ -834,6 +834,7 @@
             info->index_bytes_saved = s.dev.index_bytes_saved;
             info->ks_nt = s.dev.ks ? s.dev.ks_nt : 0;
             info->ks_head_groups = s.dev.ks ? s.dev.ks_gh : 0;
+            info->ks_wpos = s.dev.ks && s.dev.ks_wp ? 1 : 0;
             info->nm_tiles = s.dev.nm ? s.dev.nm_tiles : 0;
         }
     });
diff --git a/generalsparse_amd/csrc/host/code_generator.cc b/generalsparse_amd/csrc/host/code_generator.cc
--- a/generalsparse_amd/csrc/host/code_generator.cc
+++ b/generalsparse_amd/csrc/host/code_generator.cc
@@ -228,8 +228,10 @@
         const uint64_t nb = L.tbr.size() - 1, nwg = nb * t.S;
         o << "    auto tbr = rd(\"TBLOCK_META_first_row_indices_0\");\n"
           << "    std::vector<uint32_t> t32(tbr.begin(), tbr.end()); uint32_t *d_tbr = up(t32);\n"
-          << (t.P8 ? "    uint8_t *d_pos = up(rdb<uint8_t>(\"TBLOCK_META_mfma_ks_entry_pos_0.bin\"));  // 8-bit positions\n"
-                   : "    uint16_t *d_pos = up(rdb<uint16_t>(\"TBLOCK_META_mfma_ks_entry_pos_0.bin\"));\n")
+          << (t.WP ? "    uint8_t *d_pos = up(rdb<uint8_t>(\"TBLOCK_META_mfma_ks_entry_pos_0.bin\"));  // positions inside the group's window\n"
+                     "    uint8_t *d_win = up(rdb<uint8_t>(\"TBLOCK_META_mfma_ks_group_win_0.bin\"));  // window byte per group\n"
+              : t.P8 ? "    uint8_t *d_pos = up(rdb<uint8_t>(\"TBLOCK_META_mfma_ks_entry_pos_0.bin\"));  // 8-bit positions\n"
+                     : "    uint16_t *d_pos = up(rdb<uint16_t>(\"TBLOCK_META_mfma_ks_entry_pos_0.bin\"));\n")
           << "    uint16_t *d_val = up(rdb<uint16_t>(\"TBLOCK_META_mfma_ks_entry_val_0.bin\"));\n"
           << "    uint32_t *d_steps = up(rdb<uint32_t>(\"TBLOCK_META_mfma_ks_steps_0.bin\"));\n"
           << "    // the tagged slabs start (and are left by every launch) all 0\n"
@@ -239,7 +241,8 @@
           << "ull + 4);\n";
         const std::string k = "gsk::k_mfma_ks<" + std::to_string(CT) + ", " + std::to_string(t.RT) + ", " +
                               std::to_string(t.W) + ", " + std::to_string(kKsDepth) + ", " + std::to_string(t.MAXG) +
-                              std::string(", false, ") + (t.AP ? "true" : "false") + ", " + (t.P8 ? "true" : "false") +
+                              std::string(", false, ") + (t.AP ? "true" : "false") + ", " +
+                              (t.WP ? "gsk::kKsPosWin" : t.P8 ? "true" : "false") +
                               (t.NT ? ", " + std::to_string(t.NT) + ">" : ">");
         setup = "hipFuncSetAttribute((const void *)" + k + ", hipFuncAttributeMaxDynamicSharedMemorySize, " +
                 std::to_string(t.lds_bytes) + ")";
@@ -247,7 +250,7 @@
                  std::to_string(64 * t.W) + ", " + std::to_string(t.lds_bytes) +
                  ">>>(d_tbr, (const gsk::u32x4 *)d_pos, (const gsk::u32x4 *)d_val, (const gsk::u32x2 *)d_steps, d_B, d_C, "
                  "(uint32_t)K, N, " + std::to_string(t.S) + "u, " + std::to_string(t.NS) + "u, " + std::to_string(nwg) + "u, 0u, d_ws, d_arr, nullptr, " +
-                 std::to_string((uint32_t)get_config().KS_PRIO | (t.GH << 8)) + "u)";
+                 std::to_string((uint32_t)get_config().KS_PRIO | (t.GH << 8)) + (t.WP ? "u, d_win)" : "u)");
     } else if (L.kind == mc_layout::BM) {
         const bm_tiles &t = L.bm;
         const uint64_t nb = L.tbr.size() - 1, nwg = nb * t.S;
@@ -578,7 +581,9 @@
     uint64_t id = meta->output_format_to_dir(root, spec.arrays, &dir);
     const mc_layout L = emitted_layout(*meta, spec, sub);
     if (L.kind == mc_layout::KS) {
-        if (L.ks.P8)
+        if (L.ks.WP)
+            write_bin(dir + "/TBLOCK_META_mfma_ks_group_win_0.bin", L.ks.win);
+        if (L.ks.P8 || L.ks.WP)
             write_bin(dir + "/TBLOCK_META_mfma_ks_entry_pos_0.bin", L.ks.pos8);
         else
             write_bin(dir + "/TBLOCK_META_mfma_ks_entry_pos_0.bin", L.ks.pos);
diff --git a/generalsparse_amd/csrc/host/device_layout.cc b/generalsparse_amd/csrc/host/device_layout.cc
--- a/generalsparse_amd/csrc/host/device_layout.cc
+++ b/generalsparse_amd/csrc/host/device_layout.cc
@@ -1,6 +1,7 @@
 #include "device_layout.hpp"
 
 #include <algorithm>
+#include <array>
 #include <cstring>
 
 namespace gs {
@@ -191,6 +192,61 @@
     return groups;
 }
 
+constexpr uint32_t kKsWinRows = 5;
+static size_t wpos_step(const std::vector<uint16_t> &row, const std::vector<uint16_t> &colw,
+                        const std::vector<uint16_t> &hv, uint32_t RS, std::vector<uint8_t> &out_pos8,
+                        std::vector<uint8_t> &out_win, std::vector<uint16_t> &out_val) {
+    const size_t n = row.size();
+    uint32_t nwin = 0;
+    for (size_t i = 0; i < n; i++) nwin = std::max<uint32_t>(nwin, row[i] / kKsWinRows + 1u);
+    std::vector<std::vector<uint32_t>> win(nwin);
+    for (uint32_t i = 0; i < n; i++) win[row[i] / kKsWinRows].push_back(i);
+    size_t groups = 0;
+    std::vector<std::array<uint32_t, 8>> used;
+    std::vector<std::vector<uint32_t>> bucket(32);
+    std::vector<uint32_t> slot;
+    for (uint32_t w = 0; w < nwin; w++) {
+        const auto &es = win[w];
+        if (es.empty()) continue;
+        GS_CHECK(w < 256, "KS_WPOS: window beyond 8 bits");
+        const size_t ng = (es.size() + 7) / 8;
+        for (auto &b : bucket) b.clear();
+        for (uint32_t i : es) bucket[((uint32_t)row[i] * RS + colw[i]) / 2 % 32].push_back(i);
+        used.resize((groups + ng + 31) / 32, std::array<uint32_t, 8>{});
+        slot.assign(ng * 8, UINT32_MAX);
+        size_t left = es.size();
+        for (int e = 0; e < 8 && left; e++)
+            for (size_t l = 0; l < ng && left; l++) {
+                uint32_t &mask = used[(groups + l) / 32][e];
+                int best = -1, any = -1;
+                for (int k = 0; k < 32; k++) {
+                    if (bucket[k].empty()) continue;
+                    if (any < 0 || bucket[k].size() > bucket[any].size()) any = k;
+                    if (!((mask >> k) & 1u) && (best < 0 || bucket[k].size() > bucket[best].size())) best = k;
+                }
+                const int k = best >= 0 ? best : any;
+                slot[l * 8 + e] = bucket[k].back();
+                bucket[k].pop_back();
+                mask |= 1u << k;
+                left--;
+            }
+        for (size_t gi = 0; gi < ng; gi++) {
+            const uint32_t first = slot[gi * 8];
+            GS_CHECK(first != UINT32_MAX, "KS_WPOS: a group without entries");
+            for (int e = 0; e < 8; e++) {
+                const uint32_t i = slot[gi * 8 + e] == UINT32_MAX ? first : slot[gi * 8 + e];
+                const uint32_t code = (row[i] % kKsWinRows) * RS + colw[i];
+                GS_CHECK(code < kKsWinRows * RS && kKsWinRows * RS <= 256, "KS_WPOS: position beyond its window");
+                out_pos8.push_back((uint8_t)code);
+                out_val.push_back(hv[i]);
+            }
+            out_win.push_back((uint8_t)w);
+        }
+        groups += ng;
+    }
+    return groups;
+}
+
 bool build_mfma_tiles(const std::vector<uint64_t> &tb_rows, const std::vector<uint32_t> &row_ptr,
                       const std::vector<uint64_t> &col, const std::vector<float> &vals, uint64_t K, uint32_t N,
                       size_t lds_budget, int64_t max_fill, mfma_tiles &t, std::string &why) {
@@ -300,10 +356,18 @@
     t.W = W;
     t.P8 = get_config().KS_POS8 && CT == 2 && (W == kKsWaves || W == 4);
     t.NT = (CT == 2 || CT == 8) && (W == kKsWaves || W == 12) && !t.P8 && t.AP && get_config().KS_NT ? 1u : 0u;
+    if (get_config().KS_WPOS && CT == 2) {
+        if (dtype != kF16) throw gs_error("KS_WPOS: window positions are an fp16 layout (bf16 plans take the u16 positions)", -2);
+        if (W != kKsWaves || !t.AP || t.P8 || get_config().KS_PERSIST > 0)
+            throw gs_error("KS_WPOS: window positions are built for 8 waves, the apart LDS layout and the static grid "
+                           "(not with KS_WAVES, KS_APART = 0, KS_POS8 or KS_PERSIST)", -2);
+        t.WP = true;
+    }
     uint64_t gmax = 1;
+    const uint32_t nwn = (16 * RT + kKsWinRows - 1) / kKsWinRows;
     {
-        const uint32_t nsg = 4 * RT;
-        std::vector<uint32_t> cnt((size_t)((K + 31) / 32) * (t.P8 ? nsg : 1u));
+        const uint32_t nsg = t.WP ? nwn : 4 * RT;
+        std::vector<uint32_t> cnt((size_t)((K + 31) / 32) * (t.P8 || t.WP ? nsg : 1u));
         for (uint64_t g = 0; g < nb; g++) {
             std::fill(cnt.begin(), cnt.end(), 0u);
             for (uint64_t r = tb_rows[g]; r < tb_rows[g + 1]; r++)
@@ -311,10 +375,12 @@
                     const uint64_t st = col[e] / 32;
                     if (t.P8)
                         cnt[st * nsg + ((r - tb_rows[g]) / 8) * 2 + (col[e] % 32) / 16]++;
+                    else if (t.WP)
+                        cnt[st * nsg + (r - tb_rows[g]) / kKsWinRows]++;
                     else
                         cnt[st]++;
                 }
-            if (t.P8) {
+            if (t.P8 || t.WP) {
                 for (size_t st = 0; st < cnt.size() / nsg; st++) {
                     uint64_t ngs = 0;
                     for (uint32_t k = 0; k < nsg; k++) ngs += (cnt[st * nsg + k] + 7) / 8;
@@ -350,13 +416,16 @@
     const uint32_t HS = std::min<uint32_t>(W * kKsDepth, t.NS);
     if (!t.P8 && get_config().KS_HEAD) {
         uint64_t gh = 1, head_groups = 0, all_groups = 0;
-        std::vector<uint32_t> c2((size_t)S * t.NS);
+        const uint32_t nsg = t.WP ? nwn : 1u;
+        std::vector<uint32_t> c2((size_t)S * t.NS * nsg);
         for (uint64_t g = 0; g < nb; g++) {
             std::fill(c2.begin(), c2.end(), 0u);
             for (uint64_t r = tb_rows[g]; r < tb_rows[g + 1]; r++)
-                for (uint64_t e = row_ptr[r]; e < row_ptr[r + 1]; e++) c2[col[e] / 32]++;
-            for (size_t st = 0; st < c2.size(); st++) {
-                const uint64_t ng = (c2[st] + 7) / 8;
+                for (uint64_t e = row_ptr[r]; e < row_ptr[r + 1]; e++)
+                    c2[col[e] / 32 * nsg + (t.WP ? (r - tb_rows[g]) / kKsWinRows : 0u)]++;
+            for (size_t st = 0; st < c2.size() / nsg; st++) {
+                uint64_t ng = 0;
+                for (uint32_t k = 0; k < nsg; k++) ng += (c2[st * nsg + k] + 7) / 8;
                 all_groups += ng;
                 if (st % t.NS < HS) {
                     head_groups += ng;
@@ -373,16 +442,23 @@
     }
     const uint32_t RS = gsk::kKsStride / 2;
     const uint32_t pad_h = 16 * RT * RS;
-    if (t.P8)
-        t.pos8.reserve(row_ptr[tb_rows[nb]] - row_ptr[tb_rows[0]] + (size_t)nb * S * t.NS * 8 * RT + 8);
+    const uint32_t zwin = 16 * RT / kKsWinRows, zcode = (16 * RT % kKsWinRows) * RS;
+    if (t.P8 || t.WP)
+        t.pos8.reserve(row_ptr[tb_rows[nb]] - row_ptr[tb_rows[0]] + (size_t)nb * S * t.NS * 8 * (t.WP ? nwn : RT) + 8);
     else
         t.pos.reserve(row_ptr[tb_rows[nb]] - row_ptr[tb_rows[0]] + (size_t)nb * S * t.NS * 8 + 8);
-    t.val.reserve(t.P8 ? t.pos8.capacity() : t.pos.capacity());
+    t.val.reserve(t.P8 || t.WP ? t.pos8.capacity() : t.pos.capacity());
     t.steps.reserve((size_t)nb * S * t.NS * 2);
-    if (t.GH) {
+    if (t.GH && t.WP) {
+        t.pos8.resize((size_t)nb * S * HS * t.GH * 8);
+        for (size_t i = 0; i < t.pos8.size(); i++) t.pos8[i] = (uint8_t)(zcode + 2 * (i % 8));
+        t.win.assign((size_t)nb * S * HS * t.GH, (uint8_t)zwin);
+        t.val.assign(t.pos8.size(), 0);
+    } else if (t.GH) {
         t.pos.assign((size_t)nb * S * HS * t.GH * 8, (uint16_t)pad_h);
         t.val.assign(t.pos.size(), 0);
     }
+    std::vector<uint8_t> hpos8, hwin;
     std::vector<uint64_t> cur;
     std::vector<uint16_t> pos, hv, prow, pcol, hpos, hval;
     for (uint64_t g = 0; g < nb; g++) {
@@ -407,7 +483,20 @@
                     cur[i] = e;
                 }
                 size_t before, ng;
-                if (t.GH && s < HS) {
+                if (t.WP && t.GH && s < HS) {
+                    hpos8.clear();
+                    hwin.clear();
+                    hval.clear();
+                    ng = wpos_step(prow, pcol, hv, RS, hpos8, hwin, hval);
+                    GS_CHECK(ng <= t.GH, "k_mfma_ks head step exceeds its slot");
+                    before = (((size_t)g * S + q) * HS + s) * t.GH * 8;
+                    std::copy(hpos8.begin(), hpos8.end(), t.pos8.begin() + before);
+                    std::copy(hwin.begin(), hwin.end(), t.win.begin() + before / 8);
+                    std::copy(hval.begin(), hval.end(), t.val.begin() + before);
+                } else if (t.WP) {
+                    before = t.pos8.size();
+                    ng = wpos_step(prow, pcol, hv, RS, t.pos8, t.win, t.val);
+                } else if (t.GH && s < HS) {
                     hpos.clear();
                     hval.clear();
                     bank_order_segment(pos, hv, pad_h, hpos, hval, RS / 2);
@@ -429,7 +518,10 @@
                 t.steps.push_back((uint32_t)ng);
             }
     }
-    if (t.P8)
+    if (t.WP) {
+        for (uint32_t e = 0; e < 8; e++) t.pos8.push_back((uint8_t)(zcode + 2 * e));
+        t.win.push_back((uint8_t)zwin);
+    } else if (t.P8)
         t.pos8.insert(t.pos8.end(), 8, (uint8_t)0);
     else
         t.pos.insert(t.pos.end(), 8, (uint16_t)pad_h);
diff --git a/generalsparse_amd/csrc/host/device_layout.hpp b/generalsparse_amd/csrc/host/device_layout.hpp
--- a/generalsparse_amd/csrc/host/device_layout.hpp
+++ b/generalsparse_amd/csrc/host/device_layout.hpp
@@ -47,11 +47,13 @@
     uint32_t CT = 0;
     bool AP = true;
     bool P8 = false;
+    bool WP = false;
     uint32_t NT = 0;
     uint32_t GH = 0;
     size_t lds_bytes = 0;
     std::vector<uint16_t> pos, val;
     std::vector<uint8_t> pos8;
+    std::vector<uint8_t> win;
     std::vector<uint32_t> steps;
 };
 
diff --git a/generalsparse_amd/csrc/host/gs_core.cc b/generalsparse_amd/csrc/host/gs_core.cc
--- a/generalsparse_amd/csrc/host/gs_core.cc
+++ b/generalsparse_amd/csrc/host/gs_core.cc
@@ -135,6 +135,7 @@
     else if (k == "NM_V4") c.NM_V4 = i();
     else if (k == "KS_POS8") c.KS_POS8 = i();
     else if (k == "KS_NT") c.KS_NT = i();
+    else if (k == "KS_WPOS") c.KS_WPOS = i();
     else if (k == "NM_KROT") c.NM_KROT = i();
     else if (k == "NM_TILES") c.NM_TILES = i();
     else if (k == "LDS_KSPLIT") c.LDS_KSPLIT = i();
@@ -226,7 +227,7 @@
     GS_KEY(SHARED_MEM_TOTAL_SIZE) GS_KEY(MAX_DIV_TIMES_OF_DIV) GS_KEY(MFMA_GLDS) GS_KEY(MFMA_COMPUTE_WAVES)
     GS_KEY(MFMA_GLDS_NBUF) GS_KEY(MODEL_DRIVEN_COMPRESS) GS_KEY(LDS_STAGE_B) GS_KEY(MFMA_TILES) GS_KEY(MFMA_KROT)
     GS_KEY(WARP_ROWS_GROUPS) GS_KEY(WARP_ROWS_CHUNKS) GS_KEY(MFMA_MAX_FILL) GS_KEY(NM_MFMA) GS_KEY(MFMA_KSPLIT) GS_KEY(MFMA_KS)
-    GS_KEY(NM_KS) GS_KEY(NM_SPLIT) GS_KEY(MFMA_FLAGS) GS_KEY(MFMA_BM) GS_KEY(BM_SPLIT) GS_KEY(BM_WAVES) GS_KEY(BM_V2) GS_KEY(BM_KB) GS_KEY(KS_MIN_ROWS) GS_KEY(KS_SPLIT) GS_KEY(KS_WAVES) GS_KEY(KS_PRIO) GS_KEY(KS_FORCE_TIMEOUT) GS_KEY(KS_APART) GS_KEY(NM_V4) GS_KEY(KS_POS8) GS_KEY(KS_NT) GS_KEY(NM_KROT) GS_KEY(NM_TILES) GS_KEY(LDS_KSPLIT) GS_KEY(LDS_DMA) GS_KEY(MP_COL_PARTS) GS_KEY(MP_HUB_COLS) GS_KEY(KS_PERSIST) GS_KEY(KS_HEAD) GS_KEY(NM_NT) GS_KEY(MP_ROWS) GS_KEY(MP_SOLO) GS_KEY(MP_COL_PERM) GS_KEY(MP_PERM_HOT) GS_KEY(MP_PERM_SCATTER)
+    GS_KEY(NM_KS) GS_KEY(NM_SPLIT) GS_KEY(MFMA_FLAGS) GS_KEY(MFMA_BM) GS_KEY(BM_SPLIT) GS_KEY(BM_WAVES) GS_KEY(BM_V2) GS_KEY(BM_KB) GS_KEY(KS_MIN_ROWS) GS_KEY(KS_SPLIT) GS_KEY(KS_WAVES) GS_KEY(KS_PRIO) GS_KEY(KS_FORCE_TIMEOUT) GS_KEY(KS_APART) GS_KEY(NM_V4) GS_KEY(KS_POS8) GS_KEY(KS_NT) GS_KEY(KS_WPOS) GS_KEY(NM_KROT) GS_KEY(NM_TILES) GS_KEY(LDS_KSPLIT) GS_KEY(LDS_DMA) GS_KEY(MP_COL_PARTS) GS_KEY(MP_HUB_COLS) GS_KEY(KS_PERSIST) GS_KEY(KS_HEAD) GS_KEY(NM_NT) GS_KEY(MP_ROWS) GS_KEY(MP_SOLO) GS_KEY(MP_COL_PERM) GS_KEY(MP_PERM_HOT) GS_KEY(MP_PERM_SCATTER)
 #undef GS_KEY
     throw gs_error("get_config_int: no integer key " + k);
 }
diff --git a/generalsparse_amd/csrc/host/gs_core.hpp b/generalsparse_amd/csrc/host/gs_core.hpp
--- a/generalsparse_amd/csrc/host/gs_core.hpp
+++ b/generalsparse_amd/csrc/host/gs_core.hpp
@@ -90,6 +90,7 @@
     int64_t KS_FORCE_TIMEOUT = 0;
     int64_t KS_PRIO = 1;
     int64_t KS_NT = 0;
+    int64_t KS_WPOS = 0;
     int64_t KS_HEAD = 1;
     int64_t KS_PERSIST = 0;
     int64_t MP_HUB_COLS = 0;
diff --git a/generalsparse_amd/csrc/host/gs_plan.hpp b/generalsparse_amd/csrc/host/gs_plan.hpp
--- a/generalsparse_amd/csrc/host/gs_plan.hpp
+++ b/generalsparse_amd/csrc/host/gs_plan.hpp
@@ -12,6 +12,7 @@
     void *col = nullptr, *val = nullptr;
     void *pad_out = nullptr;
     void *tcol = nullptr, *tval = nullptr;
+    void *tw = nullptr;
     uint32_t *t0 = nullptr, *t1 = nullptr, *t2 = nullptr, *t3 = nullptr, *t4 = nullptr;
     uint32_t *a0 = nullptr, *a1 = nullptr, *a2 = nullptr, *a3 = nullptr, *a4 = nullptr;
     uint64_t *m0 = nullptr;
@@ -40,6 +41,7 @@
     uint32_t ks_ctw = 0;
     bool ks_ap = true;
     bool ks_p8 = false;
+    bool ks_wp = false;
     uint32_t ks_gh = 0;
     uint32_t ks_nt = 0;
     uint32_t ks_persist = 0;
diff --git a/generalsparse_amd/csrc/kernels/device_plan.hip b/generalsparse_amd/csrc/kernels/device_plan.hip
--- a/generalsparse_amd/csrc/kernels/device_plan.hip
+++ b/generalsparse_amd/csrc/kernels/device_plan.hip
@@ -557,12 +557,15 @@
             d.ks_ctw = kt.CT;
             d.ks_ap = kt.AP;
             d.ks_p8 = kt.P8;
+            d.ks_wp = kt.WP;
             d.ks_nt = kt.NT;
             d.ks_gh = kt.GH;
             d.ks_persist = (uint32_t)std::max<int64_t>(0, get_config().KS_PERSIST);
             if (d.ks_persist) a.t3 = dev_copy(d, std::vector<uint32_t>(9, 0u));
             a.t0 = dev_copy(d, to_u32(mc.tbr, "BMTB first_row_indices"));
-            a.tcol = kt.P8 ? (void *)dev_copy(d, kt.pos8) : (void *)dev_copy(d, kt.pos);
+            GS_CHECK(!(kt.WP && d.ks_persist), "KS_WPOS: window positions are not built for the persistent grid (KS_PERSIST)");
+            a.tcol = kt.P8 || kt.WP ? (void *)dev_copy(d, kt.pos8) : (void *)dev_copy(d, kt.pos);
+            if (kt.WP) a.tw = dev_copy(d, kt.win);
             a.tval = dev_copy(d, kt.val);
             a.t1 = dev_copy(d, kt.steps);
             d.bytes_tile = d.bytes_A - before;
@@ -926,6 +929,7 @@
     r.m0 = (uint64_t *)dup(s.m0);
     r.tcol = dup(s.tcol);
     r.tval = dup(s.tval);
+    r.tw = dup(s.tw);
     r.t0 = (uint32_t *)dup(s.t0);
     r.t1 = (uint32_t *)dup(s.t1);
     r.t2 = (uint32_t *)dup(s.t2);
diff --git a/generalsparse_amd/csrc/kernels/ks_launch.hip b/generalsparse_amd/csrc/kernels/ks_launch.hip
--- a/generalsparse_amd/csrc/kernels/ks_launch.hip
+++ b/generalsparse_amd/csrc/kernels/ks_launch.hip
@@ -46,6 +46,7 @@
         GS_CHECK(d.waves == kKsWaves && !d.ks_p8 && d.ks_ap && !d.ks_persist,
                  "k_mfma_ks at bf16 is built for 8 waves, 16-bit positions and the apart LDS layout: the experiments "
                  "variants (KS_WAVES, KS_POS8, KS_APART = 0, KS_PERSIST) are fp16 kernels");
+        GS_CHECK(!d.ks_wp, "k_mfma_ks at bf16 is built for 16-bit positions: KS_WPOS is an fp16 layout");
     }
 #ifdef GS_EXPERIMENTS
     if constexpr (F16 && W == (int)kKsWaves && !STAMPS) {
@@ -70,7 +71,7 @@
             hipLaunchKernelGGL(kd, dim3((uint32_t)d.n_rows_aux * d.ksplit, ks_col_tiles_ct(N, CT)), dim3(64 * W), d.lds_bytes, s,
                                a.t0, (const gsk::u32x4 *)a.tcol, (const gsk::u32x4 *)a.tval, (const gsk::u32x2 *)a.t1, B, C,
                                (uint32_t)p.K, N, d.ksplit, d.ks_ns, (uint32_t)d.n_rows_aux * d.ksplit, (uint32_t)d.row_base,
-                               a.ws, a.t2, stamps, ks_prio_arg());
+                               a.ws, a.t2, stamps, ks_prio_arg(), (const uint8_t *)nullptr);
             HIP_OK(hipGetLastError());
             return;
         }
@@ -79,14 +80,15 @@
         if (d.waves == 4) {
             if constexpr (CT == 2) {
                 GS_CHECK(!d.ks_ap, "k_mfma_ks with 4 waves runs the overlapped LDS layout");
-                auto k4 = d.ks_p8 ? gsk::k_mfma_ks<CT, RT, 4, (int)kKsDepth, MAXG, false, false, true>
-                                  : gsk::k_mfma_ks<CT, RT, 4, (int)kKsDepth, MAXG, false, false, false>;
+                GS_CHECK(!d.ks_wp, "k_mfma_ks: window positions (KS_WPOS) are built for 8 waves");
+                auto k4 = d.ks_p8 ? gsk::k_mfma_ks<CT, RT, 4, (int)kKsDepth, MAXG, false, false, gsk::kKsPos8>
+                                  : gsk::k_mfma_ks<CT, RT, 4, (int)kKsDepth, MAXG, false, false, gsk::kKsPosU16>;
                 GS_CHECK(gsk::ks_lds_bytes(CT, RT, 4, false) <= d.lds_bytes, "k_mfma_ks: LDS size disagrees with the upload");
                 grant_lds(d.device, k4, d.lds_bytes);
                 hipLaunchKernelGGL(k4, dim3((uint32_t)d.n_rows_aux * d.ksplit, ks_col_tiles_ct(N, CT)), dim3(256), d.lds_bytes,
                                    s, a.t0, (const gsk::u32x4 *)a.tcol, (const gsk::u32x4 *)a.tval, (const gsk::u32x2 *)a.t1, B,
                                    C, (uint32_t)p.K, N, d.ksplit, d.ks_ns, (uint32_t)d.n_rows_aux * d.ksplit,
-                                   (uint32_t)d.row_base, a.ws, a.t2, stamps, ks_prio_arg() | (d.ks_gh << 8));
+                                   (uint32_t)d.row_base, a.ws, a.t2, stamps, ks_prio_arg() | (d.ks_gh << 8), (const uint8_t *)nullptr);
                 HIP_OK(hipGetLastError());
                 return;
             } else {
@@ -98,21 +100,31 @@
     GS_CHECK(d.waves == kKsWaves && !d.ks_p8 && d.ks_ap,
              "k_mfma_ks with 4 or 16 waves, 8-bit positions or the overlapped LDS layout: experiments build");
 #endif
-    auto kern = gsk::k_mfma_ks<CT, RT, W, (int)kKsDepth, MAXG, STAMPS, true, false, 0, ET>;
+    auto kern = gsk::k_mfma_ks<CT, RT, W, (int)kKsDepth, MAXG, STAMPS, true, gsk::kKsPosU16, 0, ET>;
     if (d.ks_nt) {
         if constexpr ((CT == 2 || CT == 8) && (W == (int)kKsWaves || W == 12) && !STAMPS) {
             GS_CHECK(d.ks_ap && !d.ks_p8, "k_mfma_ks: non-temporal loads are built for the apart layout, 16-bit positions");
             GS_CHECK(d.ks_nt == 1, "k_mfma_ks: KS_NT is built for A's groups (1)");
-            kern = gsk::k_mfma_ks<CT, RT, W, (int)kKsDepth, MAXG, false, true, false, 1, ET>;
+            kern = gsk::k_mfma_ks<CT, RT, W, (int)kKsDepth, MAXG, false, true, gsk::kKsPosU16, 1, ET>;
         } else {
             throw gs_error("k_mfma_ks: non-temporal loads are built for N = 32 and 128-column tiles, 8 waves");
+        }
+    }
+    if (d.ks_wp) {
+        if constexpr (F16 && CT == 2 && W == (int)kKsWaves && !STAMPS) {
+            GS_CHECK(d.ks_ap && !d.ks_p8 && !d.ks_persist && a.tw,
+                     "k_mfma_ks: window positions are built for the apart LDS layout and the static grid");
+            kern = d.ks_nt ? gsk::k_mfma_ks<CT, RT, W, (int)kKsDepth, MAXG, false, true, gsk::kKsPosWin, 1>
+                           : gsk::k_mfma_ks<CT, RT, W, (int)kKsDepth, MAXG, false, true, gsk::kKsPosWin, 0>;
+        } else {
+            throw gs_error("k_mfma_ks: window positions (KS_WPOS) are built for fp16, N = 32, 8 waves");
         }
     }
 #ifdef GS_EXPERIMENTS
     if (d.ks_p8) {
         if constexpr (F16 && CT == 2 && W == (int)kKsWaves && !STAMPS) {
             GS_CHECK(d.ks_ap, "k_mfma_ks: 8-bit positions are built with the apart LDS layout");
-            kern = gsk::k_mfma_ks<CT, RT, W, (int)kKsDepth, MAXG, false, true, true>;
+            kern = gsk::k_mfma_ks<CT, RT, W, (int)kKsDepth, MAXG, false, true, gsk::kKsPos8>;
         } else {
             throw gs_error("k_mfma_ks: 8-bit positions are built for N = 32, 8 waves");
         }
@@ -127,7 +139,7 @@
 #ifdef GS_EXPERIMENTS
     if (d.ks_persist) {
         if constexpr (F16 && W == (int)kKsWaves && !STAMPS && (CT == 2 || CT == 8)) {
-            GS_CHECK(d.ks_ap && !d.ks_p8 && a.t3 && ks_col_tiles_ct(N, CT) == 1, "k_mfma_ks_persist: 8 waves, apart layout, one column tile");
+            GS_CHECK(d.ks_ap && !d.ks_p8 && !d.ks_wp && a.t3 && ks_col_tiles_ct(N, CT) == 1, "k_mfma_ks_persist: 8 waves, apart layout, 16-bit positions, one column tile");
             auto kp = d.ks_nt ? gsk::k_mfma_ks_persist<CT, RT, W, (int)kKsDepth, MAXG, 1>
                               : gsk::k_mfma_ks_persist<CT, RT, W, (int)kKsDepth, MAXG, 0>;
             grant_lds(d.device, kp, d.lds_bytes);
@@ -150,7 +162,7 @@
     hipLaunchKernelGGL(kern, dim3((uint32_t)d.n_rows_aux * d.ksplit, ks_col_tiles_ct(N, CT)), dim3(64 * W), d.lds_bytes, s, a.t0,
                        (const gsk::u32x4 *)a.tcol, (const gsk::u32x4 *)a.tval, (const gsk::u32x2 *)a.t1, B, C,
                        (uint32_t)p.K, N, d.ksplit, d.ks_ns, (uint32_t)d.n_rows_aux * d.ksplit, (uint32_t)d.row_base, a.ws, a.t2, stamps,
-                       ks_prio_arg() | (d.ks_gh << 8));
+                       ks_prio_arg() | (d.ks_gh << 8), (const uint8_t *)a.tw);
     HIP_OK(hipGetLastError());
 }
 
@@ -311,16 +323,24 @@
             return;
         }
     }
-    auto kern = gsk::k_mfma_ks_group<2, RT, W, (int)kKsDepth, MAXG, false, AP, 0, ET>;
+    auto kern = gsk::k_mfma_ks_group<2, RT, W, (int)kKsDepth, MAXG, gsk::kKsPosU16, AP, 0, ET>;
     if constexpr (F16) {
-        if (it[0].p->dev.ks_p8) kern = gsk::k_mfma_ks_group<2, RT, W, (int)kKsDepth, MAXG, true, AP>;
+        if (it[0].p->dev.ks_p8) kern = gsk::k_mfma_ks_group<2, RT, W, (int)kKsDepth, MAXG, gsk::kKsPos8, AP>;
     }
 #else
     GS_CHECK(!it[0].p->dev.ks_p8, "k_mfma_ks_group: 8-bit positions are an experiments-build layout");
-    auto kern = gsk::k_mfma_ks_group<2, RT, W, (int)kKsDepth, MAXG, false, AP, 0, ET>;
+    auto kern = gsk::k_mfma_ks_group<2, RT, W, (int)kKsDepth, MAXG, gsk::kKsPosU16, AP, 0, ET>;
 #endif
     if constexpr (AP) {
-        if (it[0].p->dev.ks_nt) kern = gsk::k_mfma_ks_group<2, RT, W, (int)kKsDepth, MAXG, false, true, 1, ET>;
+        if (it[0].p->dev.ks_nt) kern = gsk::k_mfma_ks_group<2, RT, W, (int)kKsDepth, MAXG, gsk::kKsPosU16, true, 1, ET>;
+    }
+    if (it[0].p->dev.ks_wp) {
+        if constexpr (F16 && AP) {
+            kern = it[0].p->dev.ks_nt ? gsk::k_mfma_ks_group<2, RT, W, (int)kKsDepth, MAXG, gsk::kKsPosWin, true, 1>
+                                      : gsk::k_mfma_ks_group<2, RT, W, (int)kKsDepth, MAXG, gsk::kKsPosWin, true, 0>;
+        } else {
+            throw gs_error("k_mfma_ks_group: window positions (KS_WPOS) are built for fp16, 8 waves");
+        }
     }
     GS_CHECK(!it.empty() && it.size() <= (size_t)gsk::kKsGroupMax, "k_mfma_ks_group: 1..32 entries");
     gsk::ks_group_args args;
@@ -348,6 +368,8 @@
         e.nwg = (uint32_t)d.n_rows_aux * d.ksplit;
         e.row_base = (uint32_t)d.row_base;
         e.pad0 = d.ks_gh;
+        GS_CHECK(d.ks_wp == it[0].p->dev.ks_wp && (!d.ks_wp || a.tw), "k_mfma_ks_group: entries of different position forms");
+        e.tW = (const uint8_t *)a.tw;
         args.begin[i] = wg;
         wg += (e.nwg + 7u) & ~7u;
     }
@@ -411,11 +433,12 @@
     const device_plan &d = p.dev;
     const bool w8 = d.waves == kKsWaves && d.ks_ap, w4 = d.waves == 4 && !d.ks_ap;
     if (!p.uploaded || !d.mfma || !d.ks || d.pad_rows || N != 32 || d.lds_N != 32 || !(w8 || w4) || d.ks_persist) return 0;
-    if (d.dtype == kBF16 && (d.ks_p8 || !w8)) return 0;
+    if (d.dtype == kBF16 && (d.ks_p8 || d.ks_wp || !w8)) return 0;
+    if (d.ks_wp && !w8) return 0;
 #ifndef GS_EXPERIMENTS
     if (d.ks_p8 || !w8) return 0;
 #endif
-    return (d.dtype == kBF16 ? 1u << 20 : 0u) | (d.ks_nt << 18) | (w4 ? 1u << 17 : 0u) | (d.ks_p8 ? 1u << 16 : 0u) | (d.maxr << 8) |
+    return (d.ks_wp ? 1u << 21 : 0u) | (d.dtype == kBF16 ? 1u << 20 : 0u) | (d.ks_nt << 18) | (w4 ? 1u << 17 : 0u) | (d.ks_p8 ? 1u << 16 : 0u) | (d.maxr << 8) |
            d.seg_cap;
 }
 
diff --git a/include/generalsparse.h b/include/generalsparse.h
--- a/include/generalsparse.h
+++ b/include/generalsparse.h
@@ -42,6 +42,7 @@
     uint32_t ks_nt;
     uint32_t ks_head_groups;
     uint32_t nm_tiles;
+    uint32_t ks_wpos;
 } gs_plan_info;
 
 const char *gs_last_error(void);
```

Result: faster. 40940 (median of 6 runs) (+3.5%).
